# microsoft/Sora

Measured on AMD Instinct MI355X. Metric: IQ Msamples/s through 802.11a 54 Mbps RX PHY, higher is better.
Workload: dtype int16 IQ / u8 path metrics

## Files before the change

### sora_amd/csrc/dev_sym11a.h

```cpp
#pragma once
#include "kernels.h"
#include "dev_viterbi.h"
#include "dev_pilot11a.h"

namespace sora {

__device__ __forceinline__ VitJob frame_vitjob(const FrameRow& r)
{
    VitJob J;
    J.valid = 1; J.soft_off = r.slot0 * (uint32_t)kSoftBytesPerSlot; J.nsoft = (uint32_t)r.nsym * 48u * r.nbpsc; J.length = r.length;
    J.dec_off = 0; J.out_off = r.slot0 * (uint32_t)kOutPerSlot; J.code_rate = r.code_rate; J.soft_bits = 3;
    return J;
}

__device__ __forceinline__ unsigned pilot_sgn(unsigned count)
{
    const unsigned w = count < 32 ? kPilotW0 : count < 64 ? kPilotW1 : count < 96 ? kPilotW2 : kPilotW3;
    return (w >> (count & 31u)) & 1u;
}
static __device__ __constant__ PilotPolarity kPilotSgn = kPilotPolarity;
__device__ __forceinline__ int pilot_angle(int th, unsigned count) { return kPilotSgn.neg[count] ? w16(th + 0x8000) : th; }

template <typename COEF> __device__ __forceinline__ pcx sym_freq_comp(uint32_t raw, COEF fq) { return pk_cmul<15>(pk_sra(raw, 1), pk_tw_mul(fq)); }
template <typename COEF> __device__ __forceinline__ pcx sym_equalise(pcx y, COEF ch, int bin)
{
    return (bin >= 28 && bin < 36) ? 0u : pk_cmul<8>(y, pk_tw_mul(ch));
}
template <typename COEF>
__device__ __forceinline__ void sym_front_quad(const uint32_t raw[4], const COEF fq[4], const COEF ch[4], uint32_t* sl, int e, const Fft64TwPk& W, uint32_t o[4])
{
    pcx x[4];
#pragma unroll
    for (int m = 0; m < 4; m++) x[m] = sym_freq_comp(raw[m], fq[m]);
    fft64_core_pk(x, sl, e, W, wave_lds_sync);
    const unsigned rv = __brev((unsigned)e) >> 28;
#pragma unroll
    for (int q = 0; q < 4; q++) o[q] = sym_equalise(sl[rv + 16u * ((q & 1) * 2 + (q >> 1))], ch[q], 4 * e + q);
    wave_lds_sync();
}

constexpr int kSlotIters = 4;
constexpr uint32_t kNoOwner = 0xFFFFFFFFu;
struct WaveSlots {
    uint32_t first;
    uint32_t my_own;
    unsigned long long owned;
    uint32_t row0;
    bool one_frame;
    __device__ __forceinline__ uint32_t slot(int it, int g) const { return first + 4u * (uint32_t)it + (uint32_t)g; }
    __device__ __forceinline__ uint32_t owner(int it, int g) const { return (uint32_t)__shfl((int)my_own, 4 * it + g); }
    __device__ __forceinline__ unsigned quad(int it) const { return (unsigned)(owned >> (4 * it)) & 0xFu; }
};
__device__ __forceinline__ WaveSlots wave_slots(const RxArgs& A, uint32_t bid)
{
    const int w = threadIdx.x >> 6, lane = threadIdx.x & 63;
    WaveSlots S;
    S.first = (bid * 4u + (uint32_t)w) * (4u * kSlotIters);
    const uint32_t my_slot = S.first + (uint32_t)(lane & 15);
    S.my_own = (lane < 16 && my_slot < A.total_slots) ? A.slot_row[my_slot] : kNoOwner;
    S.owned = __ballot(S.my_own != kNoOwner);
    S.row0 = S.owned ? (uint32_t)__builtin_amdgcn_readlane((int)S.my_own, __builtin_ctzll(S.owned)) : kNoOwner;
    S.one_frame = __ballot(lane < 16 && S.my_own != kNoOwner && S.my_own != S.row0) == 0;
    return S;
}

__device__ __forceinline__ int4 track_advance(int th1, int th2, int th3, int th4, bool act, int& cfo_comp, int& sfo_comp, int& cfo_tr, int& sfo_tr)
{
    const int c0 = cfo_comp, s0 = sfo_comp;
    const int avg = w16((th1 + th2 + th3 + th4) / 4);
    const int del = w16(((th3 - th1) / 28 + (th4 - th2) / 28) >> 1);
    if (act) {
        cfo_tr = w16(cfo_tr + (avg >> 2)); sfo_tr = w16(sfo_tr + (del >> 2));
        cfo_comp = w16(cfo_comp + avg + cfo_tr); sfo_comp = w16(sfo_comp + del + sfo_tr);
    }
    return int4{ c0, s0, act ? avg : 0, act ? del : 0 };
}

__device__ __forceinline__ int4 track_rec4(TrackRec t) { return int4{ t.cfo_comp, t.sfo_comp, t.avg, t.del }; }
__device__ __forceinline__ void sym_back_demap(const Tables& T, const uint8_t* s_demap, const uint32_t v3[3], int4 rec, int nb, int e, uint8_t* dst)
{
    cpx c1[3], c2[3];
#pragma unroll
    for (int m = 0; m < 3; m++) {
        const int bin = carrier_bin48(e + 16 * m);
        const int c = bin < 32 ? bin : bin - 64;
        c1[m] = rot_coeff(T, w16(rec.x + c * rec.y));
        c2[m] = rot_coeff(T, w16(rec.z + c * rec.w));
    }
#pragma unroll
    for (int m = 0; m < 3; m++) {
        const int k = e + 16 * m;
        cpx v = mul_q15(unpack(v3[m]), c1[m]);
        v = mul_q15(v, c2[m]);
        int re = v.re >> 4, im = v.im >> 4;
        re = min(max(re, -128), 127); im = min(max(im, -128), 127);
        const unsigned ur = (unsigned)re & 0xFF, ui = (unsigned)im & 0xFF;
        uint8_t* o = dst + k * nb;
        const int h = nb >> 1;
        o[0] = s_demap[ur];
        if (nb >= 2) {
            o[h] = s_demap[ui];
            if (nb >= 4) {
                const int t1 = nb == 4 ? 256 : 512;
                o[1] = s_demap[t1 + ur]; o[h + 1] = s_demap[t1 + ui];
                if (nb == 6) { o[2] = s_demap[768 + ur]; o[5] = s_demap[768 + ui]; }
            }
        }
    }
}

__device__ __forceinline__ bool deint_packs(int nb, int lane) { return 8 * lane < 48 * nb; }
__device__ __forceinline__ void deint_map_words(const Tables& T, int nb, int lane, uint32_t mp[4])
{
    const uint16_t* map = T.deint + (nb == 1 ? 0 : nb == 2 ? 1 : nb == 4 ? 2 : 3) * 288;
    const bool packs = deint_packs(nb, lane);
#pragma unroll
    for (int t = 0; t < 4; t++) mp[t] = packs ? (uint32_t)map[8 * lane + 2 * t] | ((uint32_t)map[8 * lane + 2 * t + 1] << 16) : 0u;
}
__device__ __forceinline__ uint32_t deint_gather24(const uint8_t* src, const uint32_t mp[4])
{
    uint32_t v[8];
#pragma unroll
    for (int t = 0; t < 4; t++) { v[2 * t] = src[mp[t] & 0xFFFFu]; v[2 * t + 1] = src[mp[t] >> 16]; }
    return soft3_pack8(v);
}

}
```

### sora_amd/csrc/dev_vit16.h

```cpp
#pragma once
#include <hip/hip_runtime.h>
#include "kernels.h"
#include "dev_viterbi.h"

namespace sora {
namespace {

template <int WIN, int LOOK> struct Geom16 {
    static constexpr int kMaxWalk = (WIN + LOOK + 7) / 8 + 2;
    static constexpr int P = kMaxWalk;
    static constexpr int kPathBytes = 40;
};

template <int WIN, int LOOK> struct Lds16 {
    uint16_t ring[Geom16<WIN, LOOK>::P][4][64];
    union {
        uint32_t udump[4][64];
        uint16_t ops[4][24][2];
        uint16_t ops2[2][4][24][2];
    };
    uint32_t path[8][Geom16<WIN, LOOK>::kPathBytes / 4];
};

constexpr unsigned kW[4] = { 0u, 21u, 42u, 63u };
// ... 8 lines not shown
{
    const unsigned c0 = v & 1u, c1 = (v >> 1) & 1u, c2 = (v >> 2) & 1u, c3 = (v >> 3) & 1u;
    return c0 ^ (c2 << 1) ^ (c1 << 3) ^ (c3 ? 7u : 0u);
}
__device__ __forceinline__ unsigned rev6u(unsigned x) { return __brev(x) >> 26; }

template <int CTRL> __device__ __forceinline__ unsigned dppx(unsigned v) { return (unsigned)__builtin_amdgcn_update_dpp(0, (int)v, CTRL, 0xF, 0xF, true); }

__device__ __forceinline__ unsigned partner(unsigned v, int ph)
{
    switch (ph) {
    case 0: return dppx<0x140>(v);
    case 1: return dppx<0x1B>(v);
    case 2: return dppx<0x141>(v);
    case 3: return dppx<0x4E>(v);
    case 4: return dppx<0x128>(v);
    default: return dppx<0xB1>(v);
    }
}

struct Vit16 {
    unsigned U[4];
    unsigned MX[24];
    unsigned MY[6];
    unsigned sadr[3][4];
};

template <int WHICH, int P>
__device__ __forceinline__ void acs16(Vit16& V, int t24, unsigned a, unsigned b, unsigned pos512[3])
{
    const int ph = t24 % 6, k = t24 % 8;
    const unsigned Kp = (WHICH == 0 ? 14u : 7u) * kFld + (kOne << k);
    unsigned bm;
    if (WHICH == 0)      bm = (a ^ V.MX[t24]) + (b ^ V.MY[ph]);
    else if (WHICH == 1) bm = a ^ V.MX[t24];
    else                 bm = b ^ V.MX[t24];
    const unsigned bo = Kp - bm;
    const int rx = ph == 0 ? 2 : ph == 1 ? 1 : 0;
    unsigned N[4];
#pragma unroll
    for (int i = 0; i < 4; i++) {
        const unsigned X = V.U[i], Y = partner(V.U[i ^ rx], ph);
        const bool wb = (kW[i] >> (5 - ph)) & 1u;
        N[i] = wb ? pk_min16(X + bo, Y + bm) : pk_min16(X + bm, Y + bo);
    }
#pragma unroll
    for (int i = 0; i < 4; i++) V.U[i] = N[i];
    if (k == 7) {
        const int jb = t24 / 8;
#pragma unroll
        for (int i = 0; i < 4; i++) {
            const unsigned w = bank_word(V.U[i]);
            const unsigned addr = V.sadr[jb][i] + pos512[jb];
            asm volatile("ds_write_b16 %0, %1" : : "v"(addr), "v"(w) : "memory");
            V.U[i] &= 0xFE00FE00u;
        }
    }
}

__device__ __forceinline__ unsigned row_min_u32(unsigned v)
{
    v = min(v, dppx<0xB1>(v)); v = min(v, dppx<0x4E>(v)); v = min(v, dppx<0x141>(v)); v = min(v, dppx<0x128>(v));
    return v;
}
__device__ __forceinline__ unsigned row_pkmin(unsigned v)
{
    v = pk_min16(v, dppx<0xB1>(v)); v = pk_min16(v, dppx<0x4E>(v)); v = pk_min16(v, dppx<0x141>(v)); v = pk_min16(v, dppx<0x128>(v));
    return v;
}
__device__ __forceinline__ unsigned wave_min_u32(unsigned v) { return (unsigned)__builtin_amdgcn_readfirstlane((int)dpp_min_u32_wave(v)); }
__device__ __forceinline__ unsigned wave_max_u32(unsigned v) { return ~wave_min_u32(~v); }

template <int CR, int WIN, int LOOK, int BITS>
struct Forward16 {
    static constexpr int P = Geom16<WIN, LOOK>::P, GB = Puncture<CR>::GB, GS = Puncture<CR>::GS, CW = Puncture<CR>::CW;
    static constexpr int NV = Puncture<CR>::NV;
    struct Chunk { uint32_t v[CW]; };
    struct Raw { SoftRaw r[NV]; };

    Vit16 V;
    unsigned row, half;
    uint32_t my_j;
    SoftCursor<BITS, CW> cur[NV];
    const uint8_t* soft;
    uint16_t* my_ops;
    const uint4* row_ops;
    uint32_t pos;
    unsigned pos512[3];
    uint32_t tr, nsteps;
    uint32_t next_thr;
    bool all_done;

    __device__ __forceinline__ void init(Lds16<WIN, LOOK>& S, const uint8_t* __restrict__ soft_, uint32_t my_soft_off, uint32_t my_first, uint32_t my_last, unsigned start,
                                         uint32_t nsteps_)
    {
        const unsigned lane = threadIdx.x & 63, l16 = lane & 15;
        row = lane >> 4; half = lane & 1u;
        const unsigned v0 = v_of_lane(l16);
        nsteps = nsteps_;
#pragma unroll
        for (int i = 0; i < 4; i++) V.U[i] = (v0 ^ kW[i]) == 0 ? 0u : start;
        const unsigned ring_base = (unsigned)(uintptr_t)&S.ring[0][0][0];
#pragma unroll
        for (int jb = 0; jb < 3; jb++)
#pragma unroll
            for (int i = 0; i < 4; i++) V.sadr[jb][i] = ring_base + ((row * 64u + rev6u(rol6(v0 ^ kW[i], jb == 0 ? 2 : jb == 1 ? 4 : 0))) << 1);
#pragma unroll
        for (int t = 0; t < 24; t++) {
            const int ph = t % 6, k = t % 8;
            const unsigned n = rol6(v0, ph + 1);
            const bool vb = (v0 >> (5 - ph)) & 1u;
            const unsigned ma = (__popc(n & 0155) & 1) ? 7u * kFld : 0u, mb = (__popc(n & 0117) & 1) ? 7u * kFld : 0u;
            const unsigned mx = Puncture<CR>::which_of(ph) == 2 ? mb : ma;
            V.MX[t] = vb ? ((mx ^ (7u * kFld)) | (kOne << k)) : mx;
            if (t < 6) V.MY[t] = vb ? (mb ^ (7u * kFld)) : mb;
        }
        tr = 0; pos = 0;
        my_j = l16 >> 1;
#pragma unroll
        for (int v = 0; v < NV; v++) cur[v].init(my_soft_off, my_first + my_j + 8u * v, my_last);
        soft = soft_;
        my_ops = &S.ops[row][my_j][half];
        row_ops = reinterpret_cast<const uint4*>(&S.ops[row][0][0]);
        set_row_pos();
    }
    __device__ __forceinline__ bool going() const { return tr < nsteps && !all_done; }

    __device__ __forceinline__ void normalize()
    {
        const unsigned m = row_pkmin(pk_min16(pk_min16(V.U[0], V.U[1]), pk_min16(V.U[2], V.U[3])));
#pragma unroll
        for (int i = 0; i < 4; i++) V.U[i] -= m;
    }
    static __device__ __forceinline__ uint32_t pos_of(uint32_t p, int jb) { const uint32_t q = p + 512u * (uint32_t)jb; return min(q, q - 512u * (uint32_t)P); }
    __device__ __forceinline__ void set_row_pos()
    {
        pos512[0] = pos; pos512[1] = pos_of(pos, 1); pos512[2] = pos_of(pos512[1], 1);
    }
    __device__ __forceinline__ void end_row() { pos = pos_of(pos512[2], 1); set_row_pos(); }
    __device__ __forceinline__ Raw fetch(uint32_t c) const
    {
        Raw R;
#pragma unroll
        for (int v = 0; v < NV; v++) R.r[v] = cur[v].fetch(soft, c);
        return R;
    }
    __device__ __forceinline__ void put(const Raw& R, uint16_t* mine) const
    {
#pragma unroll
        for (int v = 0; v < NV; v++) mine[16 * v] = (uint16_t)cur[v].field(R.r[v]);
    }
    static __device__ __forceinline__ Chunk get(const uint4* table)
    {
        Chunk K;
#pragma unroll
        for (int i = 0; i < (CW + 3) / 4; i++) {
            const uint4 x = table[i];
            K.v[4 * i] = x.x; K.v[4 * i + 1] = x.y;
            if (4 * i + 2 < CW) { K.v[4 * i + 2] = x.z; K.v[4 * i + 3] = x.w; }
        }
        return K;
    }
    __device__ __forceinline__ Chunk unpack(const Raw& R) const
    {
        put(R, my_ops);
        lds_fence();
        const Chunk K = get(row_ops);
        lds_fence();
        return K;
    }
    __device__ __forceinline__ void group(const Chunk& K, int h, int i0)
    {
        const int k0 = i0 / GS * GB, t24 = 12 * h + i0;
        acs16<0, P>(V, t24, K.v[k0], K.v[k0 + 1], pos512);
        if (CR != 0) acs16<1, P>(V, t24 + 1, K.v[k0 + 2], 0, pos512);
        if (CR == 2) acs16<2, P>(V, t24 + 2, 0, K.v[k0 + 3], pos512);
        if ((t24 + GS) % 8 == 0) normalize();
    }
    __device__ __forceinline__ void fast_chunk(const Chunk& K, int h)
    {
#pragma unroll
        for (int g = 0; g < 12 / GS; g++) group(K, h, g * GS);
        tr += 12;
    }
    template <typename CHECK> __device__ __forceinline__ void slow_chunk(const Chunk& K, int h, CHECK& check)
    {
#pragma unroll
        for (int g = 0; g < 12 / GS; g++) {
            if (going()) {
                group(K, h, g * GS);
                tr += GS;
                check(12 * h + g * GS + GS - 1);
            }
        }
    }
    template <typename CHECK> __device__ __forceinline__ void chunk(const Chunk& K, int h, CHECK& check)
    {
        if (tr + 12 <= nsteps && next_thr > tr + 12) fast_chunk(K, h); else slow_chunk(K, h, check);
    }
};

template <int WIN, int LOOK, bool LANE_OB = false>
__device__ __noinline__ void trace16(unsigned lds_off, unsigned U0, unsigned U1, unsigned U2, unsigned U3, uint32_t tr_, uint32_t ob_, uint32_t pj_, uint32_t k_,
                                     uint32_t my_cnt, uint8_t* my_out)
{
    using G = Geom16<WIN, LOOK>;
    constexpr int P = G::P, K = G::kMaxWalk;
    constexpr int NR = K - 1, NF = NR / 4, NW = K / 4 + 1;
    static_assert(NR % 4 == 0 || NR % 4 == 2, "the walk's words are packed in pairs");
    static_assert(NW * 4 <= G::kPathBytes && NW >= WIN / 32 + 1, "the stream's registers hold a window and fit Lds16::path");
    typedef __attribute__((address_space(3))) Lds16<WIN, LOOK> lds_t;
    typedef __attribute__((address_space(3))) const uint16_t lds_u16;
    lds_t& S = *(lds_t*)(uintptr_t)lds_off;
    auto uni = [](uint32_t v) { return (uint32_t)__builtin_amdgcn_readfirstlane((int)v); };
    const uint32_t tr = uni(tr_), ob = LANE_OB ? ob_ : uni(ob_), pj = uni(pj_), k = uni(k_);
    const unsigned lane = threadIdx.x & 63, row = lane >> 4, l16 = lane & 15, half = lane & 1u;
    const unsigned v0 = v_of_lane(l16);
    const unsigned U[4] = { U0, U1, U2, U3 };
    const uint32_t j = (tr - 1) >> 3, nn = tr - 8u * j, m_lo = ob >> 3;
    const unsigned rowbase = (unsigned)(uintptr_t)&S.ring[0][row][0], sh = 8u * half;
    auto ring_j = [&](unsigned idx) -> unsigned { return *(lds_u16*)(uintptr_t)(rowbase + pj + (idx << 1)); };
#pragma unroll
    for (int i = 0; i < 4; i++) S.udump[i][lane] = U[i];
    lds_fence();
    unsigned key[2] = { 0xFFFFFFFFu, 0xFFFFFFFFu };
#pragma unroll
    for (int i = 0; i < 4; i++) {
        const unsigned st = rol6(v0 ^ kW[i], tr);
        unsigned lastA, lastB;
        if (k == 7) { const unsigned w = ring_j(rev6u(st)); lastA = (w >> 7) & 1u; lastB = (w >> 15) & 1u; }
        else { lastA = (U[i] >> k) & 1u; lastB = (U[i] >> (17 + k)) & 1u; }
        const unsigned mA = ((U[i] & 0xFFFFu) >> 9 << 1) | lastA, mB = (U[i] >> 25 << 1) | lastB;
        key[0] = min(key[0], (mA << 8) | (st << 2)); key[1] = min(key[1], (mB << 8) | (st << 2));
// ... 63 lines not shown
```

### sora_amd/csrc/dev_viterbi.h

```cpp
#pragma once
#include <hip/hip_runtime.h>
#include "rx_types.h"

namespace sora {

__device__ __forceinline__ uint32_t uni(uint32_t v) { return (uint32_t)__builtin_amdgcn_readfirstlane((int)v); }
__device__ __forceinline__ void lds_fence() { __builtin_amdgcn_fence(__ATOMIC_RELEASE, "wavefront"); __builtin_amdgcn_wave_barrier();
    __builtin_amdgcn_fence(__ATOMIC_ACQUIRE, "wavefront"); }
constexpr uint32_t kNever = 0xFFFFFFFFu;

template <int CR> struct Puncture {
    static constexpr int GB = CR == 0 ? 2 : CR == 2 ? 4 : 3;
    static constexpr int GS = CR == 0 ? 1 : CR == 2 ? 3 : 2;
    static constexpr int CW = 12 / GS * GB;
    static constexpr int NV = (CW + 7) / 8;
    static constexpr int which_of(int ph) { return CR == 0 ? 0 : CR == 1 ? (ph & 1) : ph % 3; }
};

__device__ __forceinline__ unsigned rol6(unsigned v, unsigned r) { r %= 6; return ((v << r) | (v >> (6 - r))) & 63u; }
__device__ __forceinline__ unsigned lane_map(unsigned x) { return x ^ ((x & 4u) ? 3u : 0u); }

__device__ __forceinline__ unsigned dpp_min_u32_wave(unsigned v)
{
    v = min(v, (unsigned)__builtin_amdgcn_update_dpp(0, (int)v, 0xB1, 0xF, 0xF, true));
    v = min(v, (unsigned)__builtin_amdgcn_update_dpp(0, (int)v, 0x4E, 0xF, 0xF, true));
    v = min(v, (unsigned)__builtin_amdgcn_update_dpp(0, (int)v, 0x124, 0xF, 0xF, true));
    v = min(v, (unsigned)__builtin_amdgcn_update_dpp(0, (int)v, 0x128, 0xF, 0xF, true));
    auto r16 = __builtin_amdgcn_permlane16_swap(v, v, false, false);
    v = min(r16[0], r16[1]);
    auto r32 = __builtin_amdgcn_permlane32_swap(v, v, false, false);
    return min(r32[0], r32[1]);
}

typedef unsigned short u16x2_t __attribute__((ext_vector_type(2)));
__device__ __forceinline__ unsigned pk_add16(unsigned a, unsigned b) { return __builtin_bit_cast(unsigned, (u16x2_t)(__builtin_bit_cast(u16x2_t,
        a) + __builtin_bit_cast(u16x2_t, b))); }
__device__ __forceinline__ unsigned pk_sub16(unsigned a, unsigned b) { return __builtin_bit_cast(unsigned, (u16x2_t)(__builtin_bit_cast(u16x2_t,
        a) - __builtin_bit_cast(u16x2_t, b))); }
__device__ __forceinline__ unsigned pk_min16(unsigned a, unsigned b) { return __builtin_bit_cast(unsigned,
        __builtin_elementwise_min(__builtin_bit_cast(u16x2_t, a), __builtin_bit_cast(u16x2_t, b))); }

__device__ __forceinline__ unsigned dpp_pkmin_wave(unsigned v)
{
    v = pk_min16(v, (unsigned)__builtin_amdgcn_update_dpp(0, (int)v, 0xB1, 0xF, 0xF, true));
    v = pk_min16(v, (unsigned)__builtin_amdgcn_update_dpp(0, (int)v, 0x4E, 0xF, 0xF, true));
    v = pk_min16(v, (unsigned)__builtin_amdgcn_update_dpp(0, (int)v, 0x124, 0xF, 0xF, true));
    v = pk_min16(v, (unsigned)__builtin_amdgcn_update_dpp(0, (int)v, 0x128, 0xF, 0xF, true));
    auto r16 = __builtin_amdgcn_permlane16_swap(v, v, false, false);
    v = pk_min16(r16[0], r16[1]);
    auto r32 = __builtin_amdgcn_permlane32_swap(v, v, false, false);
    return pk_min16(r32[0], r32[1]);
}

__device__ __forceinline__ uint32_t soft3_pack8(const uint32_t v[8])
{
    return v[0] | (v[1] << 3) | (v[2] << 6) | (v[3] << 9) | (v[4] << 12) | (v[5] << 15) | (v[6] << 18) | (v[7] << 21);
}
__device__ __forceinline__ void soft3_store8(uint8_t* stream, uint32_t group, uint32_t bits24)
{
    uint8_t* p = stream + 3u * group;
    p[0] = (uint8_t)bits24; p[1] = (uint8_t)(bits24 >> 8); p[2] = (uint8_t)(bits24 >> 16);
}
struct SoftRaw { uint32_t w, sh; };
template <int BITS, int CW> struct SoftCursor {
    static constexpr int ADV = BITS * CW;
    static constexpr bool kConst = ADV % 8 == 0;
    uint32_t off;
    uint32_t pos;
    uint32_t lim;
    uint32_t lsh;
    __device__ __forceinline__ void init(uint32_t stream_off, uint32_t k, uint32_t last)
    {
        const uint32_t t0 = (uint32_t)BITS * min(k, last), tl = (uint32_t)BITS * last;
        if (kConst) { off = stream_off + (t0 >> 3); pos = 0; lim = stream_off + (tl >> 3); lsh = 9u - (t0 & 7u); }
        else { off = stream_off; pos = t0; lim = tl; lsh = 0; }
    }
    __device__ __forceinline__ SoftRaw fetch(const uint8_t* __restrict__ base, uint32_t c) const
    {
        SoftRaw r;
        if (kConst) { r.sh = 0; r.w = *reinterpret_cast<const uint16_t*>(base + min(off + c * (uint32_t)(ADV / 8), lim)); }
        else { const uint32_t t = min(pos + c * (uint32_t)ADV, lim); r.sh = t & 7u; r.w = *reinterpret_cast<const uint16_t*>(base + (off + (t >> 3))); }
        return r;
    }
    __device__ __forceinline__ uint32_t field(const SoftRaw& r) const
    {
        return kConst ? (r.w << lsh) & 0x0E00u : ((r.w >> r.sh) & 7u) << 9;
    }
};

constexpr unsigned kFld = (1u << 9) | (1u << 25);
constexpr unsigned kOne = 0x00020001u;
constexpr unsigned kGuard = 1u << 16;

template <int WIN, int LOOK> struct RingGeom {
    static constexpr int kMaxWalk = (WIN + LOOK + 7) / 8 + 2;
    static constexpr int P = (kMaxWalk + 2) / 3 * 3;
    static constexpr int kEntries = 2 * P * 64;
};

__device__ __forceinline__ unsigned bank_word(unsigned U) { return __builtin_amdgcn_perm(U >> 1, U, 0x0C0C0600u); }

struct VitLane {
    unsigned U;
    unsigned MX[24];
    unsigned MY[6];
    uint16_t* ring;
    unsigned rowpos;
    unsigned sidx[3];
};

template <int WHICH, int P>
__device__ __forceinline__ void acs_step(VitLane& V, int t24, unsigned a, unsigned b)
{
    const int ph = t24 % 6, k = t24 % 8;
    const unsigned Kp = (WHICH == 0 ? 14u : 7u) * kFld + (kOne << k);
    unsigned bm;
    if (WHICH == 0)      bm = (a ^ V.MX[t24]) + (b ^ V.MY[ph]);
    else if (WHICH == 1) bm = a ^ V.MX[t24];
    else                 bm = b ^ V.MX[t24];
    const unsigned bo = Kp - bm;
    unsigned X, Y;
    const int u = (int)V.U;
    switch (ph) {
    case 0: { auto r = __builtin_amdgcn_permlane32_swap(V.U, V.U, false, false); X = r[0]; Y = r[1]; break; }
    case 1: { auto r = __builtin_amdgcn_permlane16_swap(V.U, V.U, false, false); X = r[0]; Y = r[1]; break; }
    case 2: X = V.U; Y = (unsigned)__builtin_amdgcn_update_dpp(0, u, 0x128, 0xF, 0xF, true); break;
    case 3: X = V.U; Y = (unsigned)__builtin_amdgcn_update_dpp(0, u, 0x141, 0xF, 0xF, true); break;
    case 4: X = V.U; Y = (unsigned)__builtin_amdgcn_update_dpp(0, u, 0x4E, 0xF, 0xF, true); break;
    default: X = V.U; Y = (unsigned)__builtin_amdgcn_update_dpp(0, u, 0xB1, 0xF, 0xF, true); break;
    }
    V.U = pk_min16(X + bm, Y + bo);
    if (k == 7) {
        uint16_t* e = V.ring + V.rowpos + (t24 / 8) * 64 + V.sidx[t24 / 8];
        const uint16_t w = (uint16_t)bank_word(V.U);
        e[0] = w; e[P * 64] = w;
        V.U &= 0xFE00FE00u;
    }
}

template <int kMaxWalk>
__device__ __noinline__ void viterbi_trace(unsigned U, const uint16_t* ring, uint32_t tr_, uint32_t ob_, unsigned mA, unsigned mB,
                                           uint32_t cntA_, uint32_t cntB_, uint8_t* outA, uint8_t* outB, uint32_t top_)
{
    const unsigned lane = threadIdx.x & 63;
    auto uni = [](uint32_t v) { return (uint32_t)__builtin_amdgcn_readfirstlane((int)v); };
    const uint32_t tr = uni(tr_), ob = uni(ob_), cntA = uni(cntA_), cntB = uni(cntB_), top = uni(top_);
    auto rev6 = [](unsigned x) { return __brev(x) >> 26; };
    auto writelane = [](unsigned& vec, unsigned val, unsigned ln) {
        asm volatile("s_mov_b32 m0, %2\n\ts_nop 0\n\tv_writelane_b32 %0, %1, m0" : "+v"(vec) : "s"(val), "s"(ln) : "m0");
    };
    const unsigned lbl = rol6(lane_map(lane), tr) << 2;
    const unsigned kA = (unsigned)__builtin_amdgcn_readfirstlane((int)dpp_min_u32_wave((mA << 8) | lbl));
    const unsigned kB = (unsigned)__builtin_amdgcn_readfirstlane((int)dpp_min_u32_wave((mB << 8) | lbl));
    const unsigned stA = (kA >> 2) & 0x3F, stB = (kB >> 2) & 0x3F;
    const unsigned back = 6u - tr % 6u;
    const unsigned pA = (unsigned)__builtin_amdgcn_readlane((int)U, (int)lane_map(rol6(stA, back))) & 0xFFu;
    const unsigned pB = ((unsigned)__builtin_amdgcn_readlane((int)U, (int)lane_map(rol6(stB, back))) >> 17) & 0xFFu;
    const int m_lo = (int)(ob >> 3);
    const int j = (int)((tr - 1) >> 3);
    const unsigned n = tr - 8u * (unsigned)j;
    const int nblk = j - m_lo;
    __builtin_amdgcn_fence(__ATOMIC_RELEASE, "wavefront"); __builtin_amdgcn_wave_barrier(); __builtin_amdgcn_fence(__ATOMIC_ACQUIRE, "wavefront");
    const unsigned low = (unsigned)(uintptr_t)ring + ((((top - (unsigned)(kMaxWalk - 1)) << 6) | lane) << 1);
    uint32_t W[kMaxWalk];
#pragma unroll
    for (int i = 0; i < kMaxWalk; i++)
        asm volatile("ds_read_u16 %0, %1 offset:%2" : "=v"(W[i]) : "v"(low), "n"((kMaxWalk - 1 - i) * 128) : "memory");
    asm volatile("s_waitcnt lgkmcnt(0)" : "+v"(W[0]) : : "memory");
    unsigned HA, HB;
    if (n == 8) {
        HA = (unsigned)__builtin_amdgcn_readlane((int)W[0], (int)rev6(stA)) & 0xFFu;
        HB = ((unsigned)__builtin_amdgcn_readlane((int)W[0], (int)rev6(stB)) >> 8) & 0xFFu;
    } else { HA = pA & ((1u << n) - 1u); HB = pB & ((1u << n) - 1u); }
    unsigned qA = rev6(((stA >> n) | rev6(HA & 0x3Fu)) & 0x3Fu), qB = rev6(((stB >> n) | rev6(HB & 0x3Fu)) & 0x3Fu);
    unsigned tA = 0, tB = 0;
    asm volatile("s_nop 1\n\tv_writelane_b32 %0, %2, 0\n\tv_writelane_b32 %1, %3, 0" : "+v"(tA), "+v"(tB) : "s"(HA), "s"(HB << 8));
#pragma unroll
    for (int i = 1; i < kMaxWalk; i++) {
        unsigned t;
        asm volatile("v_readlane_b32 %[a], %[w], %[a]\n\t"
                     "v_readlane_b32 %[t], %[w], %[b]\n\t"
                     "s_lshr_b32 %[b], %[t], 8\n\t"
                     "v_writelane_b32 %[ta], %[a], %[i]\n\t"
                     "v_writelane_b32 %[tb], %[t], %[i]"
                     : [a] "+s"(qA), [b] "+s"(qB), [t] "=&s"(t), [ta] "+v"(tA), [tb] "+v"(tB) : [w] "v"(W[i]), [i] "n"(i));
    }
    const int at = (nblk - (int)lane) << 2;
    const unsigned loA = (unsigned)__builtin_amdgcn_ds_bpermute(at, (int)tA) & 0xFFu, upA = (unsigned)__builtin_amdgcn_ds_bpermute(at - 4, (int)tA) & 0xFFu;
    const unsigned loB = ((unsigned)__builtin_amdgcn_ds_bpermute(at, (int)tB) >> 8) & 0xFFu, upB = ((unsigned)__builtin_amdgcn_ds_bpermute(at - 4, (int)tB) >> 8) & 0xFFu;
    if (lane < (cntA >> 3)) outA[m_lo + (int)lane] = (uint8_t)((loA >> 6) | ((upA & 0x3Fu) << 2));
    if (lane < (cntB >> 3)) outB[m_lo + (int)lane] = (uint8_t)((loB >> 6) | ((upB & 0x3Fu) << 2));
}

struct VitSide {
    uint8_t* out; uint32_t nsteps, tr_end; bool done;
    uint32_t soft_off, last, i0;
};

struct WholeFrames {
    __device__ __forceinline__ uint32_t next_event(uint32_t t) const { return t; }
    template <typename E> __device__ __forceinline__ void at_event(E&) {}
    template <typename E> __device__ __forceinline__ void window_done(E&) {}
};

template <int CR, int WIN, int LOOK, int BITS>
struct VitForward {
    using RG = RingGeom<WIN, LOOK>;
    static constexpr int P = RG::P, GB = Puncture<CR>::GB, GS = Puncture<CR>::GS, CW = Puncture<CR>::CW;
    struct Chunk { uint32_t v[(CW + 3) / 4 * 4]; };

    VitLane V;
    VitSide A, B;
    uint32_t nsteps;
    uint32_t tr, ob;
    uint32_t next_thr;
    SoftCursor<BITS, CW> cur;
    const uint8_t* soft_base;
    uint16_t *ops, *my_op;

    __device__ __forceinline__ void init(const VitSide& A_, const VitSide& B_, unsigned start, uint32_t ob0, const uint8_t* __restrict__ soft_base_, uint16_t* ring, uint16_t* ops_)
    {
        const unsigned lane = threadIdx.x & 63;
        A = A_; B = B_;
        nsteps = max(A.nsteps, B.nsteps);
        const VitSide& M = lane >= 32u && !B.done ? B : A;
        const uint32_t my_k = lane & 31u;

        const unsigned vl = lane_map(lane);
        V.U = vl == 0 ? 0u : start;
        V.ring = ring; V.rowpos = 0;
        V.sidx[0] = __brev(rol6(vl, 2)) >> 26; V.sidx[1] = __brev(rol6(vl, 4)) >> 26; V.sidx[2] = __brev(vl) >> 26;
#pragma unroll
        for (int t = 0; t < 24; t++) {
            const int ph = t % 6, k = t % 8;
            const unsigned n = rol6(vl, ph + 1);
            const bool own1 = ph >= 2 && ((vl >> (5 - ph)) & 1);
            const unsigned ma = (__popc(n & 0155) & 1) ? 7u * kFld : 0u, mb = (__popc(n & 0117) & 1) ? 7u * kFld : 0u;
            const unsigned mx = Puncture<CR>::which_of(ph) == 2 ? mb : ma;
            V.MX[t] = own1 ? ((mx ^ (7u * kFld)) | (kOne << k)) : mx;
            if (t < 6) V.MY[t] = own1 ? (mb ^ (7u * kFld)) : mb;
        }
        tr = 0; ob = ob0;
        cur.init(M.soft_off, my_k + M.i0, M.last);
        soft_base = soft_base_; ops = ops_;
        my_op = ops + 2u * my_k + (lane >> 5);
    }
    __device__ __forceinline__ bool going() const { return tr < nsteps && !(A.done && B.done); }

    __device__ __forceinline__ void normalize() { V.U = V.U - dpp_pkmin_wave(V.U); }
    __device__ __forceinline__ SoftRaw fetch(uint32_t c) const { return cur.fetch(soft_base, c); }
    __device__ __forceinline__ Chunk unpack(const SoftRaw& R)
    {
        *my_op = (uint16_t)cur.field(R);
        lds_fence();
        Chunk K;
#pragma unroll
        for (int i = 0; i < (CW + 3) / 4; i++) {
            const uint4 x = reinterpret_cast<const uint4*>(ops)[i];
            K.v[4 * i] = x.x; K.v[4 * i + 1] = x.y; K.v[4 * i + 2] = x.z; K.v[4 * i + 3] = x.w;
        }
        lds_fence();
        return K;
    }
    __device__ __forceinline__ void group(const Chunk& K, int h, int i0)
    {
        const int k0 = i0 / GS * GB, t24 = 12 * h + i0;
        acs_step<0, P>(V, t24, K.v[k0], K.v[k0 + 1]);
        if (CR != 0) acs_step<1, P>(V, t24 + 1, K.v[k0 + 2], 0);
        if (CR == 2) acs_step<2, P>(V, t24 + 2, 0, K.v[k0 + 3]);
        if ((t24 + GS) % 8 == 0) normalize();
    }
    __device__ __forceinline__ void end_row() { V.rowpos = V.rowpos + 3 * 64 == (unsigned)P * 64 ? 0u : V.rowpos + 3 * 64; }
    __device__ __forceinline__ void fast_chunk(const Chunk& K, int h)
    {
#pragma unroll
        for (int g = 0; g < 12 / GS; g++) group(K, h, g * GS);
        tr += 12;
    }

    template <typename SCHED> __device__ __forceinline__ uint32_t next_event(const SCHED& sched) const
    {
        uint32_t t = ob + (uint32_t)(WIN + LOOK + 6);
        if (!A.done) t = min(t, A.tr_end);
        if (!B.done) t = min(t, B.tr_end);
        return sched.next_event(t);
    }
    template <typename SCHED> __device__ __forceinline__ void check(SCHED& sched, int t24_last)
    {
        if (tr >= next_thr) {
            sched.at_event(*this);
            const int k = t24_last % 8;
            const uint32_t pos = V.rowpos + (uint32_t)(t24_last / 8) * 64u;
            unsigned lastA, lastB;
            if (k == 7) { const unsigned w = V.ring[pos + V.sidx[t24_last / 8]]; lastA = (w >> 7) & 1u; lastB = (w >> 15) & 1u; }
            else { lastA = (V.U >> k) & 1u; lastB = (V.U >> (17 + k)) & 1u; }
            const unsigned mA = ((V.U & 0xFFFFu) >> 9 << 1) | lastA, mB = (V.U >> 25 << 1) | lastB;
            const bool partial = tr >= ob + (uint32_t)(WIN + LOOK + 6);
            uint32_t cntA = 0, cntB = 0;
            if (!A.done) {
                if (tr >= A.tr_end) { cntA = A.tr_end - ob - 6; A.done = true; }
                else if (partial) cntA = WIN;
            }
            if (!B.done) {
                if (tr >= B.tr_end) { cntB = B.tr_end - ob - 6; B.done = true; }
                else if (partial) cntB = WIN;
            }
            if (cntA | cntB) viterbi_trace<RG::kMaxWalk>(V.U, V.ring, tr, ob, mA, mB, cntA, cntB, A.out, B.out, (pos >> 6) + (uint32_t)P);
            if (partial) { ob += WIN; sched.window_done(*this); }
            next_thr = next_event(sched);
        }
    }
    template <typename SCHED> __device__ __forceinline__ void slow_chunk(SCHED& sched, const Chunk& K, int h)
    {
#pragma unroll
        for (int g = 0; g < 12 / GS; g++) {
            if (going()) {
                group(K, h, g * GS);
                tr += GS;
                check(sched, 12 * h + g * GS + GS - 1);
            }
        }
    }
    template <typename SCHED> __device__ __forceinline__ void chunk(SCHED& sched, const Chunk& K, int h)
    {
        if (tr + 12 <= nsteps && next_thr > tr + 12) fast_chunk(K, h); else slow_chunk(sched, K, h);
    }

    template <typename SCHED> __device__ __forceinline__ void run(SCHED& sched)
    {
        next_thr = next_event(sched);
        uint32_t c = 0;
        SoftRaw r0 = fetch(0), r1 = fetch(1);
        while (going()) {
            const uint32_t lim = min(nsteps, next_thr - 1);
            for (uint32_t rows = lim > tr ? (lim - tr) / 24 : 0; rows > 0; rows--) {
                const Chunk K0 = unpack(r0); r0 = fetch(c + 2);
// ... 20 lines not shown
```

### sora_amd/csrc/dev_vitwin.h

```cpp
#pragma once
#include <hip/hip_runtime.h>
#include <type_traits>
#include "dev_vit16.h"
#include "dev_winplan.h"

namespace sora {

namespace {

struct UnitGeom {
    uint32_t soft_off, last;
    uint32_t i0;
    uint32_t nsteps;
    uint32_t ob;
    uint32_t tr_end;
    uint32_t vstep, estep;
    uint32_t wleft;
    uint32_t vec;
    uint8_t* out;
    uint32_t need;
    uint32_t idx;
    bool valid, first;
};

// ... 12 lines not shown
    g.soft_off = J.soft_off; g.last = max(J.nsoft, 1u) - 1u;
    g.i0 = s0 / GS * GB;
    g.nsteps = has ? J.nsoft / GB * GS - s0 : 0u;
    g.ob = (uint32_t)WIN * k0 - s0;
    g.tr_end = J.length * 8u + 16u + 6u - s0;
    g.vstep = (has && u != 0) ? (uint32_t)kWinWarm : kNever;
    g.estep = (has && !last) ? (uint32_t)WIN * k1 / 24u * 24u - s0 : kNever;
    g.wleft = last ? 0x10000u : m;
    g.vec = vbase + idx * q + u;
    g.out = out + J.out_off + (s0 >> 3);
    g.need = last ? J.nsoft : min(J.nsoft, (((uint32_t)WIN * k1 + (uint32_t)LOOK + 6u + GS) / GS + 1u) * GB);
    g.idx = idx;
    return g;
}

struct UnitRef { uint32_t idx, uu, m, nun; };
template <int CR, int WIN, int LOOK>
__device__ __forceinline__ UnitRef unit_ref(const VitJob& J, uint32_t n, uint32_t p, uint32_t q, bool inside, uint32_t upos, uint32_t idx)
{
    const uint32_t nev = win_events(J.length, CR, WIN, LOOK), m = win_per_unit(nev, q), nun = (nev + m - 1u) / m;
    const uint32_t uu = !inside ? kWinNone : m != 1u ? (upos < nun ? upos : kWinNone) : n == 1u ? win_unit_lone(upos, nun) : (upos < nun ? win_unit_at(upos, nun) : kWinNone);
    return UnitRef{ idx, uu, m, nun };
}
template <int CR, int WIN, int LOOK, typename JOBS>
__device__ __forceinline__ UnitGeom unit_geom(JOBS job_at, uint32_t n, uint32_t p, uint32_t q, uint32_t vbase, uint8_t* __restrict__ out)
{
    const bool inside = p < win_slots(n, q);
    const uint32_t upos = inside ? p / n : 0u, idx = inside ? p - upos * n : 0u;
    const VitJob J = job_at(idx);
    const UnitRef R = unit_ref<CR, WIN, LOOK>(J, n, p, q, inside, upos, idx);
    return unit_of<CR, WIN, LOOK>(J, idx, R.uu, R.m, R.nun, q, vbase, out);
}
template <int CR, int WIN, int LOOK, typename JOBS>
__device__ __forceinline__ UnitGeom unit_geom_direct(JOBS job_at, uint32_t idx, uint32_t u, bool exists, uint32_t q, uint32_t vbase, uint8_t* __restrict__ out)
{
    const VitJob J = job_at(idx);
    const uint32_t nev = win_events(J.length, CR, WIN, LOOK), m = win_per_unit(nev, q), nun = (nev + m - 1u) / m;
    return unit_of<CR, WIN, LOOK>(J, idx, exists && u < nun ? u : kWinNone, m, nun, q, vbase, out);
}

template <int CR, int WIN, int LOOK, int BITS, typename READY>
__device__ __forceinline__ void forward16w(Lds16<WIN, LOOK>& S, const uint8_t* __restrict__ soft, const UnitGeom& GA, const UnitGeom& GB_, uint16_t* __restrict__ vecs, READY ready)
{
    using F16 = Forward16<CR, WIN, LOOK, BITS>;
    using Raw = typename F16::Raw;
    constexpr uint32_t THR = WIN + LOOK + 6;
    const unsigned l16 = threadIdx.x & 15;
    const UnitGeom& Mine = (threadIdx.x & 1u) ? GB_ : GA;
    F16 F;
    F.init(S, soft, Mine.soft_off, Mine.i0, Mine.last, (GA.first ? 0x18u << 9 : 0u) | (GB_.first ? 0x18u << 25 : 0u), wave_max_u32(max(GA.nsteps, GB_.nsteps)));

    uint32_t my_ob = Mine.ob, my_wleft = Mine.wleft;
    const uint32_t my_tr_end = Mine.tr_end;
    bool my_done = !Mine.valid;
    uint32_t vstepA = GA.vstep, vstepB = GB_.vstep, estepA = GA.estep, estepB = GB_.estep;

    auto trace = [&](uint32_t my_cnt, int t24_last) {
        trace16<WIN, LOOK, true>((unsigned)(uintptr_t)&S, F.V.U[0], F.V.U[1], F.V.U[2], F.V.U[3], F.tr, my_ob, F16::pos_of(F.pos, t24_last / 8), (uint32_t)(t24_last % 8), my_cnt,
                                 Mine.out);
    };
    auto next_event = [&]() -> uint32_t {
        uint32_t mine = my_done ? kNever : min(my_ob + THR, my_tr_end);
        mine = min(min(mine, min(vstepA, vstepB)), min(estepA, estepB));
        return wave_min_u32(mine);
    };
    F.next_thr = next_event();
    F.all_done = wave_min_u32(my_done ? 1u : 0u) != 0u;
    auto save = [&](uint32_t vec, int which, bool hi) {
        uint16_t* d = vecs + ((size_t)vec * 2u + (uint32_t)which) * 64u + l16;
#pragma unroll
        for (int i = 0; i < 4; i++) d[16 * i] = (uint16_t)(hi ? F.V.U[i] >> 16 : F.V.U[i]);
    };
    auto check = [&](int t24_last) {
        if (F.tr >= F.next_thr) {
            if (F.tr == vstepA) { save(GA.vec, 0, false); vstepA = kNever; }
            if (F.tr == vstepB) { save(GB_.vec, 0, true); vstepB = kNever; }
            if (F.tr == estepA) { save(GA.vec, 1, false); estepA = kNever; }
            if (F.tr == estepB) { save(GB_.vec, 1, true); estepB = kNever; }
            uint32_t cnt = 0; bool partial = false;
            if (!my_done) {
                if (F.tr >= my_tr_end) { cnt = my_tr_end - my_ob - 6; my_done = true; }
                else if (F.tr >= my_ob + THR) { cnt = WIN; partial = true; }
            }
            if (wave_max_u32(cnt) != 0u) trace(cnt, t24_last);
            if (partial) { my_ob += WIN; if (--my_wleft == 0) my_done = true; }
            F.next_thr = next_event();
            F.all_done = wave_min_u32(my_done ? 1u : 0u) != 0u;
        }
    };

    uint32_t c = 0;
    if (!ready()) return;
    Raw b0 = F.fetch(0), b1 = F.fetch(1), b2, b3;
    while (F.going()) {
        const uint32_t lim = min(F.nsteps, F.next_thr - 1);
        uint32_t rows = lim > F.tr ? (lim - F.tr) / 24 : 0;
        for (; rows > 0; rows--) {
            b2 = F.fetch(c + 2);
            F.fast_chunk(F.unpack(b0), 0);
            b3 = F.fetch(c + 3);
            F.fast_chunk(F.unpack(b1), 1);
            F.end_row();
            b0 = b2; b1 = b3;
            c += 2;
        }
        if (!(F.tr < F.nsteps)) break;
        b2 = F.fetch(c + 2);
        F.chunk(F.unpack(b0), 0, check);
        if (!F.going()) break;
        b3 = F.fetch(c + 3);
        F.chunk(F.unpack(b1), 1, check);
        F.end_row();
        b0 = b2; b1 = b3;
        c += 2;
    }
}

template <int WIN, int LOOK, int BITS, typename JOBSOF, typename READY>
__device__ __forceinline__ void viterbi16w_wave(Lds16<WIN, LOOK>& S, uint32_t wave_index, JOBSOF jobs_of, READY ready, const uint32_t* __restrict__ hdr,
        uint32_t target, uint32_t vstride,
                                                const uint8_t* __restrict__ soft, uint8_t* __restrict__ out, uint16_t* __restrict__ vecs)
{
    const uint32_t n[3] = { hdr[0], hdr[1], hdr[2] };
    const uint32_t q = uni(win_units_per_frame(n[0] + n[1] + n[2], target));
    uint32_t w = uni(wave_index), list = 0;
    while (list < 3 && w >= (win_slots(n[list], q) + 7) / 8) { w -= (win_slots(n[list], q) + 7) / 8; list++; }
    if (list >= 3) return;
    const uint32_t nl = uni(n[list]);
    const auto job_at = jobs_of(list);
    const unsigned lane = threadIdx.x & 63, row = lane >> 4;
    const uint32_t pa = 8u * w + 2u * row, pb = pa + 1u, vbase = list * vstride;
    const uint32_t code_rate = uni(job_at(0).code_rate);
    auto run = [&](auto cr) {
        constexpr int CR = decltype(cr)::value;
        UnitGeom A = unit_geom<CR, WIN, LOOK>(job_at, nl, pa, q, vbase, out), B = unit_geom<CR, WIN, LOOK>(job_at, nl, pb, q, vbase, out);
        if (__ballot(A.valid || B.valid) == 0) return;
        if (!B.valid) { const bool v = false; B = A; B.valid = v; B.vstep = B.estep = kNever; B.nsteps = 0; }
        if (!A.valid) { const bool v = false; const UnitGeom T = B; A = T; A.valid = v; A.vstep = A.estep = kNever; A.nsteps = 0; }
        forward16w<CR, WIN, LOOK, BITS>(S, soft, A, B, vecs, [&]() { return ready(A, B, list); });
    };
    if (code_rate == 0) run(std::integral_constant<int, 0>{});
    else if (code_rate == 1) run(std::integral_constant<int, 1>{});
    else run(std::integral_constant<int, 2>{});
}

template <int WIN, int LOOK, int BITS>
__device__ __forceinline__ void viterbi16w_body(const VitJob* __restrict__ jobs, const uint32_t* __restrict__ hdr, uint32_t jstride, uint32_t target, uint32_t vstride,
                                                const uint8_t* __restrict__ soft, uint8_t* __restrict__ out, uint16_t* __restrict__ vecs)
{
    __shared__ Lds16<WIN, LOOK> S;
    auto jobs_of = [&](uint32_t list) { const VitJob* __restrict__ jl = jobs + (size_t)list * jstride; return [jl](uint32_t idx) { return jl[idx]; }; };
    auto ready = [](const UnitGeom&, const UnitGeom&, uint32_t) { return true; };
    viterbi16w_wave<WIN, LOOK, BITS>(S, blockIdx.x, jobs_of, ready, hdr, target, vstride, soft, out, vecs);
}

}

}
```

### sora_amd/csrc/host_trellis.h

```cpp
#pragma once
#include <algorithm>
#include <optional>
#include "host_calls.h"
#include "kernels.h"
#include "dev_winplan.h"

namespace sora {

enum class Trellis { Lanes64, Lanes16, Windowed };
using TrellisChoice = std::optional<Trellis>;
inline int trellis_abi(Trellis t) { return t == Trellis::Lanes16 ? 16 : t == Trellis::Windowed ? SORA_TRELLIS_WINDOWED : 64; }
inline int trellis_abi(const TrellisChoice& c) { return c ? trellis_abi(*c) : 0; }
inline bool trellis_parse(int lanes_per_pair, TrellisChoice* out)
{
    if (lanes_per_pair == 0) *out = std::nullopt;
    else if (lanes_per_pair == 16) *out = Trellis::Lanes16;
    else if (lanes_per_pair == 64) *out = Trellis::Lanes64;
    else if (lanes_per_pair == SORA_TRELLIS_WINDOWED) *out = Trellis::Windowed;
    else return false;
    return true;
}

constexpr uint32_t kWinUnitsTarget = 16384;
constexpr uint32_t kWinLoneWaves = 3 * kWinLonePad / 8;
inline uint64_t win_units(uint64_t rows) { return std::min<uint64_t>(std::max<uint64_t>(kWinUnitsTarget, rows), (uint64_t)kWinMaxUnits * rows); }
inline uint64_t win_waves(uint64_t rows) { return (win_units(rows) + 7) / 8 + 3 + kWinLoneWaves; }
inline uint32_t win_vstride(uint64_t rows) { return (uint32_t)(win_units(rows) + rows); }

struct TrellisJobs { const VitJob* jobs; const uint32_t* hdr; uint32_t n, stride; bool single; };
inline TrellisJobs trellis_lists(const VitJob* jobs, const uint32_t* hdr, uint32_t n, uint32_t stride) { return TrellisJobs{ jobs, hdr, n, stride, false }; }
inline TrellisJobs trellis_single(const VitJob* jobs, const uint32_t* hdr, uint32_t n) { return TrellisJobs{ jobs, hdr, n, n, true }; }
inline uint32_t trellis_pair_groups(const TrellisJobs& J) { return J.single ? (J.n + 7) / 8 : (J.n / 2 + 3 + 3) / 4; }
inline uint32_t trellis_waves16(const TrellisJobs& J) { return (J.n + 7) / 8 + (J.single ? 0u : 2u); }
inline uint32_t trellis_win_waves(const TrellisJobs& J)
{
    return J.single ? (win_slots(J.n, win_units_per_frame(J.n, kWinUnitsTarget)) + 7) / 8 : (uint32_t)win_waves(J.n);
}

constexpr size_t kWinStatsBytes = 4 * kWinStatBanks * sizeof(unsigned long long);
struct WinScratch {
    uint16_t* d_vecs = nullptr; unsigned long long* d_stats = nullptr; uint32_t stride = 0;

    unsigned long long* redone() const { return d_stats + kWinStatsBytes / sizeof(unsigned long long); }
    int ensure(uint64_t cap_rows, hipStream_t zero_on, bool extra)
    {
        if (d_vecs) return SORA_OK;
        stride = win_vstride(cap_rows);
        HIPCHK(hipMalloc((void**)&d_vecs, 3 * (size_t)kWinVecBytes * stride));
        HIPCHK(hipMalloc((void**)&d_stats, kWinStatsBytes + sizeof(unsigned long long)));
        const size_t bytes = kWinStatsBytes + (extra ? sizeof(unsigned long long) : 0);
        if (zero_on) HIPCHK(hipMemsetAsync(d_stats, 0, bytes, zero_on));
        else HIPCHK(hipMemset(d_stats, 0, bytes));
        return SORA_OK;
    }
    void free() { (void)hipFree(d_vecs); (void)hipFree(d_stats); d_vecs = nullptr; d_stats = nullptr; stride = 0; }
};
inline int win_stats_add(const unsigned long long* d_stats, hipStream_t st, unsigned long long out[4])
{
    unsigned long long v[4 * kWinStatBanks];
    HIPCHK(hipMemcpyAsync(v, d_stats, sizeof v, hipMemcpyDeviceToHost, st));
    HIPCHK(hipStreamSynchronize(st));
    for (unsigned i = 0; i < 4 * kWinStatBanks; i++) out[i & 3u] += v[i];
    return SORA_OK;
}
template <typename P> inline int win_stats_sum(P* const* s, int n, int device, unsigned long long out[4])
{
    HIPCHK(hipSetDevice(device));
    for (int i = 0; i < 4; i++) out[i] = 0;
    for (int i = 0; i < n; i++) if (s[i] && s[i]->win.d_stats) { const int rc = win_stats_add(s[i]->win.d_stats, s[i]->stream, out); if (rc) return rc; }
    return SORA_OK;
}

template <int WIN> inline void trellis_proof(const TrellisJobs& J, const uint8_t* soft, uint8_t* out, const WinScratch& W, hipStream_t st)
{
    static_assert(WIN == 256 || WIN == 192, "the 802.11a (256) or the 802.11n (192) window schedule");
    if constexpr (WIN == 256)
        hipLaunchKernelGGL(k_win_redo, dim3(trellis_pair_groups(J)), dim3(256), 0, st, J.jobs, J.hdr, J.stride, kWinUnitsTarget, W.stride, (const uint16_t*)W.d_vecs, soft, out, W.d_stats);
    else
        hipLaunchKernelGGL(k_win_redo_11n, dim3(trellis_pair_groups(J)), dim3(256), 0, st, J.jobs, J.hdr, J.stride, kWinUnitsTarget, W.stride, (const uint16_t*)W.d_vecs, soft, out, W.d_stats);
}
template <int WIN> inline void trellis_launch(Trellis kind, const TrellisJobs& J, const uint8_t* soft, uint8_t* out, hipStream_t st, const WinScratch& W = WinScratch(),
        bool proof = true)
{
    static_assert(WIN == 256 || WIN == 192, "the 802.11a (256) or the 802.11n (192) window schedule");
    const uint32_t* hdr = J.single ? nullptr : J.hdr;
    const uint32_t n1 = J.single ? J.n : 0u, stride = J.single ? 0u : J.stride;
    if (kind == Trellis::Windowed) {
        if constexpr (WIN == 256) hipLaunchKernelGGL(k_viterbi16w, dim3(trellis_win_waves(J)), dim3(64), 0, st, J.jobs, J.hdr, J.stride, kWinUnitsTarget, W.stride, soft, out, W.d_vecs);
        else hipLaunchKernelGGL(k_viterbi16w_11n, dim3(trellis_win_waves(J)), dim3(64), 0, st, J.jobs, J.hdr, J.stride, kWinUnitsTarget, W.stride, soft, out, W.d_vecs);
        if (proof) trellis_proof<WIN>(J, soft, out, W, st);
    } else if (kind == Trellis::Lanes16) {
        if constexpr (WIN == 256) hipLaunchKernelGGL(k_viterbi16, dim3(trellis_waves16(J)), dim3(64), 0, st, J.jobs, hdr, n1, stride, soft, out);
        else hipLaunchKernelGGL(k_viterbi16_11n, dim3(trellis_waves16(J)), dim3(64), 0, st, J.jobs, hdr, n1, stride, soft, out);
    } else {
        if constexpr (WIN == 256) hipLaunchKernelGGL(k_viterbi, dim3(trellis_pair_groups(J)), dim3(256), 0, st, J.jobs, hdr, n1, stride, soft, out);
        else hipLaunchKernelGGL(k_viterbi11n, dim3(trellis_pair_groups(J)), dim3(256), 0, st, J.jobs, hdr, n1, stride, soft, out);
    }
}

}
```

### sora_amd/csrc/k_rx.hip

```cpp
#include <hip/hip_runtime.h>
#include <utility>
#include "kernels.h"
#include "dev_sym11a.h"
#include "dev_viterbi.h"
#include "dev_winplan.h"
#include "dev_vitwin.h"

namespace sora {

struct FrameLds {
    uint32_t eq[4][4][64];
    uint8_t  soft[4][4][288];
    uint8_t  demap[1024];
    int4     trk[4][4];
    int      nsym_of[4];
    short    st0[4][4];
};
template <bool SHARED>
__device__ __forceinline__ void frame_symbols(const RxArgs& A, uint32_t j, FrameLds& lds, bool valid = true)
{
    uint32_t (&s_eq)[4][4][64] = lds.eq; uint8_t (&s_soft)[4][4][288] = lds.soft; const uint8_t* s_demap = lds.demap;
    const int w = threadIdx.x >> 6, lane = threadIdx.x & 63, g = lane >> 4, e = lane & 15;
    const Tables& T = A.T;
    const uint32_t f = valid ? A.joblist[j] : 0u;
// ... 15 lines not shown
    const int pbin = pk == 0 ? 43 : pk == 1 ? 57 : pk == 2 ? 7 : 21, pc = pk == 0 ? -21 : pk == 1 ? -7 : pk == 2 ? 7 : 21;
    int cfo_comp = r.cfo_comp, sfo_comp = r.sfo_comp, cfo_tr = r.cfo_tracker, sfo_tr = r.sfo_tracker;
    unsigned symbol_count = 0;

    const uint32_t str_shift = A.str >> 1;
    auto load_samples = [&](int s0, uint32_t raw[4]) {
        const uint32_t p0 = r.data_start + __umul24(80u, (uint32_t)min(s0 + g, nsym)) + 8u + (uint32_t)e;
#pragma unroll
        for (int m = 0; m < 4; m++) raw[m] = iq[(p0 + 16u * (uint32_t)m) << str_shift];
    };
    int nsym_loop = nsym, nsym_f = nsym;
    if (SHARED) {
        if (lane == 0) { lds.nsym_of[w] = nsym; lds.st0[w][0] = (short)cfo_comp; lds.st0[w][1] = (short)sfo_comp; lds.st0[w][2] = (short)cfo_tr; lds.st0[w][3] = (short)sfo_tr; }
        __syncthreads();
        nsym_loop = max(max(lds.nsym_of[0], lds.nsym_of[1]), max(lds.nsym_of[2], lds.nsym_of[3]));
        const int fr = (lane >> 2) & 3;
        nsym_f = lds.nsym_of[fr];
        cfo_comp = lds.st0[fr][0]; sfo_comp = lds.st0[fr][1]; cfo_tr = lds.st0[fr][2]; sfo_tr = lds.st0[fr][3];
    }
    uint32_t raw[4] = { 0u, 0u, 0u, 0u };
    if (1 <= nsym) load_samples(1, raw);
    for (int s0 = 1; s0 <= nsym_loop; s0 += 4) {
        const int sym = s0 + g;
        const bool active = sym <= nsym;
        const bool mine = s0 <= nsym;
        int4 rec = { 0, 0, 0, 0 };
        if (mine) {
            pcx x[4], Y[4];
#pragma unroll
            for (int m = 0; m < 4; m++) x[m] = sym_freq_comp(raw[m], fq[m]);
            if (s0 + 4 <= nsym) load_samples(s0 + 4, raw);
            fft64_core_pk(x, s_eq[w][g], e, W, wave_lds_sync);
#pragma unroll
            for (int q = 0; q < 4; q++) Y[q] = s_eq[w][g][__brev((unsigned)(e + 16 * q)) >> 26];
            wave_lds_sync();
#pragma unroll
            for (int q = 0; q < 4; q++) s_eq[w][g][e + 16 * q] = sym_equalise(Y[q], ch[q], e + 16 * q);
            wave_lds_sync();
        }
        if (SHARED) {
            __syncthreads();
            if (w == 0) {
                const int fr = (lane >> 2) & 3;
#pragma unroll
                for (int gg = 0; gg < 4; gg++) {
                    const cpx p = mul_q15(unpack(s_eq[fr][gg][pbin]), rot_coeff(T, w16(cfo_comp + pc * sfo_comp)));
                    const int th = pilot_angle(pk == 3 ? uatan2(T, -p.im, -p.re) : uatan2(T, p.im, p.re), (symbol_count + (unsigned)gg) % 127u);
                    int th1 = __builtin_amdgcn_update_dpp(0, th, 0x00, 0xF, 0xF, true), th2 = __builtin_amdgcn_update_dpp(0, th, 0x55, 0xF, 0xF, true);
                    int th3 = __builtin_amdgcn_update_dpp(0, th, 0xAA, 0xF, 0xF, true), th4 = __builtin_amdgcn_update_dpp(0, th, 0xFF, 0xF, 0xF, true);
                    asm volatile("" : "+v"(th1), "+v"(th2), "+v"(th3), "+v"(th4));
                    const int4 t = track_advance(th1, th2, th3, th4, s0 + gg <= nsym_f, cfo_comp, sfo_comp, cfo_tr, sfo_tr);
                    if (lane < 16 && pk == 0) lds.trk[fr][gg] = t;
                }
            }
            symbol_count = (symbol_count + 4u) % 127u;
            __syncthreads();
            rec = lds.trk[w][g];
        } else {
            int4 t[4];
#pragma unroll
            for (int gg = 0; gg < 4; gg++) {
                t[gg] = int4{ cfo_comp, sfo_comp, 0, 0 };
                if (s0 + gg <= nsym) {
                    const cpx p = mul_q15(unpack(s_eq[w][gg][pbin]), rot_coeff(T, w16(cfo_comp + pc * sfo_comp)));
                    const int th = pilot_angle(pk == 3 ? uatan2(T, -p.im, -p.re) : uatan2(T, p.im, p.re), symbol_count);
                    symbol_count++; if (symbol_count >= 127) symbol_count = 0;
                    t[gg] = track_advance(__builtin_amdgcn_readlane(th, 0), __builtin_amdgcn_readlane(th, 1), __builtin_amdgcn_readlane(th, 2), __builtin_amdgcn_readlane(th, 3),
                                          true, cfo_comp, sfo_comp, cfo_tr, sfo_tr);
                }
            }
            rec = t[0];
            if (g == 1) rec = t[1]; else if (g == 2) rec = t[2]; else if (g == 3) rec = t[3];
        }
        if (!mine) continue;
        if (active) {
            uint32_t v3[3];
#pragma unroll
            for (int m = 0; m < 3; m++) v3[m] = s_eq[w][g][carrier_bin48(e + 16 * m)];
            sym_back_demap(T, s_demap, v3, rec, nb, e, s_soft[w][g]);
        }
        wave_lds_sync();
        {
            const int nact = min(4, nsym - s0 + 1);
            const uint32_t sym_bytes = 3u * (uint32_t)ncbps / 8u;
            uint8_t* d = dst + (size_t)(s0 - 1) * sym_bytes;
            for (int gs = 0; gs < nact; gs++, d += sym_bytes)
                if (packs) soft3_store8(d, (uint32_t)lane, deint_gather24(s_soft[w][gs], mp));
        }
        wave_lds_sync();
    }
}
__global__ void __launch_bounds__(256) k_frame(RxArgs A)
{
    __shared__ FrameLds lds;
    reinterpret_cast<uint32_t*>(lds.demap)[threadIdx.x] = reinterpret_cast<const uint32_t*>(A.T.demap)[threadIdx.x];
    __syncthreads();
    if (!locate_job(blockIdx.x * 4, A.njobs).ok) return;
    const JobRef jr = locate_job(blockIdx.x * 4 + (threadIdx.x >> 6), A.njobs);
    frame_symbols<true>(A, jr.ok ? jr.list * A.nrows + jr.idx : 0u, lds, jr.ok);
}

typedef uint32_t u32x4_t __attribute__((ext_vector_type(4)));
__device__ __forceinline__ void store16_through(uint4* p, uint4 v)
{
    const u32x4_t x = { v.x, v.y, v.z, v.w };
    asm volatile("global_store_dwordx4 %0, %1, off sc1\n\ts_nop 1" : : "v"(p), "v"(x) : "memory");
}
__device__ __forceinline__ void store4_through(uint32_t* p, uint32_t v) { __hip_atomic_store(p, v, __ATOMIC_RELAXED, __HIP_MEMORY_SCOPE_AGENT); }

template <bool THROUGH>
__device__ __forceinline__ void sym_front_block(const RxArgs& A, uint32_t bid, uint32_t (*s_eq)[4][64])
{
    const int w = threadIdx.x >> 6, lane = threadIdx.x & 63, g = lane >> 4, e = lane & 15;
    const Tables& T = A.T;
    const WaveSlots S = wave_slots(A, bid);
    if (S.owned == 0) return;
    uint32_t own[kSlotIters];
#pragma unroll
    for (int it = 0; it < kSlotIters; it++) own[it] = S.owner(it, g);
    const Fft64TwPk W = fft64_twiddles_pk(T, e);
    uint32_t* sl = s_eq[w][g];
    uint4* eq4 = reinterpret_cast<uint4*>(A.eq);
    auto store = [&](uint32_t slot, const uint32_t o[4]) {
        if (THROUGH) store16_through(eq4 + ((size_t)slot * 16u + (uint32_t)e), uint4{ o[0], o[1], o[2], o[3] });
        else eq4[(size_t)slot * 16u + (uint32_t)e] = uint4{ o[0], o[1], o[2], o[3] };
        auto pilot = [&](uint32_t k, uint32_t v) { if (THROUGH) store4_through(A.pil + ((size_t)slot * 4u + k), v); else A.pil[(size_t)slot * 4u + k] = v; };
        if (e == 10) pilot(0u, o[3]);
        if (e == 14) pilot(1u, o[1]);
        if (e == 1)  pilot(2u, o[3]);
        if (e == 5)  pilot(3u, o[1]);
    };
    if (S.one_frame) {
        const FrameRow& r = A.frames[S.row0];
        const uint32_t* iq = A.iq + A.caps[r.capture].offset;
        const uint32_t ds = r.data_start, s0 = r.slot0, str = A.str;
        const FrameCtx* fx = A.fctx + S.row0;
        uint32_t raw[kSlotIters][4];
#pragma unroll
        for (int it = 0; it < kSlotIters; it++) {
            const uint32_t p0 = ds + 80u * (S.slot(it, g) - s0) + 8u;
#pragma unroll
            for (int m = 0; m < 4; m++) raw[it][m] = own[it] != kNoOwner ? iq[(size_t)(p0 + (uint32_t)(e + 16 * m)) * str] : 0u;
        }
        PkTw fq[4], ch[4];
#pragma unroll
        for (int m = 0; m < 4; m++) { fq[m] = pk_tw_mul(fx->freq[e + 16 * m]); ch[m] = pk_tw_mul(fx->chan[4 * e + m]); }
#pragma unroll
        for (int it = 0; it < kSlotIters; it++) {
            if (S.quad(it) == 0) continue;
            uint32_t o[4];
            sym_front_quad(raw[it], fq, ch, sl, e, W, o);
            if (own[it] != kNoOwner) store(S.slot(it, g), o);
        }
        return;
    }
#pragma unroll 1
    for (int it = 0; it < kSlotIters; it++) {
        if (S.quad(it) == 0) continue;
        const uint32_t ow = S.owner(it, g);
        const bool mine = ow != kNoOwner;
        const uint32_t slot = S.slot(it, g);
        uint32_t raw[4] = { 0u, 0u, 0u, 0u };
        PkTw fq[4], ch[4];
        const FrameCtx* fx = A.fctx + (mine ? ow : 0u);
        if (mine) {
            const FrameRow& r = A.frames[ow];
            const uint32_t* iq = A.iq + A.caps[r.capture].offset;
            const uint32_t p0 = r.data_start + 80u * (slot - r.slot0) + 8u;
#pragma unroll
            for (int m = 0; m < 4; m++) raw[m] = iq[(size_t)(p0 + (uint32_t)(e + 16 * m)) * A.str];
        }
#pragma unroll
        for (int m = 0; m < 4; m++) { fq[m] = pk_tw_mul(mine ? fx->freq[e + 16 * m] : 0u); ch[m] = pk_tw_mul(mine ? fx->chan[4 * e + m] : 0u); }
        uint32_t o[4];
        sym_front_quad(raw, fq, ch, sl, e, W, o);
        if (mine) store(slot, o);
    }
}
// ... 25 lines not shown
                 "v_mov_b32_dpp %1, %4 quad_perm:[1,1,1,1] row_mask:0xf bank_mask:0xf bound_ctrl:1\n\t"
                 "v_mov_b32_dpp %2, %4 quad_perm:[2,2,2,2] row_mask:0xf bank_mask:0xf bound_ctrl:1\n\t"
                 "v_mov_b32_dpp %3, %4 quad_perm:[3,3,3,3] row_mask:0xf bank_mask:0xf bound_ctrl:1"
                 : "=&v"(th1), "=&v"(th2), "=&v"(th3), "=&v"(th4) : "v"(th));
    const int sum = th1 + th2 + th3 + th4;
    const int avg = (sum + ((sum >> 31) & 3)) >> 2;
    const int del = ((int)((float)(th3 - th1) * kInv28) + (int)((float)(th4 - th2) * kInv28)) >> 1;
    const uint2 rec = uint2{ __builtin_amdgcn_perm((uint32_t)sfo, (uint32_t)cfo, 0x05040100u), __builtin_amdgcn_perm((uint32_t)del, (uint32_t)avg, 0x05040100u) };
    ctr += avg >> 2; str += del >> 2;
    cfo = (int)((unsigned)cfo + (unsigned)avg + (unsigned)ctr); sfo = __builtin_amdgcn_sbfe(sfo + del + str, 0, 16);
    return rec;
}

__device__ __forceinline__ void track_tables_to_lds(const uint32_t* __restrict__ trk, TrkTables& s_t, uint32_t* s_pol)
{
    if (threadIdx.x < 127) {
        unsigned b = 0;
#pragma unroll
        for (unsigned u = 0; u < 8; u++) b |= pilot_sgn((threadIdx.x + u) % 127u) << u;
        s_pol[threadIdx.x] = b;
    }
    const uint4* src = reinterpret_cast<const uint4*>(trk);
    uint4* dst = reinterpret_cast<uint4*>(&s_t);
    constexpr uint32_t kWords = sizeof(TrkTables) / 16, kBatch = 11;
    for (uint32_t i0 = threadIdx.x; i0 < kWords; i0 += 256u * kBatch) {
        uint4 v[kBatch];
#pragma unroll
        for (uint32_t b = 0; b < kBatch; b++) v[b] = src[min(i0 + 256u * b, kWords - 1u)];
#pragma unroll
        for (uint32_t b = 0; b < kBatch; b++) if (i0 + 256u * b < kWords) dst[i0 + 256u * b] = v[b];
    }
}

__global__ void __launch_bounds__(256) k_track_lds(RxArgs A)
{
    __shared__ TrkTables s_t;
    __shared__ uint32_t s_pol[128];
    track_tables_to_lds(A.T.trk, s_t, s_pol);
    __syncthreads();
    const int lane = threadIdx.x & 63, pk = lane & 3;
    const JobRef jr = locate_job(blockIdx.x * 64u + (threadIdx.x >> 2), A.njobs);
    const uint32_t j = jr.ok ? jr.list * A.nrows + jr.idx : 0u;
    const uint32_t f = jr.ok ? A.joblist[j] : 0u;
    const FrameRow r = A.frames[f];
    const int nsym = jr.ok ? (int)r.nsym : 0;
    if (jr.ok && pk == 0) A.jobs[j] = frame_vitjob(r);
    const int pc = pk == 0 ? -21 : pk == 1 ? -7 : pk == 2 ? 7 : 21;
    const int m3 = pk == 3 ? -1 : 0;
    int cfo = r.cfo_comp, sfo = r.sfo_comp, ctr = r.cfo_tracker, str = r.sfo_tracker;
    int nmax = nsym;
#pragma unroll
    for (int o = 32; o >= 4; o >>= 1) nmax = max(nmax, __shfl_xor(nmax, o));
    nmax = __builtin_amdgcn_readfirstlane(nmax);
    const uint32_t w0 = (jr.ok ? (r.slot0 + 1u) * 4u + (uint32_t)pk : (uint32_t)pk) * 4u;
    const uint32_t t0 = (jr.ok ? r.slot0 + 1u : A.total_slots + 1u) * 8u;
    const char* __restrict__ pil = reinterpret_cast<const char*>(A.pil);
    char* __restrict__ trk2 = reinterpret_cast<char*>(A.track);
    const unsigned last = (unsigned)max(nsym, 1) - 1u, nrec = (unsigned)nsym;
    constexpr int kAhead = 8;
    uint32_t q[kAhead];
#pragma unroll
    for (int i = 0; i < kAhead; i++) q[i] = *reinterpret_cast<const uint32_t*>(pil + (w0 + 16u * min((unsigned)i, last)));
    unsigned cnt = 0;
    for (int s0 = 1; s0 <= nmax; s0 += kAhead) {
        const unsigned pol = (unsigned)__builtin_amdgcn_readfirstlane((int)s_pol[cnt]);
        cnt = cnt + (unsigned)kAhead >= 127u ? cnt + (unsigned)kAhead - 127u : cnt + (unsigned)kAhead;
#pragma unroll
        for (int u = 0; u < kAhead; u++) {
            const int s = s0 + u;
            const uint32_t cur = q[u];
            q[u] = *reinterpret_cast<const uint32_t*>(pil + (w0 + 16u * min((unsigned)(s + kAhead - 1), last)));
            const int flip = (int)((pol << (15 - u)) & 0x8000u);
            *reinterpret_cast<uint2*>(trk2 + (t0 + 8u * min((unsigned)(s - 1), nrec))) = track_step(s_t, cur, flip, pc, m3, cfo, sfo, ctr, str);
        }
    }
}

__global__ void __launch_bounds__(256) k_sym_back(RxArgs A)
{
    __shared__ uint8_t s_soft[4][4][288];
    __shared__ uint8_t s_demap[1024];
    const int w = threadIdx.x >> 6, lane = threadIdx.x & 63, g = lane >> 4, e = lane & 15;
    const Tables& T = A.T;
    reinterpret_cast<uint32_t*>(s_demap)[threadIdx.x] = reinterpret_cast<const uint32_t*>(T.demap)[threadIdx.x];
    __syncthreads();
    const WaveSlots S = wave_slots(A, blockIdx.x);
    if (S.owned == 0) return;
    int bins[3];
#pragma unroll
    for (int m = 0; m < 3; m++) bins[m] = carrier_bin48(e + 16 * m);
    if (S.one_frame) {
        const FrameRow& r = A.frames[S.row0];
        const int nb = __builtin_amdgcn_readfirstlane((int)r.nbpsc), ncbps = 48 * nb;
        const uint32_t slot0 = (uint32_t)__builtin_amdgcn_readfirstlane((int)r.slot0), sym_bytes = 3u * (uint32_t)ncbps / 8u;
        uint8_t* stream = A.soft + (size_t)slot0 * kSoftBytesPerSlot;
        const bool packs = deint_packs(nb, lane);
        uint32_t mp[4];
        deint_map_words(T, nb, lane, mp);
        TrackRec tr[kSlotIters]; uint32_t v3[kSlotIters][3];
#pragma unroll
        for (int it = 0; it < kSlotIters; it++) {
            const uint32_t slot = S.slot(it, g);
            const bool mine = (S.quad(it) >> g) & 1u;
            tr[it] = mine ? A.track[slot] : TrackRec{ 0, 0, 0, 0 };
#pragma unroll
            for (int m = 0; m < 3; m++) v3[it][m] = mine ? A.eq[(size_t)slot * 64u + (uint32_t)bins[m]] : 0u;
        }
#pragma unroll
        for (int it = 0; it < kSlotIters; it++) {
            const unsigned quad = S.quad(it);
            if (quad == 0) continue;
            if ((quad >> g) & 1u) sym_back_demap(T, s_demap, v3[it], track_rec4(tr[it]), nb, e, s_soft[w][g]);
            wave_lds_sync();
#pragma unroll
            for (int gs = 0; gs < 4; gs++) {
                if (!((quad >> gs) & 1u) || !packs) continue;
                const uint32_t sg = S.slot(it, gs);
                soft3_store8(stream + (size_t)(sg - slot0 - 1u) * sym_bytes, (uint32_t)lane, deint_gather24(s_soft[w][gs], mp));
            }
            wave_lds_sync();
        }
        return;
    }
    int cur_nb = 0; uint32_t mp[4] = { 0, 0, 0, 0 };
#pragma unroll 1
    for (int it = 0; it < kSlotIters; it++) {
        const unsigned quad = S.quad(it);
        if (quad == 0) continue;
        const uint32_t ow = S.owner(it, g);
        const bool mine = ow != kNoOwner;
        const uint32_t slot = S.slot(it, g);
        int nb = 0; uint32_t slot0 = 0;
        if (mine) {
            const FrameRow& r = A.frames[ow];
            nb = r.nbpsc; slot0 = r.slot0;
            uint32_t v3[3];
#pragma unroll
            for (int m = 0; m < 3; m++) v3[m] = A.eq[(size_t)slot * 64u + (uint32_t)bins[m]];
            sym_back_demap(T, s_demap, v3, track_rec4(A.track[slot]), nb, e, s_soft[w][g]);
        }
        wave_lds_sync();
#pragma unroll 1
        for (int gs = 0; gs < 4; gs++) {
            if (!((quad >> gs) & 1u)) continue;
            const int nbg = __shfl(nb, 16 * gs);
            const uint32_t slot0g = (uint32_t)__shfl((int)slot0, 16 * gs);
            if (nbg != cur_nb) { cur_nb = nbg; deint_map_words(T, nbg, lane, mp); }
            if (deint_packs(nbg, lane)) {
                const uint32_t sg = S.slot(it, gs);
                uint8_t* d = A.soft + (size_t)slot0g * kSoftBytesPerSlot + (size_t)(sg - slot0g - 1u) * (3u * 48u * (uint32_t)nbg / 8u);
                soft3_store8(d, (uint32_t)lane, deint_gather24(s_soft[w][gs], mp));
            }
        }
        wave_lds_sync();
    }
}

constexpr uint32_t kPipeMaxSym = 1376;
constexpr uint32_t kPipeRing = 512;
struct PipeTrackLds {
    TrkTables t;
    uint32_t pol[128];
    uint32_t pil[kPipeMaxSym][4];
    uint2 rec[kPipeRing];
    uint8_t demap[1024];
    uint8_t soft[3][4][288];
    uint32_t done;
    uint32_t next_quad[3];
    uint32_t give_up;
    uint32_t pad[11];
};
constexpr uint32_t kPipeLdsBytes = sizeof(PipeTrackLds);
static_assert(kPipeLdsBytes <= 160 * 1024 && sizeof(TrkTables) % 16 == 0, "k_pipe: a tracker workgroup's LDS");
static_assert(4 * sizeof(Lds16<256, 24>) <= kPipeLdsBytes, "k_pipe: four trellis waves' LDS");

#ifdef SORA_DBG_PIPE_TIMELINE
#define PIPE_STAMP(P, i) do { if ((threadIdx.x & 63) == 0) (P).flags[(P).stamp_base + (i)] = (uint32_t)wall_clock64(); } while (0)
#else
#define PIPE_STAMP(P, i) do {} while (0)
#endif
__device__ __forceinline__ uint32_t flag_load(const uint32_t* p) { return __hip_atomic_load(p, __ATOMIC_RELAXED, __HIP_MEMORY_SCOPE_AGENT); }
__device__ __forceinline__ bool pipe_expired(long long t0, uint32_t wait_ticks) { return wall_clock64() - t0 > (long long)wait_ticks; }

__device__ __forceinline__ void pipe_track_block(const RxArgs& A, const PipeArgs& P, uint32_t t, PipeTrackLds& L)
{
    const int w = threadIdx.x >> 6, lane = threadIdx.x & 63;
    const JobRef jr = locate_job(t, A.njobs);
    if (!jr.ok) return;
    track_tables_to_lds(A.T.trk, L.t, L.pol);
    reinterpret_cast<uint32_t*>(L.demap)[threadIdx.x] = reinterpret_cast<const uint32_t*>(A.T.demap)[threadIdx.x];
    const uint32_t j = jr.list * A.nrows + jr.idx, f = A.joblist[j];
    const FrameRow r = A.frames[f];
    const uint32_t nsym = min((uint32_t)r.nsym, kPipeMaxSym - 8u), slot0 = r.slot0;
    if (threadIdx.x == 0) {
        A.jobs[j] = frame_vitjob(r);
        L.done = 0; L.give_up = 0; L.next_quad[0] = 0; L.next_quad[1] = 1; L.next_quad[2] = 2;
    }
    if (w == 0) {
        const uint32_t b0 = (slot0 + 1u) >> 6, b1 = (slot0 + max(nsym, 1u)) >> 6;
        const uint32_t* fl = P.flags + 4u + 4u * A.nrows + b0 + (uint32_t)lane;
        const bool mine = b0 + (uint32_t)lane <= b1;
        const long long t0 = wall_clock64();
        bool gave_up = false;
        while (!__all(!mine || flag_load(fl) != 0u)) {
            if (pipe_expired(t0, P.wait_ticks)) { gave_up = true; break; }
            __builtin_amdgcn_s_sleep(8);
        }
        if (gave_up && lane == 0) { L.give_up = 1; atomicOr(P.flags, 1u); }
        PIPE_STAMP(P, 1);
    }
    __syncthreads();
    if (L.give_up) return;
    {
        const unsigned long long* src = reinterpret_cast<const unsigned long long*>(A.pil) + 2u * (size_t)(slot0 + 1u);
        unsigned long long* dst = reinterpret_cast<unsigned long long*>(&L.pil[0][0]);
        for (uint32_t i = threadIdx.x; i < 2u * (nsym + 8u); i += 256u) dst[i] = i < 2u * nsym ? __hip_atomic_load(src + i, __ATOMIC_RELAXED, __HIP_MEMORY_SCOPE_AGENT) : 0ull;
    }
    __syncthreads();
    if (w == 0) {
        __builtin_amdgcn_s_setprio(3);
        PIPE_STAMP(P, 2);
        if (lane < 4) {
            const int pk = lane & 3;
            const int pc = pk == 0 ? -21 : pk == 1 ? -7 : pk == 2 ? 7 : 21, m3 = pk == 3 ? -1 : 0;
            int cfo = r.cfo_comp, sfo = r.sfo_comp, ctr = r.cfo_tracker, str = r.sfo_tracker;
            unsigned cnt = 0;
            volatile uint32_t* done = &L.done; volatile uint32_t* nq = L.next_quad;
            for (uint32_t s0 = 1; s0 <= nsym; s0 += 8u) {
                if (s0 + 7u > kPipeRing) {
                    while (4u * min(min(nq[0], nq[1]), nq[2]) + kPipeRing < s0 + 7u) __builtin_amdgcn_s_sleep(1);
                }
                const unsigned pol = (unsigned)__builtin_amdgcn_readfirstlane((int)L.pol[cnt]);
                cnt = cnt + 8u >= 127u ? cnt + 8u - 127u : cnt + 8u;
                uint32_t q[8];
#pragma unroll
                for (int u = 0; u < 8; u++) q[u] = L.pil[s0 - 1u + (uint32_t)u][pk];
                const uint32_t ring = (s0 - 1u) & (kPipeRing - 1u);
#pragma unroll
                for (int u = 0; u < 8; u++) L.rec[ring + (uint32_t)u] = track_step(L.t, q[u], (int)((pol << (15 - u)) & 0x8000u), pc, m3, cfo, sfo, ctr, str);
                asm volatile("" ::: "memory");
                if (lane == 0) *done = min(s0 + 7u, nsym);
            }
        }
        PIPE_STAMP(P, 3);
        return;
    }
    __builtin_amdgcn_fence(__ATOMIC_ACQUIRE, "agent");
    const int h = w - 1, g = lane >> 4, e = lane & 15;
    const int nb = __builtin_amdgcn_readfirstlane((int)r.nbpsc), ncbps = 48 * nb;
    const uint32_t sym_bytes = 3u * (uint32_t)ncbps / 8u;
    uint8_t* stream = A.soft + (size_t)slot0 * kSoftBytesPerSlot;
    const bool packs = deint_packs(nb, lane);
    uint32_t mp[4];
    deint_map_words(A.T, nb, lane, mp);
    int bins[3];
#pragma unroll
    for (int m = 0; m < 3; m++) bins[m] = carrier_bin48(e + 16 * m);
    volatile uint32_t* done = &L.done; volatile uint32_t* nq = L.next_quad;
    uint32_t* my_count = P.flags + 4u + 4u * f + (uint32_t)h;
    uint32_t quads = 0;
    uint8_t* bytes = &L.soft[h][0][0];
    for (uint32_t k = (uint32_t)h; 4u * k < nsym; k += 3u) {
        const uint32_t nact = min(4u, nsym - 4u * k), s = 4u * k + 1u + (uint32_t)g;
        const bool mine = (uint32_t)g < nact;
        uint32_t v3[3];
#pragma unroll
        for (int m = 0; m < 3; m++) v3[m] = mine ? A.eq[(size_t)(slot0 + s) * 64u + (uint32_t)bins[m]] : 0u;
        while (*done < 4u * k + nact) __builtin_amdgcn_s_sleep(1);
        asm volatile("" ::: "memory");
        const uint2 rw = L.rec[(s - 1u) & (kPipeRing - 1u)];
        if (mine) sym_back_demap(A.T, L.demap, v3, int4{ (int16_t)rw.x, (int16_t)(rw.x >> 16), (int16_t)rw.y, (int16_t)(rw.y >> 16) }, nb, e, L.soft[h][g]);
        wave_lds_sync();
        uint32_t b24[4];
#pragma unroll
        for (int gs = 0; gs < 4; gs++) b24[gs] = deint_gather24(L.soft[h][gs], mp);
        wave_lds_sync();
        if (packs) {
#pragma unroll
            for (int gs = 0; gs < 4; gs++) soft3_store8(bytes + (uint32_t)gs * sym_bytes, (uint32_t)lane, b24[gs]);
        }
        wave_lds_sync();
        const uint32_t ndw = (nact * sym_bytes + 3u) / 4u;
        uint32_t* out32 = reinterpret_cast<uint32_t*>(stream + (size_t)(4u * k) * sym_bytes);
        for (uint32_t i = (uint32_t)lane; i < ndw; i += 64u) store4_through(out32 + i, reinterpret_cast<const uint32_t*>(bytes)[i]);
        asm volatile("s_waitcnt vmcnt(0)" ::: "memory");
        wave_lds_sync();
        quads++;
        if (lane == 0) { store4_through(my_count, quads); nq[h] = k + 3u; }
    }
    if (lane == 0) nq[h] = 0x3FFFFFFFu;
    PIPE_STAMP(P, 4 + h);
}

__device__ __forceinline__ bool pipe_units_ready(const RxArgs& A, const PipeArgs& P, uint32_t list, const UnitGeom& M, bool polls_, uint32_t wave_index)
{
    const unsigned lane = threadIdx.x & 63;
    const bool polls = polls_ && M.valid;
    const uint32_t f = A.joblist[(size_t)list * A.nrows + M.idx];
    const uint32_t ncbps = 48u * A.frames[f].nbpsc;
    const uint32_t quads = polls ? ((M.need + ncbps - 1u) / ncbps + 3u) / 4u : 0u;
    const uint32_t* c = P.flags + 4u + 4u * f;
    const long long t0 = wall_clock64();
    for (;;) {
        bool ok = true;
#pragma unroll
        for (uint32_t h = 0; h < 3; h++) ok = ok && flag_load(c + h) >= (quads + 2u - h) / 3u;
        if (__all(ok)) break;
        if (pipe_expired(t0, P.wait_ticks)) { if (lane == 0) atomicOr(P.flags, 1u); return false; }
        __builtin_amdgcn_s_sleep(2);
    }
    __builtin_amdgcn_fence(__ATOMIC_ACQUIRE, "agent");
    PIPE_STAMP(P, 16 + 2 * wave_index);
    return true;
}

__device__ __forceinline__ auto pipe_jobs_of(const RxArgs& A, uint32_t list)
{
    const uint32_t* jl = A.joblist + (size_t)list * A.nrows; const FrameRow* fr = A.frames;
    return [jl, fr](uint32_t idx) { return frame_vitjob(fr[jl[idx]]); };
}
__device__ __forceinline__ void pipe_trellis_wave(const RxArgs& A, const PipeArgs& P, uint32_t wave_index, Lds16<256, 24>& S)
{
    auto jobs_of = [&](uint32_t list) { return pipe_jobs_of(A, list); };
    auto ready = [&](const UnitGeom& GA, const UnitGeom& GB_, uint32_t list) -> bool {
        const unsigned lane = threadIdx.x & 63;
        return pipe_units_ready(A, P, list, (lane & 1u) ? GB_ : GA, (lane & 15u) < 2u, wave_index);
    };
    viterbi16w_wave<256, 24, 3>(S, wave_index, jobs_of, ready, A.njobs, P.target, P.vstride, (const uint8_t*)A.soft, A.vout, P.vecs);
    PIPE_STAMP(P, 17 + 2 * wave_index);
}


template <int CR, int WIN, int LOOK, int BITS>
__device__ __forceinline__ void viterbi_forward(const VitJob& JA, const VitJob& JB, bool hasB, const uint8_t* __restrict__ soft_base,
        uint8_t* __restrict__ out_base, uint16_t* ring, uint16_t* ops)
{
    auto side = [&](const VitJob& J, bool has) {
        VitSide s;
        s.out = out_base + J.out_off; s.nsteps = has ? J.nsoft / Puncture<CR>::GB * Puncture<CR>::GS : 0u; s.tr_end = has ? J.length * 8u + 16u + 6u : 0u; s.done = !has;
        s.soft_off = J.soft_off; s.last = max(J.nsoft, 1u) - 1u; s.i0 = 0;
        return s;
    };
    VitForward<CR, WIN, LOOK, BITS> F;
    F.init(side(JA, true), side(JB, hasB), 0x18u * kFld, 0, soft_base, ring, ops);
    WholeFrames sched;
    F.run(sched);
}

struct UnitSchedule64 {
    uint16_t* __restrict__ vecs;
    uint32_t vecA, vecB;
    uint32_t wA, wB, vstepA, vstepB, estepA, estepB;
    __device__ __forceinline__ uint32_t next_event(uint32_t t) const { return min(min(t, min(vstepA, vstepB)), min(estepA, estepB)); }
    __device__ __forceinline__ void save(unsigned U, uint32_t vec, int which, bool hi) const
    {
        vecs[((size_t)vec * 2u + (uint32_t)which) * 64u + (threadIdx.x & 63)] = (uint16_t)(hi ? U >> 16 : U);
    }
    template <typename E> __device__ __forceinline__ void at_event(E& F)
    {
        if (F.tr == vstepA) { save(F.V.U, vecA, 0, false); vstepA = kNever; }
        if (F.tr == vstepB) { save(F.V.U, vecB, 0, true); vstepB = kNever; }
        if (F.tr == estepA) { save(F.V.U, vecA, 1, false); estepA = kNever; }
        if (F.tr == estepB) { save(F.V.U, vecB, 1, true); estepB = kNever; }
    }
    template <typename E> __device__ __forceinline__ void window_done(E& F)
    {
        if (!F.A.done && --wA == 0) F.A.done = true;
        if (!F.B.done && --wB == 0) F.B.done = true;
    }
};
template <int CR, int WIN, int LOOK, int BITS, typename READY>
__device__ __forceinline__ void viterbi_forward_unit(const UnitGeom& GA, const UnitGeom& GB_, const uint8_t* __restrict__ soft_base, uint16_t* ring, uint16_t* ops,
        uint16_t* __restrict__ vecs, READY ready)
{
    const bool hasB = GB_.valid;
    auto side = [](const UnitGeom& G, bool has) {
        VitSide s;
        s.out = G.out; s.nsteps = has ? G.nsteps : 0u; s.tr_end = has ? G.tr_end : 0u; s.done = !has;
        s.soft_off = G.soft_off; s.last = G.last; s.i0 = G.i0;
        return s;
    };
    VitForward<CR, WIN, LOOK, BITS> F;
    F.init(side(GA, true), side(GB_, hasB), (GA.first ? 0x18u << 9 : 0u) | ((hasB && GB_.first) ? 0x18u << 25 : 0u), GA.ob, soft_base, ring, ops);
    UnitSchedule64 sched{ vecs, GA.vec, GB_.vec, GA.wleft, GB_.wleft, GA.vstep, hasB ? GB_.vstep : kNever, GA.estep, hasB ? GB_.estep : kNever };
    if (!ready()) return;
    F.run(sched);
}

struct PipeUnitLds { uint16_t ring[RingGeom<256, 24>::kEntries]; uint16_t ops[64]; };
static_assert(4 * sizeof(PipeUnitLds) <= kPipeLdsBytes, "k_pipe: four 64-lane trellis waves' LDS");
__device__ __forceinline__ void pipe_trellis_wave64(const RxArgs& A, const PipeArgs& P, uint32_t wave_index, PipeUnitLds& L)
{
    const uint32_t n[3] = { A.njobs[0], A.njobs[1], A.njobs[2] };
    const uint32_t q = uni(win_units_per_frame(n[0] + n[1] + n[2], P.target));
    uint32_t w = uni(wave_index), list = 0;
    while (list < 3 && w >= q * ((n[list] + 1u) / 2u)) { w -= q * ((n[list] + 1u) / 2u); list++; }
    if (list >= 3) return;
    const uint32_t nl = uni(n[list]), pairs = (nl + 1u) / 2u, u = w / pairs, ia = 2u * (w - u * pairs), ib = ia + 1u;
    const auto job_at = pipe_jobs_of(A, list);
    const uint32_t code_rate = uni(job_at(0).code_rate), vbase = list * P.vstride;
    auto run = [&](auto cr) {
        constexpr int CR = decltype(cr)::value;
        UnitGeom GA = unit_geom_direct<CR, 256, 24>(job_at, ia, u, true, q, vbase, A.vout);
        UnitGeom GB_ = unit_geom_direct<CR, 256, 24>(job_at, ib < nl ? ib : ia, u, ib < nl, q, vbase, A.vout);
        if (GB_.valid && GA.valid && GB_.ob != GA.ob && (threadIdx.x & 63) == 0) atomicOr(P.flags, 1u);
        if (GB_.valid && (!GA.valid || GB_.ob != GA.ob)) { if (!GA.valid) { GA = GB_; } const bool no = false; GB_.valid = no; }
        if (!GA.valid) return;
        const unsigned lane = threadIdx.x & 63;
        viterbi_forward_unit<CR, 256, 24, 3>(GA, GB_, (const uint8_t*)A.soft, L.ring, L.ops, P.vecs,
                                             [&]() { return pipe_units_ready(A, P, list, lane >= 32u ? GB_ : GA, (lane & 31u) == 0u, wave_index); });
    };
    if (code_rate == 0) run(std::integral_constant<int, 0>{});
    else if (code_rate == 1) run(std::integral_constant<int, 1>{});
    else run(std::integral_constant<int, 2>{});
    PIPE_STAMP(P, 17 + 2 * wave_index);
}

__global__ void __launch_bounds__(256) k_pipe(RxArgs A, PipeArgs P)
{
    __shared__ __attribute__((aligned(16))) char lds[kPipeLdsBytes];
    uint32_t b = blockIdx.x;
    if (b == 0) PIPE_STAMP(P, 0);
    if (b < P.nfront) {
        sym_front_block<true>(A, b, reinterpret_cast<uint32_t (*)[4][64]>(lds));
        asm volatile("s_waitcnt vmcnt(0)" ::: "memory");
        __syncthreads();
#ifndef SORA_DBG_PIPE_LOSE_FLAGS
        if (threadIdx.x == 0) store4_through(P.flags + 4u + 4u * A.nrows + b, 1u);
#endif
        if (b == 0) PIPE_STAMP(P, 8);
        return;
    }
    b -= P.nfront;
    if (b < P.ntrack) { pipe_track_block(A, P, b, *reinterpret_cast<PipeTrackLds*>(lds)); return; }
    b -= P.ntrack;
    if (P.lanes64) pipe_trellis_wave64(A, P, b * 4u + (threadIdx.x >> 6), reinterpret_cast<PipeUnitLds*>(lds)[threadIdx.x >> 6]);
    else pipe_trellis_wave(A, P, b * 4u + (threadIdx.x >> 6), reinterpret_cast<Lds16<256, 24>*>(lds)[threadIdx.x >> 6]);
}


struct DecodeEveryPair { __device__ __forceinline__ bool operator()(uint32_t, uint32_t, uint32_t, bool) const { return true; } };
struct NothingAfter { __device__ __forceinline__ void operator()(uint32_t, uint32_t, uint32_t, bool) const {} };
template <int WIN, int LOOK, int BITS, typename GATE = DecodeEveryPair, typename AFTER = NothingAfter>
__device__ __forceinline__ void viterbi_kernel_body(const VitJob* __restrict__ jobs, const uint32_t* __restrict__ njobs3, uint32_t njobs_single,
        uint32_t stride, const uint8_t* __restrict__ soft, uint8_t* __restrict__ out,
                                                    GATE gate = GATE(), AFTER after = AFTER())
{
    __shared__ uint16_t s_ring[4][RingGeom<WIN, LOOK>::kEntries];
    __shared__ uint16_t s_ops[4][64];
    uint32_t n[3] = { njobs_single, 0, 0 };
    if (njobs3) { n[0] = njobs3[0]; n[1] = njobs3[1]; n[2] = njobs3[2]; }
    uint32_t pw = uni(blockIdx.x * 4 + (threadIdx.x >> 6)), list = 0;
    while (list < 3 && pw >= (n[list] + 1) / 2) { pw -= (n[list] + 1) / 2; list++; }
    if (list >= 3) return;
    const uint32_t njobs = uni(n[list]);
    jobs += (size_t)list * stride;
    const uint32_t fa = pw * 2, fb = fa + 1;
    if (gate(list, fa, fb, fb < njobs)) {
        uint16_t* ring = s_ring[threadIdx.x >> 6];
        auto load_job = [&](uint32_t f) {
            const VitJob& G = jobs[f];
            VitJob J;
            J.soft_off = uni(G.soft_off); J.nsoft = uni(G.nsoft); J.length = uni(G.length); J.dec_off = uni(G.dec_off);
            J.out_off = uni(G.out_off); J.valid = uni(G.valid); J.code_rate = uni(G.code_rate); J.soft_bits = uni(G.soft_bits);
            return J;
        };
        const VitJob JA = load_job(fa);
        const bool hasB = fb < njobs;
        const VitJob JB = hasB ? load_job(fb) : JA;
        if (JA.code_rate == 0)      viterbi_forward<0, WIN, LOOK, BITS>(JA, JB, hasB, soft, out, ring, s_ops[threadIdx.x >> 6]);
        else if (JA.code_rate == 1) viterbi_forward<1, WIN, LOOK, BITS>(JA, JB, hasB, soft, out, ring, s_ops[threadIdx.x >> 6]);
        else                        viterbi_forward<2, WIN, LOOK, BITS>(JA, JB, hasB, soft, out, ring, s_ops[threadIdx.x >> 6]);
        __builtin_amdgcn_fence(__ATOMIC_SEQ_CST, "workgroup");
    }
    after(list, fa, fb, fb < njobs);
}

__global__ void __launch_bounds__(256) k_viterbi(const VitJob* __restrict__ jobs, const uint32_t* __restrict__ njobs3, uint32_t njobs_single, uint32_t stride,
        const uint8_t* __restrict__ soft, uint8_t* __restrict__ out)
{ viterbi_kernel_body<256, 24, 3>(jobs, njobs3, njobs_single, stride, soft, out); }
__global__ void __launch_bounds__(256) k_viterbi11n(const VitJob* __restrict__ jobs, const uint32_t* __restrict__ njobs3, uint32_t njobs_single,
        uint32_t stride, const uint8_t* __restrict__ soft, uint8_t* __restrict__ out)
{ viterbi_kernel_body<192, 36, 8>(jobs, njobs3, njobs_single, stride, soft, out); }

template <uint32_t WIN, uint32_t LOOK>
struct WinProofGateT {
    const VitJob* jobs; const uint32_t* hdr; uint32_t jstride, target, vstride; const uint16_t* vecs; unsigned long long* stats;
    __device__ __forceinline__ bool operator()(uint32_t list, uint32_t fa, uint32_t fb, bool hasB) const
    {
        const unsigned lane = threadIdx.x & 63, side = lane >> 5, l32 = lane & 31u;
        const uint32_t q = win_units_per_frame(hdr[0] + hdr[1] + hdr[2], target);
        const uint32_t idx = side ? fb : fa;
        const bool have = side ? hasB : true;
        const VitJob& J = jobs[(size_t)list * jstride + (have ? idx : fa)];
        const uint32_t nev = win_events(J.length, J.code_rate, WIN, LOOK), m = win_per_unit(nev, q), nun = have ? (nev + m - 1u) / m : 1u;
        const size_t vec0 = (size_t)list * vstride + (size_t)idx * q;
        uint32_t bad = 0;
        for (uint32_t u = 1u + l32; u < nun; u += 32u) {
            const uint4* a = reinterpret_cast<const uint4*>(vecs + ((vec0 + u) * 2u) * 64u);
            const uint4* b = reinterpret_cast<const uint4*>(vecs + ((vec0 + u - 1u) * 2u + 1u) * 64u);
            uint32_t d = 0;
#pragma unroll
            for (int i = 0; i < 8; i++) { const uint4 x = a[i], y = b[i]; d |= (x.x ^ y.x) | (x.y ^ y.y) | (x.z ^ y.z) | (x.w ^ y.w); }
            bad += d != 0u;
        }
        const unsigned long long ba = __ballot(bad != 0u);
        uint32_t nbad = bad;
#pragma unroll
        for (int o = 16; o >= 1; o >>= 1) nbad += __shfl_xor(nbad, o);
        if (stats && l32 == 0 && have) {
            unsigned long long* bk = stats + 4u * ((blockIdx.x * 4u + (threadIdx.x >> 6)) & (kWinStatBanks - 1u));
            atomicAdd(&bk[0], (unsigned long long)(nun - 1u)); atomicAdd(&bk[3], (unsigned long long)nun);
            if (nbad) { atomicAdd(&bk[1], (unsigned long long)nbad); atomicAdd(&bk[2], 1ull); }
        }
        return ba != 0ull;
    }
};
using WinProofGate = WinProofGateT<256u, 24u>;
__global__ void __launch_bounds__(256) k_win_redo(const VitJob* __restrict__ jobs, const uint32_t* __restrict__ hdr, uint32_t jstride, uint32_t target,
        uint32_t vstride, const uint16_t* __restrict__ vecs,
                                                  const uint8_t* __restrict__ soft, uint8_t* __restrict__ out, unsigned long long* __restrict__ stats)
{ viterbi_kernel_body<256, 24, 3>(jobs, hdr, 0u, jstride, soft, out, WinProofGate{ jobs, hdr, jstride, target, vstride, vecs, stats }); }
__global__ void __launch_bounds__(256) k_win_redo_11n(const VitJob* __restrict__ jobs, const uint32_t* __restrict__ hdr, uint32_t jstride, uint32_t target,
        uint32_t vstride, const uint16_t* __restrict__ vecs,
                                                      const uint8_t* __restrict__ soft, uint8_t* __restrict__ out, unsigned long long* __restrict__ stats)
{ viterbi_kernel_body<192, 36, 8>(jobs, hdr, 0u, jstride, soft, out, WinProofGateT<192u, 36u>{ jobs, hdr, jstride, target, vstride, vecs, stats }); }

struct FinishLds {
    uint32_t crc[256]; uint32_t z[6 * 8 * 16]; uint32_t bufs[4][2504 / 4 + 2];
    uint32_t seq4[128];
    uint8_t  phase[128];
};
__device__ __forceinline__ void finish_tables_to_lds(const RxArgs& A, FinishLds& L)
{
    L.crc[threadIdx.x] = A.T.crc[threadIdx.x];
    for (int i = threadIdx.x; i < 6 * 8 * 16; i += 256) L.z[i] = A.T.crcz[i];
    if (threadIdx.x < 127) {
        const uint8_t* q = A.T.scr_seq; const uint32_t p = threadIdx.x;
        L.seq4[p] = (uint32_t)q[p] | ((uint32_t)q[(p + 8u) % 127u] << 8) | ((uint32_t)q[(p + 16u) % 127u] << 16) | ((uint32_t)q[(p + 24u) % 127u] << 24);
    }
    if (threadIdx.x >= 128) L.phase[threadIdx.x - 128] = A.T.scr_phase[threadIdx.x - 128];
}
__device__ __forceinline__ void finish_frame(const RxArgs& A, uint32_t f, FinishLds& lds)
{
    const uint32_t* s_crc = lds.crc; const uint32_t* s_z = lds.z; uint32_t (*s_bufs)[2504 / 4 + 2] = lds.bufs;
    FrameRow& r = A.frames[f];
    if (!r.valid || r.error_code != 0) return;
    const int lane = threadIdx.x & 63;
    uint32_t* s_buf = s_bufs[threadIdx.x >> 6];
    const uint32_t* dec32 = reinterpret_cast<const uint32_t*>(A.vout + (size_t)r.slot0 * kOutPerSlot);
    uint32_t* mp32 = reinterpret_cast<uint32_t*>(A.mpdu + (size_t)r.slot0 * kOutPerSlot);
    uint32_t* hp32 = A.mpdu_host ? reinterpret_cast<uint32_t*>(A.mpdu_host + (size_t)r.slot0 * kOutPerSlot) : nullptr;
    const uint32_t L = min((uint32_t)r.length, 2500u), nwords = (L + 3u) / 4u;
    constexpr int kPasses = (2500 / 4 + 63) / 64;
    uint32_t lo[kPasses], hi[kPasses];
#pragma unroll
    for (int k = 0; k < kPasses; k++) {
        const uint32_t w = (uint32_t)lane + 64u * (uint32_t)k, wc = min(w, nwords);
        lo[k] = dec32[wc]; hi[k] = dec32[wc + 1u];
    }
    const unsigned seed = (unsigned)__builtin_amdgcn_readfirstlane((int)lo[0]) >> 9;
    const unsigned phase = lds.phase[seed & 0x7F];
    uint8_t* bytes = reinterpret_cast<uint8_t*>(s_buf);
#pragma unroll
    for (int k = 0; k < kPasses; k++) {
        const uint32_t w = (uint32_t)lane + 64u * (uint32_t)k;
        if (w < nwords) {
            const uint32_t sb = phase == 255 ? 0u : lds.seq4[(phase + 32u * w) % 127u];
            const uint32_t o = __builtin_amdgcn_alignbyte(hi[k], lo[k], 2u) ^ sb;
            s_buf[w] = o;
            mp32[w] = o;
            if (hp32) hp32[w] = o;
        }
    }
    __builtin_amdgcn_fence(__ATOMIC_RELEASE, "wavefront");
    __builtin_amdgcn_wave_barrier();
    __builtin_amdgcn_fence(__ATOMIC_ACQUIRE, "wavefront");
    const int n = L >= 4 ? (int)L - 4 : 0;
    uint32_t crc;
    if (n >= 4) {
        crc = crc32_wave(bytes, n, s_crc, s_z, lane);
    } else {
        crc = 0xFFFFFFFFu;
        for (int i = 0; i < n; i++) crc = (crc >> 8) ^ s_crc[(bytes[i] ^ crc) & 0xFF];
    }
    if (lane == 0) {
        uint32_t fcs = 0;
        if (L >= 4) fcs = (uint32_t)bytes[L - 4] | ((uint32_t)bytes[L - 3] << 8) | ((uint32_t)bytes[L - 2] << 16) | ((uint32_t)bytes[L - 1] << 24);
        r.crc32 = fcs;
        r.error_code = ((~crc) == fcs) ? E_FRAME_OK : E_CRC32_FAIL;
    }
}

__global__ void __launch_bounds__(256) k_finish(RxArgs A)
{
    __shared__ FinishLds L;
    finish_tables_to_lds(A, L);
    __syncthreads();
    const JobRef jr = locate_job(blockIdx.x * 4 + (threadIdx.x >> 6), A.njobs);
    if (!jr.ok) return;
    finish_frame(A, A.joblist[jr.list * A.nrows + jr.idx], L);
}

struct PipeFallbackGate {
    WinProofGate proof; const RxArgs* A; FrameLds* lds; bool gave_up;
    __device__ __forceinline__ bool operator()(uint32_t list, uint32_t fa, uint32_t fb, bool hasB) const
    {
        if (!gave_up) return proof(list, fa, fb, hasB);
        frame_symbols<false>(*A, list * A->nrows + fa, *lds);
        if (hasB) frame_symbols<false>(*A, list * A->nrows + fb, *lds);
        __builtin_amdgcn_fence(__ATOMIC_RELEASE, "agent"); __builtin_amdgcn_fence(__ATOMIC_ACQUIRE, "agent");
        return true;
    }
};
template <bool PIPE>
__device__ __forceinline__ void win_redo_finish_body(const VitJob* jobs, const uint32_t* hdr, uint32_t jstride, uint32_t target, uint32_t vstride,
                                                     const uint16_t* vecs, const uint8_t* soft, uint8_t* out, unsigned long long* stats, const RxArgs& A, uint32_t* host_note)
{
    __shared__ FinishLds L;
    finish_tables_to_lds(A, L);
    auto after = [&](uint32_t list, uint32_t fa, uint32_t fb, bool hasB) {
        finish_frame(A, A.joblist[list * A.nrows + fa], L);
        if (hasB) finish_frame(A, A.joblist[list * A.nrows + fb], L);
    };
    const WinProofGate proof{ jobs, hdr, jstride, target, vstride, vecs, stats };
    if constexpr (PIPE) {
        __shared__ FrameLds F;
        reinterpret_cast<uint32_t*>(F.demap)[threadIdx.x] = reinterpret_cast<const uint32_t*>(A.T.demap)[threadIdx.x];
        __syncthreads();
        const bool gave_up = __builtin_amdgcn_readfirstlane((int)A.pipe_flags[0]) != 0;
        if (gave_up && blockIdx.x == 0 && threadIdx.x == 0) {
            if (stats) atomicAdd(&stats[4u * kWinStatBanks], 1ull);
            if (host_note) __hip_atomic_store(host_note, 1u, __ATOMIC_RELAXED, __HIP_MEMORY_SCOPE_SYSTEM);
        }
        viterbi_kernel_body<256, 24, 3>(jobs, hdr, 0u, jstride, soft, out, PipeFallbackGate{ proof, &A, &F, gave_up }, after);
    } else {
        __syncthreads();
        viterbi_kernel_body<256, 24, 3>(jobs, hdr, 0u, jstride, soft, out, proof, after);
    }
}
__global__ void __launch_bounds__(256) k_win_redo_finish(const VitJob* jobs, const uint32_t* hdr, uint32_t jstride, uint32_t target, uint32_t vstride,
                                                         const uint16_t* vecs, const uint8_t* soft, uint8_t* out, unsigned long long* stats, RxArgs A)
{ win_redo_finish_body<false>(jobs, hdr, jstride, target, vstride, vecs, soft, out, stats, A, nullptr); }
__global__ void __launch_bounds__(256) k_win_redo_finish_pipe(const VitJob* jobs, const uint32_t* hdr, uint32_t jstride, uint32_t target, uint32_t vstride,
                                                              const uint16_t* vecs, const uint8_t* soft, uint8_t* out, unsigned long long* stats, RxArgs A, uint32_t* host_note)
{ win_redo_finish_body<true>(jobs, hdr, jstride, target, vstride, vecs, soft, out, stats, A, host_note); }

struct PackedRow { uint32_t capture_id, start_sample, end_sample, error_code, rate_kbps; uint16_t length, nsym; uint32_t crc32; int16_t cfo_est;
    uint16_t flags; uint32_t mpdu_offset; };
__global__ void __launch_bounds__(1024) k_pack(const FrameRow* frames, const uint32_t* nframes, const CapDesc* caps, uint32_t ncaps, uint32_t max_frames,
                                               PackedRow* rows, uint32_t* nrows_out)
{
    __shared__ uint32_t s_scan[1024];
    __shared__ uint32_t s_base;
    const uint32_t t = threadIdx.x;
    if (t == 0) s_base = 0;
    __syncthreads();
    for (uint32_t c0 = 0; c0 < ncaps; c0 += 1024) {
        const uint32_t c = c0 + t;
        const uint32_t found = c < ncaps ? nframes[c] : 0u;
        const uint32_t n = min(found, max_frames);
        s_scan[t] = n;
        __syncthreads();
        for (uint32_t o = 1; o < 1024; o <<= 1) {
            const uint32_t v = t >= o ? s_scan[t - o] : 0u;
            __syncthreads();
            s_scan[t] += v;
            __syncthreads();
        }
        const uint32_t first = s_base + s_scan[t] - n;
        for (uint32_t i = 0; i < n; i++) {
            const FrameRow& r = frames[(size_t)c * max_frames + i];
            PackedRow o;
            o.capture_id = caps[c].capture_id; o.start_sample = r.start_sample; o.end_sample = r.end_sample; o.error_code = r.error_code;
            o.rate_kbps = r.rate_kbps; o.length = r.length; o.nsym = r.nsym; o.crc32 = r.crc32; o.cfo_est = r.cfo_est;
            o.flags = (i + 1 == n && found > max_frames) ? 1u : 0u;
            o.mpdu_offset = r.slot0 * (uint32_t)kOutPerSlot;
            rows[first + i] = o;
        }
        __syncthreads();
        if (t == 1023) s_base += s_scan[1023];
        __syncthreads();
    }
    if (t == 0) *nrows_out = s_base;
}


__global__ void __launch_bounds__(256) k_soft_pack3(const uint8_t* soft8, const uint32_t* off8, const uint32_t* nsoft, const uint16_t* flen, const uint32_t* out_off,
                                                    int code_rate, uint8_t* packed, VitJob* jobs)
{
    const uint32_t j = blockIdx.x, mine = nsoft[j], at = (off8[j] + 1u) / 2u;
    const uint8_t* in = soft8 + off8[j];
    for (uint32_t g = threadIdx.x; g < (mine + 7u) / 8u; g += blockDim.x) {
        uint32_t v[8];
#pragma unroll
        for (int k = 0; k < 8; k++) v[k] = 8u * g + k < mine ? in[8u * g + k] & 7u : 0u;
        const uint32_t bits24 = soft3_pack8(v), left = mine - 8u * g;
        if (left >= 8u) soft3_store8(packed + at, g, bits24);
        else for (uint32_t b = 0; b < (3u * left + 7u) / 8u; b++) packed[at + 3u * g + b] = (uint8_t)(bits24 >> (8u * b));
    }
    if (threadIdx.x == 0) {
        VitJob J; J.soft_off = at; J.nsoft = mine; J.length = flen[j]; J.dec_off = 0; J.out_off = out_off[j];
        J.valid = 1; J.code_rate = (uint32_t)code_rate; J.soft_bits = 3;
        jobs[j] = J;
    }
}

__global__ void __launch_bounds__(256) k_soft_jobs8(const uint32_t* off8, const uint32_t* nsoft, const uint16_t* flen, const uint32_t* out_off, int code_rate,
                                                    uint32_t n, VitJob* jobs)
{
    const uint32_t j = blockIdx.x * blockDim.x + threadIdx.x;
    if (j >= n) return;
    VitJob J; J.soft_off = off8[j]; J.nsoft = nsoft[j]; J.length = flen[j]; J.dec_off = 0; J.out_off = out_off[j];
    J.valid = 1; J.code_rate = (uint32_t)code_rate; J.soft_bits = 8;
    jobs[j] = J;
}

}
```

### sora_amd/csrc/k_vit16.hip

```cpp
#include <hip/hip_runtime.h>

#include "dev_vit16.h"

namespace sora {

namespace {

template <int CR, int WIN, int LOOK, int BITS>
__device__ __forceinline__ void forward16(Lds16<WIN, LOOK>& S, const uint8_t* __restrict__ soft, uint32_t my_soft_off, uint32_t my_nsoft,
                                          uint32_t nstepsA, uint32_t nstepsB, uint32_t my_tr_end, bool my_valid, uint8_t* my_out)
{
    using F16 = Forward16<CR, WIN, LOOK, BITS>;
    using Chunk = typename F16::Chunk;
    using Raw = typename F16::Raw;
    constexpr int GS = F16::GS;
    F16 F;
    F.init(S, soft, my_soft_off, 0, max(my_nsoft, 1u) - 1u, 0x18u * kFld, wave_max_u32(max(nstepsA, nstepsB)));

    uint32_t ob = 0;
    bool my_done = !my_valid;

    auto trace = [&](uint32_t my_cnt, int t24_last) {
        trace16<WIN, LOOK>((unsigned)(uintptr_t)&S, F.V.U[0], F.V.U[1], F.V.U[2], F.V.U[3], F.tr, ob, F16::pos_of(F.pos, t24_last / 8), (uint32_t)(t24_last % 8), my_cnt, my_out);
    };
    auto next_event = [&]() -> uint32_t {
        const uint32_t mine = my_done ? kNever : my_tr_end;
        return min(ob + (uint32_t)(WIN + LOOK + 6), wave_min_u32(mine));
    };
    F.next_thr = next_event();
    F.all_done = wave_min_u32(my_done ? 1u : 0u) != 0u;
    auto check = [&](int t24_last) {
        if (F.tr >= F.next_thr) {
            const bool partial = F.tr >= ob + (uint32_t)(WIN + LOOK + 6);
            uint32_t cnt = 0;
            if (!my_done) {
                if (F.tr >= my_tr_end) { cnt = my_tr_end - ob - 6; my_done = true; }
                else if (partial) cnt = WIN;
            }
            if (wave_max_u32(cnt) != 0u) trace(cnt, t24_last);
            if (partial) ob += WIN;
            F.next_thr = next_event();
            F.all_done = wave_min_u32(my_done ? 1u : 0u) != 0u;
        }
    };

    uint16_t* my_ops2[2] = { &S.ops2[0][F.row][F.my_j][F.half], &S.ops2[1][F.row][F.my_j][F.half] };
    const uint4* row_ops2[2] = { reinterpret_cast<const uint4*>(&S.ops2[0][F.row][0][0]), reinterpret_cast<const uint4*>(&S.ops2[1][F.row][0][0]) };
    auto stage = [&](const Raw& R, int t) { F.put(R, my_ops2[t]); };
    auto collect = [&](int t) -> Chunk { lds_fence(); return F16::get(row_ops2[t]); };
    auto fast_chunk_mid = [&](const Chunk& K, int h, Chunk& Knext, int tnext) {
#pragma unroll
        for (int g = 0; g < 12 / GS; g++) {
            if (g == (12 / GS) / 2) Knext = collect(tnext);
            F.group(K, h, g * GS);
        }
        F.tr += 12;
    };

    uint32_t c = 0;
    Raw b0 = F.fetch(0), b1 = F.fetch(1), b2, b3;
    while (F.going()) {
        const uint32_t lim = min(F.nsteps, F.next_thr - 1);
        uint32_t rows = lim > F.tr ? (lim - F.tr) / 24 : 0;
        if (rows >= 2) {
            Chunk Ka, Kb;
            b2 = F.fetch(c + 2);
            stage(b0, 0); Ka = collect(0); lds_fence();
            for (; rows >= 2; rows -= 2) {
                b3 = F.fetch(c + 3); stage(b1, 1); fast_chunk_mid(Ka, 0, Kb, 1);
                b0 = F.fetch(c + 4); stage(b2, 0); fast_chunk_mid(Kb, 1, Ka, 0);
                F.end_row();
                b1 = F.fetch(c + 5); stage(b3, 1); fast_chunk_mid(Ka, 0, Kb, 1);
                b2 = F.fetch(c + 6); stage(b0, 0); fast_chunk_mid(Kb, 1, Ka, 0);
                F.end_row();
                c += 4;
            }
            lds_fence();
        }
        if (!(F.tr < F.nsteps)) break;
        b2 = F.fetch(c + 2);
        if (rows) F.fast_chunk(F.unpack(b0), 0); else F.chunk(F.unpack(b0), 0, check);
        if (!F.going()) break;
        b3 = F.fetch(c + 3);
        if (rows) F.fast_chunk(F.unpack(b1), 1); else F.chunk(F.unpack(b1), 1, check);
        F.end_row();
        b0 = b2; b1 = b3;
        c += 2;
    }
}

template <int WIN, int LOOK, int BITS>
__device__ __forceinline__ void viterbi16_body(const VitJob* __restrict__ jobs, const uint32_t* __restrict__ njobs3, uint32_t njobs_single, uint32_t stride,
                                               const uint8_t* __restrict__ soft, uint8_t* __restrict__ out)
{
    __shared__ Lds16<WIN, LOOK> S;
    uint32_t n[3] = { njobs_single, 0, 0 };
    if (njobs3) { n[0] = njobs3[0]; n[1] = njobs3[1]; n[2] = njobs3[2]; }
    uint32_t w = uni(blockIdx.x), list = 0;
    while (list < 3 && w >= (n[list] + 7) / 8) { w -= (n[list] + 7) / 8; list++; }
    if (list >= 3) return;
    const uint32_t njobs = uni(n[list]);
    jobs += (size_t)list * stride;
    const unsigned lane = threadIdx.x & 63, row = lane >> 4, half = lane & 1u;
    const uint32_t fa = 8u * w + 2u * row, fb = fa + 1u;
    const bool hasA = fa < njobs, hasB = fb < njobs;
    const VitJob& GA = jobs[hasA ? fa : 8u * w];
    const VitJob& GBj = jobs[hasB ? fb : (hasA ? fa : 8u * w)];
    const uint32_t code_rate = uni(jobs[8u * w].code_rate);
    const uint32_t gsd = code_rate == 0 ? 2u : code_rate == 2 ? 4u : 3u, gss = code_rate == 0 ? 1u : code_rate == 2 ? 3u : 2u;
    const uint32_t nstepsA = hasA ? GA.nsoft / gsd * gss : 0u, nstepsB = hasB ? GBj.nsoft / gsd * gss : 0u;
    const VitJob& Mine = half ? GBj : GA;
    const bool my_valid = half ? hasB : hasA;
    const uint32_t my_tr_end = Mine.length * 8u + 16u + 6u;
    uint8_t* my_out = out + Mine.out_off;
    if (code_rate == 0)      forward16<0, WIN, LOOK, BITS>(S, soft, Mine.soft_off, Mine.nsoft, nstepsA, nstepsB, my_tr_end, my_valid, my_out);
    else if (code_rate == 1) forward16<1, WIN, LOOK, BITS>(S, soft, Mine.soft_off, Mine.nsoft, nstepsA, nstepsB, my_tr_end, my_valid, my_out);
    else                     forward16<2, WIN, LOOK, BITS>(S, soft, Mine.soft_off, Mine.nsoft, nstepsA, nstepsB, my_tr_end, my_valid, my_out);
}

}

__global__ void __launch_bounds__(64) k_viterbi16(const VitJob* __restrict__ jobs, const uint32_t* __restrict__ njobs3, uint32_t njobs_single, uint32_t stride,
        const uint8_t* __restrict__ soft, uint8_t* __restrict__ out)
{ viterbi16_body<256, 24, 3>(jobs, njobs3, njobs_single, stride, soft, out); }
__global__ void __launch_bounds__(64) k_viterbi16_11n(const VitJob* __restrict__ jobs, const uint32_t* __restrict__ njobs3, uint32_t njobs_single,
        uint32_t stride, const uint8_t* __restrict__ soft, uint8_t* __restrict__ out)
{ viterbi16_body<192, 36, 8>(jobs, njobs3, njobs_single, stride, soft, out); }

}
```

### sora_amd/csrc/k_vitwin.hip

```cpp
#include <hip/hip_runtime.h>
#include "dev_vitwin.h"

namespace sora {

__global__ void __launch_bounds__(64) k_viterbi16w(const VitJob* __restrict__ jobs, const uint32_t* __restrict__ hdr, uint32_t jstride, uint32_t target, uint32_t vstride,
                                                   const uint8_t* __restrict__ soft, uint8_t* __restrict__ out, uint16_t* __restrict__ vecs)
{ viterbi16w_body<256, 24, 3>(jobs, hdr, jstride, target, vstride, soft, out, vecs); }
__global__ void __launch_bounds__(64) k_viterbi16w_11n(const VitJob* __restrict__ jobs, const uint32_t* __restrict__ hdr, uint32_t jstride, uint32_t target, uint32_t vstride,
                                                       const uint8_t* __restrict__ soft, uint8_t* __restrict__ out, uint16_t* __restrict__ vecs)
{ viterbi16w_body<192, 36, 8>(jobs, hdr, jstride, target, vstride, soft, out, vecs); }


}
```

### sora_amd/csrc/kernels.h

```cpp
#pragma once
#include <hip/hip_runtime.h>
#include <vector>
#include "dev_arith.h"
#include "rx_types.h"
#include "../../include/sora_hip.h"

#if !defined(SORA_TOOLS) && (defined(SORA_SCAN_PROBE) || defined(SORA_DBG_PIPE_TIMELINE) || defined(SORA_DBG_PIPE_LOSE_FLAGS))
#error "SORA_SCAN_PROBE / SORA_DBG_* switches need -DSORA_TOOLS (sora_amd.build.build_variant)"
#endif

namespace sora {

struct ScanArgs {
    const uint32_t* iq;
    const CapDesc*  caps;
    uint32_t        ncaps;
    uint32_t        str;
    uint32_t        keep_queue;
    uint32_t        thr;
    uint32_t        max_frames;
    Tables          T;
    FrameRow*       frames;
    FrameCtx*       fctx;
    uint32_t*       nframes;
    uint32_t*       njobs;
    uint32_t*       joblist;
    uint32_t        nrows;
    uint32_t*       slot_row;
    uint32_t*       cont;
    uint32_t*       consumed;
    uint32_t*       zero_a; uint32_t nzero_a;
    uint32_t*       zero_b; uint32_t nzero_b;
    uint32_t        own_slots;
};
constexpr int kContWords = 64;

struct RxArgs {
    const uint32_t* iq;
    const CapDesc*  caps;
    uint32_t        str;
    uint32_t        total_slots;
    uint32_t        nrows;
    Tables          T;
    FrameRow*       frames;
    const FrameCtx* fctx;
    uint8_t*        soft;
    uint8_t*        vout;
    uint8_t*        mpdu;
    VitJob*         jobs;
    const uint32_t* njobs;
    const uint32_t* joblist;
    const uint32_t* slot_row;
    uint32_t*       eq;
    TrackRec*       track;
    uint32_t*       pil;
    const uint32_t* pipe_flags;
    uint8_t*        mpdu_host;
};

struct PipeArgs {
    uint32_t  nfront, ntrack;
    uint32_t* flags;
    uint32_t  target, vstride;
    uint16_t* vecs;
    uint32_t  stamp_base;
    uint32_t  lanes64;
    uint32_t  wait_ticks;
};

__global__ void k_scan(ScanArgs A);
__global__ void k_frame(RxArgs A);
__global__ void k_sym_front(RxArgs A);
__global__ void k_track_lds(RxArgs A);
__global__ void k_sym_back(RxArgs A);
__global__ void k_pipe(RxArgs A, PipeArgs P);
__global__ void k_viterbi(const VitJob* jobs, const uint32_t* njobs3, uint32_t njobs_single, uint32_t stride, const uint8_t* soft, uint8_t* out);
__global__ void k_viterbi11n(const VitJob* jobs, const uint32_t* njobs3, uint32_t njobs_single, uint32_t stride, const uint8_t* soft, uint8_t* out);
__global__ void k_viterbi16(const VitJob* jobs, const uint32_t* njobs3, uint32_t njobs_single, uint32_t stride, const uint8_t* soft, uint8_t* out);
__global__ void k_viterbi16_11n(const VitJob* jobs, const uint32_t* njobs3, uint32_t njobs_single, uint32_t stride, const uint8_t* soft, uint8_t* out);
__global__ void k_viterbi16w(const VitJob* jobs, const uint32_t* hdr, uint32_t jstride, uint32_t target, uint32_t vstride, const uint8_t* soft, uint8_t* out, uint16_t* vecs);
__global__ void k_viterbi16w_11n(const VitJob* jobs, const uint32_t* hdr, uint32_t jstride, uint32_t target, uint32_t vstride, const uint8_t* soft, uint8_t* out, uint16_t* vecs);
__global__ void k_win_redo_11n(const VitJob* jobs, const uint32_t* hdr, uint32_t jstride, uint32_t target, uint32_t vstride, const uint16_t* vecs,
        const uint8_t* soft, uint8_t* out, unsigned long long* stats);
__global__ void k_win_redo(const VitJob* jobs, const uint32_t* hdr, uint32_t jstride, uint32_t target, uint32_t vstride, const uint16_t* vecs,
        const uint8_t* soft, uint8_t* out, unsigned long long* stats);
__global__ void k_win_redo_finish(const VitJob* jobs, const uint32_t* hdr, uint32_t jstride, uint32_t target, uint32_t vstride, const uint16_t* vecs,
        const uint8_t* soft, uint8_t* out, unsigned long long* stats,
                                  RxArgs A);
__global__ void k_win_redo_finish_pipe(const VitJob* jobs, const uint32_t* hdr, uint32_t jstride, uint32_t target, uint32_t vstride, const uint16_t* vecs,
        const uint8_t* soft, uint8_t* out, unsigned long long* stats, RxArgs A, uint32_t* host_note);
__global__ void k_finish(RxArgs A);
struct PackedRow;
__global__ void k_pack(const FrameRow* frames, const uint32_t* nframes, const CapDesc* caps, uint32_t ncaps, uint32_t max_frames, PackedRow* rows, uint32_t* nrows_out);
__global__ void k_fft64_batch(const uint32_t* in, uint32_t* out, uint32_t n, Tables T);
template <int NB> __global__ void k_demap_batch(const uint32_t* in, uint8_t* soft, uint32_t n, Tables T);
template <int NB> __global__ void k_deint_batch(const uint8_t* in, uint8_t* out, uint32_t n, Tables T);
__global__ void k_lts_batch(const uint32_t* in, uint32_t* ctx, uint32_t n, Tables T);
__global__ void k_symfront_batch(const uint32_t* in, const uint32_t* ctx, const uint32_t* ctx_index, uint32_t* eq, uint32_t n, Tables T);
template <bool PHASE> __global__ void k_ptrack_batch(const uint32_t* eq, const uint32_t* first, const uint32_t* nsym, uint32_t* state, uint32_t* out, uint32_t nframes, Tables T);
template <int KIND> __global__ void k_cmul64_batch(const uint32_t* in, const uint32_t* coef, uint32_t cstride, uint32_t coff, const uint32_t* cindex, uint32_t* out, uint32_t n);
__global__ void k_fft128_batch(const uint32_t* in, uint32_t* out, uint32_t n, Tables T);
struct TxArgs {
    const uint8_t*  mpdu;
    const uint32_t* off;
    const uint32_t* len;
    const uint32_t* rate;
    const uint8_t*  seed;
    int8_t*         out8;
    const uint64_t* out_off;
    const int8_t*   preamble;
    Tables          T;
};
__global__ void k_tx_preamble(int8_t* out8, int8_t* out44, Tables T);
template <bool UP44> __global__ void k_tx11a(TxArgs A);

struct Tx11nArgs {
    const uint8_t*  mpdu;
    const uint32_t* off;
    const uint32_t* len;
    const uint32_t* mcs;
    const uint8_t*  seed;
    uint32_t*       out0;
    uint32_t*       out1;
    const uint64_t* out_off;
    const uint32_t* preamble;
    Tables          T;
};
struct Tx11nPlan { int nb, cr, ndbps; uint32_t nstd, nbytes, nvalid, nsym; };
__host__ __device__ inline bool tx11n_plan(uint32_t len, uint32_t mcs, Tx11nPlan& P)
{
    if (len < 1 || len > 4092) return false;
    switch (mcs) {
    case 8:  P.nb = 1; P.cr = 0; P.ndbps = 52;  break;  case 9:  P.nb = 2; P.cr = 0; P.ndbps = 104; break;
    case 10: P.nb = 2; P.cr = 2; P.ndbps = 156; break;  case 11: P.nb = 4; P.cr = 0; P.ndbps = 208; break;
    case 12: P.nb = 4; P.cr = 2; P.ndbps = 312; break;  case 13: P.nb = 6; P.cr = 1; P.ndbps = 416; break;
    case 14: P.nb = 6; P.cr = 2; P.ndbps = 468; break;
    default: return false;
    }
    const uint32_t nd = (uint32_t)P.ndbps, gin = (uint32_t)P.cr + 1, gout = (uint32_t)P.cr + 2;
    P.nstd = ((len + 4) * 8 + 16 + 6 + nd - 1) / nd;
    P.nbytes = (P.nstd * nd + 7) / 8;
    const uint32_t ngroups = (P.nbytes + gin - 1) / gin;
    P.nvalid = 8 * gin * ngroups;
    P.nsym = (gout * ngroups + 13 * (uint32_t)P.nb - 1) / (13 * (uint32_t)P.nb);
    return true;
}
constexpr uint32_t kTx11nPreamble = 1120;
__global__ void k_tx11n(Tx11nArgs A);

struct TxHt40Args {
    const uint8_t*  mpdu;
    const uint32_t* off;
    const uint32_t* len;
    const uint32_t* mcs;
    const uint8_t*  seed;
    uint32_t*       out0;
    uint32_t*       out1;
    const uint64_t* out_off;
    const uint32_t* preamble;
    Tables          T;
};
struct TxHt40Plan { int nb, cr, ndbps; uint32_t nsym; };
__host__ __device__ inline bool tx_ht40_plan(uint32_t len, uint32_t mcs, TxHt40Plan& P)
{
    if (len < 1 || len > 3996) return false;
    switch (mcs) {
    case 8:  P.nb = 1; P.cr = 0; P.ndbps = 54;  break;  case 9:  P.nb = 2; P.cr = 0; P.ndbps = 108; break;
// ... 107 lines not shown
```

### sora_amd/csrc/rx_types.h

```cpp
#pragma once
#include <stdint.h>

namespace sora {

struct CapDesc {
    uint64_t offset;
    uint32_t nsamples;
    uint32_t capture_id;
    uint32_t slot_base;
    uint32_t nslots;
};

struct FrameRow {
    uint32_t capture;
    uint32_t start_sample;
    uint32_t end_sample;
    uint32_t error_code;
    uint32_t rate_kbps;
    uint16_t length, nsym;
    uint16_t code_rate, nbpsc;
    uint32_t slot0;
    uint32_t crc32;
    int16_t  cfo_est;
    int16_t  cfo_comp, sfo_comp, cfo_tracker, sfo_tracker;
    uint16_t valid;
    uint32_t data_start;
    uint32_t pad[3];
};

struct FrameCtx {
    uint32_t freq[64];
    uint32_t chan[64];
};

struct VitJob {
    uint32_t soft_off;
    uint32_t nsoft;
    uint32_t length;
    uint32_t dec_off;
    uint32_t out_off;
    uint32_t valid;
    uint32_t code_rate;
    uint32_t soft_bits;
};

constexpr int kWinWarm = 144;
constexpr int kWinVecBytes = 256;
constexpr unsigned kWinStatBanks = 64;

struct TrackRec {
    int16_t cfo_comp, sfo_comp;
    int16_t avg, del;
};

struct JobRef { uint32_t list, idx; bool ok; };
__host__ __device__ inline JobRef locate_job(uint32_t g, const uint32_t* njobs)
{
    JobRef r; r.ok = true;
    const uint32_t n0 = njobs[0], n1 = njobs[1], n2 = njobs[2];
    if (g < n0) { r.list = 0; r.idx = g; }
    else if (g < n0 + n1) { r.list = 1; r.idx = g - n0; }
    else if (g < n0 + n1 + n2) { r.list = 2; r.idx = g - n0 - n1; }
    else { r.list = 0; r.idx = 0; r.ok = false; }
    return r;
}

constexpr int kSoftPerSlot = 288;
constexpr int kSoftBytesPerSlot = 108;
constexpr int kSoftSlack = 64;
constexpr int kOutPerSlot  = 32;

constexpr uint32_t E_FRAME_OK = 0x00000001u, E_PLCP_HEADER_FAIL = 0x80000005u, E_CRC32_FAIL = 0x80000006u,
                   E_CS_TIMEOUT = 0x80000007u,
                   E_INTERNAL_TIMEOUT = 0x8000F001u;

}
```

### sora_amd/csrc/sora_hip.cpp

```cpp
#include <hip/hip_runtime.h>
#include <cmath>
#include <cstdio>
#include <cstdlib>
#include <cstring>
#include <algorithm>
#include <atomic>
#include <chrono>
#include <mutex>
#include <string>
#include <vector>
#include "../../include/sora_hip.h"
#include "kernels.h"
#include "host_trellis.h"

using namespace sora;

static thread_local std::string g_last_error;
hipError_t sora_internal_stream_create(hipStream_t* out, int index)
{
    int least = 0, greatest = 0;
    (void)hipDeviceGetStreamPriorityRange(&least, &greatest);
    const int level = index % 3, prio = level == 0 ? 0 : level == 1 ? greatest : least;
    if (least != greatest) return hipStreamCreateWithPriority(out, hipStreamNonBlocking, prio);
    return hipStreamCreateWithFlags(out, hipStreamNonBlocking);
// ... 451 lines not shown
namespace { struct NamedTable { const char* name; const void* host; size_t bytes; const void* const* dev; }; }
static std::vector<NamedTable> named_tables(const HostTables& H, const std::vector<uint32_t>& sc, const std::vector<short>& at, const Tables* T,
        const uint32_t* const* dsc, const short* const* dat)
{
#define NT(n, v, d) { n, (v).data(), (v).size() * sizeof((v)[0]), (const void* const*)(d) }
    return { NT("usin", H.usin, T ? &T->usin : nullptr), NT("ucos", H.ucos, T ? &T->ucos : nullptr), NT("rot", H.rot, T ? &T->rot : nullptr), NT("uatan2",
            H.uatan2, T ? &T->uatan2 : nullptr),
             NT("demap", H.demap, T ? &T->demap : nullptr), NT("tw64", H.tw64, T ? &T->tw64 : nullptr), NT("tw16", H.tw16, T ? &T->tw16 : nullptr), NT("sts",
                     H.sts, T ? &T->sts : nullptr),
             NT("deint", H.deint, T ? &T->deint : nullptr), NT("crc", H.crc, T ? &T->crc : nullptr), NT("scr", H.scr, T ? &T->scr : nullptr), NT("scr_seq",
                     H.scr_seq, T ? &T->scr_seq : nullptr),
             NT("scr_phase", H.scr_phase, T ? &T->scr_phase : nullptr), NT("tw128", H.tw128, T ? &T->tw128 : nullptr), NT("tw32", H.tw32,
                     T ? &T->tw32 : nullptr), NT("tw8", H.tw8, T ? &T->tw8 : nullptr),
             NT("crcz", H.crcz, T ? &T->crcz : nullptr), NT("trk", H.trk, T ? &T->trk : nullptr), NT("dsp_sincos", sc, dsc), NT("dsp_atan", at, dat) };
#undef NT
}
int sora_hip_table_count(void) { return (int)(sizeof(kTablePins) / sizeof(kTablePins[0])); }
const char* sora_hip_table_name(int index) { return index >= 0 && index < sora_hip_table_count() ? kTablePins[index].name : nullptr; }
const char* sora_hip_table_pin(const char* name) { for (const TablePin& t : kTablePins) if (name && !strcmp(t.name, name)) return t.sha256; return nullptr; }
int sora_hip_table_digest(const char* name, char hex65[65])
{
    if (!name || !hex65) return fail(SORA_ERR_INVALID_PARAM, "sora_hip_table_digest: null argument");
    HostTables H; build_tables(H);
    std::vector<uint32_t> sc; std::vector<short> at; sora_internal_dsp_host_tables(sc, at);
    if (!strcmp(name, "trk") && !trk_tables_exact(H)) return fail(SORA_ERR_FAILED, "the tracker's folded tables (TrkTables) do not reproduce usin / ucos / uatan2");
    for (const NamedTable& t : named_tables(H, sc, at, nullptr, nullptr, nullptr)) if (!strcmp(t.name, name)) {
        const std::string d = table_digest(t.host, t.bytes);
        memcpy(hex65, d.c_str(), 65);
        return SORA_OK;
    }
    return fail(SORA_ERR_INVALID_PARAM, "sora_hip_table_digest: no such table");
}
int sora_hip_table_read(const char* name, void* h_out, size_t cap, size_t* bytes)
{
    if (!name || !bytes) return fail(SORA_ERR_INVALID_PARAM, "sora_hip_table_read: null argument");
    DevTables* D = stage_tables();
    if (!D) return fail(SORA_ERR_HARDWARE_FAILED, "sora_hip_table_read: no tables on this device");
    const uint32_t* dsc = nullptr; const short* dat = nullptr;
    if (!strncmp(name, "dsp_", 4) && sora_internal_dsp_tables(&dsc, &dat) != SORA_OK) return fail(SORA_ERR_HARDWARE_FAILED, "sora_hip_table_read: dsp_math tables");
    HostTables H; build_tables(H);
    std::vector<uint32_t> sc; std::vector<short> at; sora_internal_dsp_host_tables(sc, at);
    for (const NamedTable& t : named_tables(H, sc, at, &D->T, &dsc, &dat)) if (!strcmp(t.name, name)) {
        *bytes = t.bytes;
        if (!h_out) return SORA_OK;
        if (cap < t.bytes) return fail(SORA_ERR_CAPACITY, "sora_hip_table_read: buffer too small");
        HIPCHK(hipMemcpy(h_out, *t.dev, t.bytes, hipMemcpyDeviceToHost));
        return SORA_OK;
    }
    return fail(SORA_ERR_INVALID_PARAM, "sora_hip_table_read: no such table");
}

void* sora_hip_malloc(size_t bytes) { void* p = nullptr; if (hipMalloc(&p, bytes) != hipSuccess) return nullptr; return p; }
void  sora_hip_free(void* p) { if (p) (void)hipFree(p); }
int   sora_hip_memcpy_h2d(void* d, const void* h, size_t n) { HIPCHK(hipMemcpy(d, h, n, hipMemcpyHostToDevice)); return SORA_OK; }
int   sora_hip_stream_synchronize(void* stream) { HIPCHK(hipStreamSynchronize((hipStream_t)stream)); return SORA_OK; }
int   sora_hip_memcpy_d2h(void* h, const void* d, size_t n) { HIPCHK(hipMemcpy(h, d, n, hipMemcpyDeviceToHost)); return SORA_OK; }
int   sora_hip_memcpy_d2d(void* dd, const void* ds, size_t n, void* stream) { HIPCHK(hipMemcpyAsync(dd, ds, n, hipMemcpyDeviceToDevice, (hipStream_t)stream)); return SORA_OK; }
void* sora_hip_host_alloc(size_t bytes) { void* p = nullptr; if (hipHostMalloc(&p, bytes, hipHostMallocDefault) != hipSuccess) return nullptr; return p; }
void  sora_hip_host_free(void* p) { if (p) (void)hipHostFree(p); }

static int pipe_create(const sora_rx_cfg* cfg, RxPipe** out, int index = 0)
{
    if (!cfg || !out || cfg->struct_size != sizeof(sora_rx_cfg)) return fail(SORA_ERR_INVALID_PARAM, "sora_rx_create: bad cfg");
    if (cfg->sample_rate_mhz != 20 && cfg->sample_rate_mhz != 40 && cfg->sample_rate_mhz != 44) return fail(SORA_ERR_INVALID_PARAM, "sample_rate_mhz must be 20, 40 or 44");
    if (cfg->max_captures == 0 || cfg->max_total_samples == 0 || cfg->max_frames_per_capture == 0) return fail(SORA_ERR_INVALID_PARAM, "zero capacity");
    int ndev = 0;
    if (hipGetDeviceCount(&ndev) != hipSuccess || ndev <= 0) return fail(SORA_ERR_NO_DEVICE, "no HIP device: this library has no CPU path");
    if (cfg->device < 0 || cfg->device >= ndev) return fail(SORA_ERR_INVALID_PARAM, "device ordinal out of range");
    HIPCHK(hipSetDevice(cfg->device));
    RxPipe* rx = new RxPipe();
    rx->cfg = *cfg;
    if (rx->cfg.cca_pwr_threshold == 0) rx->cfg.cca_pwr_threshold = 1000 * 1000;
    rx->str = cfg->sample_rate_mhz == 20 ? 1 : 2;
    rx->tabs.device = cfg->device;
    int rc = make_dev_tables(rx->tabs);
    if (rc) { rx_free(rx); return rc; }
    hipError_t e = sora_internal_stream_create(&rx->stream, index);
    if (e != hipSuccess) { rx_free(rx); return fail(SORA_ERR_HARDWARE_FAILED, "hipStreamCreate", e); }
    e = hipHostMalloc((void**)&rx->h_caps_pinned, sizeof(CapDesc) * cfg->max_captures, hipHostMallocDefault);
    if (e == hipSuccess) e = hipEventCreateWithFlags(&rx->ev_caps, hipEventDisableTiming);
    if (e != hipSuccess) { rx_free(rx); return fail(SORA_ERR_HARDWARE_FAILED, "pinned descriptor buffer", e); }
    const uint64_t n20 = cfg->max_total_samples / rx->str;
    const uint64_t want_slots = n20 / 80 + cfg->max_captures + 16, want_rows = (uint64_t)cfg->max_captures * cfg->max_frames_per_capture;
    if (want_slots * (1ull * kSoftPerSlot) >= (1ull << 32) || want_rows >= (1ull << 31) / 3 || cfg->max_total_samples >= (1ull << 32)) {
        rx_free(rx);
        return fail(SORA_ERR_CAPACITY, "sora_rx_create: max_total_samples / max_captures x max_frames_per_capture exceed the 32-bit slot geometry of one handle "
                                       "(split the batch over several handles)");
    }
    rx->cap_slots = (uint32_t)want_slots;
    rx->cap_rows = (uint32_t)want_rows;
    struct { void** p; size_t bytes; } allocs[] = {
        { (void**)&rx->d_caps, sizeof(CapDesc) * cfg->max_captures },
        { (void**)&rx->d_fctx, sizeof(FrameCtx) * ((size_t)rx->cap_rows + cfg->max_captures) }, { (void**)&rx->d_nframes, 4 * (size_t)cfg->max_captures },
        { (void**)&rx->d_vout, (size_t)kOutPerSlot * rx->cap_slots }, { (void**)&rx->d_mpdu, (size_t)kOutPerSlot * rx->cap_slots },
        { (void**)&rx->d_rows, sizeof(sora_frame_result) * rx->cap_rows },
        { (void**)&rx->d_nrows, 4 }, { (void**)&rx->d_joblist, 3 * 4 * (size_t)rx->cap_rows },
        { (void**)&rx->d_njobs, 64 + sizeof(FrameRow) * rx->cap_rows },
    };
    for (auto& a : allocs) {
        e = hipMalloc(a.p, a.bytes);
        if (e != hipSuccess) { rx_free(rx); return fail(SORA_ERR_HARDWARE_FAILED, "hipMalloc (receive-path arrays)", e); }
    }
    rx->d_frames = reinterpret_cast<FrameRow*>(reinterpret_cast<uint8_t*>(rx->d_njobs) + 64);
    *out = rx;
    return SORA_OK;
}

static void pipe_destroy(RxPipe* rx) { if (rx) { (void)hipSetDevice(rx->cfg.device); (void)hipStreamSynchronize(rx->stream); rx_free(rx); } }

static int pipe_reset(RxPipe* rx)
{
    if (!rx) return SORA_ERR_INVALID_PARAM;
    HIPCHK(hipSetDevice(rx->cfg.device));
    HIPCHK(hipStreamSynchronize(rx->stream));
    rx->ncaps = 0; rx->total_slots = 0; rx->have_results = false; rx->h_caps.clear(); rx->ticket = 0; rx->delivered = rx->released = false;
    return SORA_OK;
}

static int pipe_flush(RxPipe* rx)
{
    if (!rx) return SORA_ERR_INVALID_PARAM;
    HIPCHK(hipSetDevice(rx->cfg.device));
    HIPCHK(hipStreamSynchronize(rx->stream));
    return SORA_OK;
}

static void* pipe_stream(RxPipe* rx) { return rx ? (void*)rx->stream : nullptr; }

static int pipe_process_dev(RxPipe* rx, const sora_complex16* d_iq, const sora_capture_desc* caps, size_t ncaps, uint64_t iq_samples = 0)
{
    if (!rx || (!d_iq && ncaps) || (!caps && ncaps)) return fail(SORA_ERR_INVALID_PARAM, "sora_rx_process_dev: null argument");
    if (ncaps > rx->cfg.max_captures) return fail(SORA_ERR_CAPACITY, "more captures than sora_rx_cfg.max_captures");
    HIPCHK(hipSetDevice(rx->cfg.device));
    std::vector<CapDesc> hc(ncaps);
    uint64_t total = 0, slots64 = 0;
    for (size_t i = 0; i < ncaps; i++) {
        if (caps[i].offset & 3) return fail(SORA_ERR_INVALID_PARAM, "capture offset must be a multiple of 4 samples (16-byte alignment, memsource.hpp:59)");
        CapDesc& c = hc[i];
        c.offset = caps[i].offset; c.nsamples = caps[i].nsamples; c.capture_id = caps[i].capture_id;
        c.slot_base = (uint32_t)slots64; c.nslots = (caps[i].nsamples / rx->str) / 80 + 1;
        slots64 += c.nslots; total += caps[i].nsamples;
        if (iq_samples && (caps[i].offset > iq_samples || caps[i].nsamples > iq_samples - caps[i].offset))
            return fail(SORA_ERR_INVALID_PARAM, "a capture descriptor reaches past the end of the sample buffer");
    }
    if (total > rx->cfg.max_total_samples || slots64 > rx->cap_slots) return fail(SORA_ERR_CAPACITY, "more samples than sora_rx_cfg.max_total_samples");
    if (rx->bound_mpdu && rx->bound_bytes < (size_t)kOutPerSlot * slots64) {
        rx->bound_mpdu = nullptr;
        return fail(SORA_ERR_CAPACITY, "sora_rx_bind_mpdu: the bound array is smaller than the call's sora_rx_mpdu_bytes()");
    }
    const uint32_t slots = (uint32_t)slots64;
    rx->h_caps.swap(hc);
    rx->ncaps = (uint32_t)ncaps; rx->total_slots = slots; rx->have_results = false; rx->delivered = rx->released = false;
    if (ncaps == 0) { rx->have_results = true; return SORA_OK; }
    if (!rx->d_soft) {
        HIPCHK(hipMalloc((void**)&rx->d_soft, (size_t)kSoftBytesPerSlot * rx->cap_slots + kSoftSlack));
        HIPCHK(hipMalloc((void**)&rx->d_jobs, 3 * sizeof(VitJob) * rx->cap_rows));
    }
    const bool windowed = rx->trellis == Trellis::Windowed;
    if (windowed) { const int rc = rx->win.ensure(rx->cap_rows, nullptr, true); if (rc) return rc; }
    const bool split = rx->front >= 3;
    const bool pipe = split && rx->front == 4 && windowed;
    if (pipe && !rx->d_pflags) {
        rx->pflag_words = (4u + 4u * rx->cap_rows + (rx->cap_slots + 63u) / 64u + 4u + 3u) / 4u * 4u;
        HIPCHK(hipMalloc((void**)&rx->d_pflags, 4 * ((size_t)rx->pflag_words + 1024)));
    }
    if (split && !rx->d_slot_row) {
        HIPCHK(hipMalloc((void**)&rx->d_slot_row, 4 * ((size_t)rx->cap_slots + 64)));
        HIPCHK(hipMalloc((void**)&rx->d_eq, 256 * ((size_t)rx->cap_slots + 64)));
        HIPCHK(hipMalloc((void**)&rx->d_track, sizeof(TrackRec) * ((size_t)rx->cap_slots + 64)));
        HIPCHK(hipMalloc((void**)&rx->d_pil, 16 * ((size_t)rx->cap_slots + 64)));
    }
    hipStream_t st = rx->stream;
    const bool prof = rx->profiling;
    if (prof) { const int rc = fold_profile(rx); if (rc) return rc; }
    int evi = 0;
    auto mark = [&]() { if (prof) (void)hipEventRecord(rx->ev[evi++], st); };
    mark();
    bool caps_changed = false;
    if (rx->caps_resident != ncaps || memcmp(rx->h_caps_pinned, rx->h_caps.data(), sizeof(CapDesc) * ncaps) != 0) {
        if (rx->caps_resident) HIPCHK(hipEventSynchronize(rx->ev_caps));
        memcpy(rx->h_caps_pinned, rx->h_caps.data(), sizeof(CapDesc) * ncaps);
        HIPCHK(hipMemcpyAsync(rx->d_caps, rx->h_caps_pinned, sizeof(CapDesc) * ncaps, hipMemcpyHostToDevice, st));
        HIPCHK(hipEventRecord(rx->ev_caps, st));
        rx->caps_resident = ncaps;
        caps_changed = true;
    }
    const uint32_t nrows = rx->ncaps * rx->cfg.max_frames_per_capture;

    auto enqueue = [&](bool recording) -> int {
#ifdef SORA_TOOLS
        const bool self_clean = false;
#else
        const bool self_clean = !recording;
#endif
        const bool fill = !self_clean || !rx->counters_ready;
        const uint32_t par = fill ? 0u : rx->parity;
        uint32_t* const counters = rx->d_njobs + 8u * par;
        const uint32_t pipe_words = pipe ? 4u + 4u * nrows + (slots + 63u) / 64u : 0u;
        if (fill && RX_ONLY(rx, 1u)) {
            const uint32_t n16 = (uint32_t)((64 + sizeof(FrameRow) * (size_t)nrows) / 16), m16 = split ? (slots + 3) / 4 : 0u;
            const uint32_t k16 = (pipe_words + 3u) / 4u;
            hipLaunchKernelGGL(k_clear16, dim3((n16 + m16 + k16 + 255) / 256), dim3(256), 0, st, reinterpret_cast<uint4*>(rx->d_njobs), n16,
                               reinterpret_cast<uint4*>(rx->d_slot_row), m16, reinterpret_cast<uint4*>(rx->d_pflags), k16);
        }
        ScanArgs S{};
        S.iq = reinterpret_cast<const uint32_t*>(d_iq); S.caps = rx->d_caps; S.ncaps = rx->ncaps; S.str = rx->str;
        S.keep_queue = rx->cfg.sample_rate_mhz == 44 ? 1u : 0u; S.thr = rx->cfg.cca_pwr_threshold;
        S.max_frames = rx->cfg.max_frames_per_capture; S.T = rx->tabs.T; S.frames = rx->d_frames; S.fctx = rx->d_fctx; S.nframes = rx->d_nframes;
        S.njobs = counters; S.joblist = rx->d_joblist; S.nrows = nrows; S.slot_row = split ? rx->d_slot_row : nullptr; S.cont = rx->cont; S.consumed = rx->consumed;
        if (self_clean) {
            S.zero_a = rx->d_njobs + 8u * (1u - par); S.nzero_a = 4; S.zero_b = pipe ? rx->d_pflags : nullptr; S.nzero_b = pipe_words; S.own_slots = 1;
        }
        rx->parity = self_clean ? 1u - par : 0u; rx->counters_ready = self_clean;
        mark();
        if (RX_ONLY(rx, 1u)) hipLaunchKernelGGL(k_scan, dim3(rx->ncaps), dim3(64), 0, st, S);
        mark();

        RxArgs R{};
        R.iq = S.iq; R.caps = rx->d_caps; R.str = rx->str; R.total_slots = slots; R.nrows = nrows; R.T = rx->tabs.T;
        R.frames = rx->d_frames; R.fctx = rx->d_fctx;
        R.vout = rx->d_vout; R.mpdu = rx->d_mpdu; R.njobs = counters; R.joblist = rx->d_joblist; R.mpdu_host = rx->bound_mpdu;
        R.soft = rx->d_soft; R.jobs = rx->d_jobs; R.slot_row = rx->d_slot_row; R.eq = rx->d_eq; R.track = rx->d_track; R.pil = rx->d_pil;
        R.pipe_flags = pipe ? rx->d_pflags : nullptr;
        const bool redo_finish = windowed && RX_ONLY(rx, 4u) && RX_ONLY(rx, 8u);
        const TrellisJobs J = trellis_lists(rx->d_jobs, counters, nrows, nrows);
        const uint32_t pair_groups = trellis_pair_groups(J);

        if (pipe) {
            if (RX_ONLY(rx, 2u)) {
                PipeArgs P{};
                P.nfront = (slots + 63) / 64; P.ntrack = nrows; P.flags = rx->d_pflags; P.target = kWinUnitsTarget; P.vstride = rx->win.stride;
                P.vecs = rx->win.d_vecs; P.stamp_base = rx->pflag_words;
                P.lanes64 = rx->pipe64 ? 1u : 0u; P.wait_ticks = rx->pipe_wait_ticks;
                const uint32_t waves = rx->pipe64 ? kWinMaxUnits * ((nrows + 3) / 2) : trellis_win_waves(J);
                hipLaunchKernelGGL(k_pipe, dim3(P.nfront + P.ntrack + (waves + 3) / 4), dim3(256), 0, st, R, P);
            }
            mark();
            if (RX_ONLY(rx, 4u) && !redo_finish) trellis_proof<256>(J, rx->d_soft, rx->d_vout, rx->win, st);
// ... 997 lines not shown
    }
    if (flags & SORA_INGEST_DECIMATE2) n = n / 8 * 4;
    return (size_t)n;
}

int sora_hip_ingest(const void* d_raw, size_t raw_bytes, unsigned flags, sora_complex16* d_out, size_t out_capacity, size_t* n_out, void* stream)
{
    if (sora_hip_device_count() <= 0) return fail(SORA_ERR_NO_DEVICE, "no HIP device: this library has no CPU path");
    if (!d_raw || !d_out || (flags & ~15u)) return fail(SORA_ERR_INVALID_PARAM, "sora_hip_ingest: bad argument");
    if (((uintptr_t)d_raw & 3) || ((uintptr_t)d_out & 3)) return fail(SORA_ERR_INVALID_PARAM, "sora_hip_ingest: buffers must be 4-byte aligned");
    const size_t n = sora_hip_ingest_count(raw_bytes, flags);
    if (n_out) *n_out = n;
    if (n > out_capacity) return fail(SORA_ERR_CAPACITY, "sora_hip_ingest: output buffer too small");
    if (n == 0) return SORA_OK;
    uint64_t done = 0;
    if ((flags & (SORA_INGEST_RXBLOCK | SORA_INGEST_44TO40)) == (SORA_INGEST_RXBLOCK | SORA_INGEST_44TO40) &&
        !((uintptr_t)d_raw & 15) && !((uintptr_t)d_out & 15)) {
        const uint64_t per_tile = (flags & SORA_INGEST_DECIMATE2) ? 700 : 1400;
        const uint64_t tiles = std::min<uint64_t>(raw_bytes / (55 * 128), n / per_tile);
        if (tiles) {
            hipLaunchKernelGGL(k_ingest_tile, dim3((unsigned)std::min<uint64_t>(tiles, 8 * 256)), dim3(256), 0, (hipStream_t)stream, (const uint8_t*)d_raw,
                    reinterpret_cast<uint32_t*>(d_out), flags, (uint32_t)tiles);
            done = tiles * per_tile;
        }
    }
    if (done < n)
        hipLaunchKernelGGL(k_ingest, dim3((unsigned)((n - done + 255) / 256)), dim3(256), 0, (hipStream_t)stream, (const uint8_t*)d_raw,
                reinterpret_cast<uint32_t*>(d_out), done, (uint64_t)n, flags);
    HIPCHK(hipGetLastError());
    return SORA_OK;
}

constexpr size_t kVitWsHdr = 0, kVitWsStats = 256, kVitWsHead = kVitWsStats + kWinStatsBytes;
static size_t vit_ws_round(size_t b) { return (b + 255) & ~(size_t)255; }
static size_t vit_ws_packed_bytes(size_t soft_span_bytes) { return vit_ws_round(soft_span_bytes / 2 + 4 + kSoftSlack); }
static size_t vit_ws_bytes8(size_t soft_span_bytes) { return vit_ws_round(soft_span_bytes + kSoftSlack); }
static size_t vit_ws_tail(size_t n) { return vit_ws_round(sizeof(VitJob) * n) + (size_t)kWinVecBytes * win_vstride(n); }
size_t sora_hip_viterbi11a_workspace_bytes(size_t soft_span_bytes, size_t n)
{
    return kVitWsHead + vit_ws_packed_bytes(soft_span_bytes) + vit_ws_tail(n);
}
size_t sora_hip_viterbi11n_workspace_bytes(size_t soft_span_bytes, size_t n)
{
    return kVitWsHead + vit_ws_bytes8(soft_span_bytes) + vit_ws_tail(n);
}

extern "C++" {
template <int WIN>
static int viterbi_ws(const char* name, const uint8_t* d_soft, size_t soft_span_bytes, const uint32_t* d_soft_off, const uint32_t* d_nsoft,
                      const uint16_t* d_frame_len, int code_rate, uint8_t* d_out, const uint32_t* d_out_off, size_t n, void* d_workspace, size_t workspace_bytes,
                      int lanes_per_pair, void* stream)
{
    const std::string nm(name);
    if (sora_hip_device_count() <= 0) return fail(SORA_ERR_NO_DEVICE, "no HIP device: this library has no CPU path");
    if (!d_soft || !d_soft_off || !d_nsoft || !d_frame_len || !d_out || !d_out_off || code_rate < 0 || code_rate > 2) return fail(SORA_ERR_INVALID_PARAM,
            (nm + ": bad argument").c_str());
    if (n == 0) return SORA_OK;
    TrellisChoice choice;
    if (!trellis_parse(lanes_per_pair, &choice)) return fail(SORA_ERR_INVALID_PARAM, (nm + ": lanes_per_pair is 0 (default: 64), 16, 64 or SORA_TRELLIS_WINDOWED").c_str());
    if (!d_workspace || ((uintptr_t)d_workspace & 15)) return fail(SORA_ERR_INVALID_PARAM, (nm + ": the workspace must be a 16-byte aligned device buffer").c_str());
    const size_t need = WIN == 256 ? sora_hip_viterbi11a_workspace_bytes(soft_span_bytes, n) : sora_hip_viterbi11n_workspace_bytes(soft_span_bytes, n);
    if (workspace_bytes < need) return fail(SORA_ERR_CAPACITY, (nm + ": workspace smaller than its _workspace_bytes()").c_str());
    if (soft_span_bytes >= (1ull << 32) || n >= (1ull << 31)) return fail(SORA_ERR_CAPACITY, (nm + ": batch too large").c_str());
    hipStream_t st = (hipStream_t)stream;
    uint8_t* ws = (uint8_t*)d_workspace;
    uint32_t* hdr = (uint32_t*)(ws + kVitWsHdr);
    unsigned long long* stats = (unsigned long long*)(ws + kVitWsStats);
    uint8_t* soft = ws + kVitWsHead;
    VitJob* jobs = (VitJob*)(soft + (WIN == 256 ? vit_ws_packed_bytes(soft_span_bytes) : vit_ws_bytes8(soft_span_bytes)));
    uint16_t* vecs = (uint16_t*)((uint8_t*)jobs + vit_ws_round(sizeof(VitJob) * n));
    if (WIN == 256)
        hipLaunchKernelGGL(k_soft_pack3, dim3((unsigned)n), dim3(256), 0, st, d_soft, d_soft_off, d_nsoft, d_frame_len, d_out_off, code_rate, soft, jobs);
    else {
        HIPCHK(hipMemcpyAsync(soft, d_soft, soft_span_bytes, hipMemcpyDeviceToDevice, st));
        hipLaunchKernelGGL(k_soft_jobs8, dim3((unsigned)((n + 255) / 256)), dim3(256), 0, st, d_soft_off, d_nsoft, d_frame_len, d_out_off, code_rate, (uint32_t)n, jobs);
    }
    const Trellis kind = choice.value_or(Trellis::Lanes64);
    const WinScratch W{ vecs, stats, win_vstride(n) };
    if (kind == Trellis::Windowed) {
        HIPCHK(hipMemsetD32Async((hipDeviceptr_t)hdr, 0, 4, st));
        HIPCHK(hipMemsetD32Async((hipDeviceptr_t)hdr, (int)n, 1, st));
        HIPCHK(hipMemsetAsync(stats, 0, kWinStatsBytes, st));
    }
    trellis_launch<WIN>(kind, trellis_single(jobs, hdr, (uint32_t)n), soft, d_out, st, W);
    HIPCHK(hipGetLastError());
    return SORA_OK;
}
}

int sora_hip_viterbi11a_ws(const uint8_t* d_soft, size_t soft_span_bytes, const uint32_t* d_soft_off, const uint32_t* d_nsoft, const uint16_t* d_frame_len,
                           int code_rate, uint8_t* d_out, const uint32_t* d_out_off, size_t n, void* d_workspace, size_t workspace_bytes, int lanes_per_pair, void* stream)
{
    return viterbi_ws<256>("sora_hip_viterbi11a_ws", d_soft, soft_span_bytes, d_soft_off, d_nsoft, d_frame_len, code_rate, d_out, d_out_off, n, d_workspace,
                           workspace_bytes, lanes_per_pair, stream);
}
int sora_hip_viterbi11n_ws(const uint8_t* d_soft, size_t soft_span_bytes, const uint32_t* d_soft_off, const uint32_t* d_nsoft, const uint16_t* d_frame_len,
                           int code_rate, uint8_t* d_out, const uint32_t* d_out_off, size_t n, void* d_workspace, size_t workspace_bytes, int lanes_per_pair, void* stream)
{
    return viterbi_ws<192>("sora_hip_viterbi11n_ws", d_soft, soft_span_bytes, d_soft_off, d_nsoft, d_frame_len, code_rate, d_out, d_out_off, n, d_workspace,
                           workspace_bytes, lanes_per_pair, stream);
}

int sora_hip_viterbi_window_stats(const void* d_workspace, unsigned long long out[4], void* stream)
{
    if (!d_workspace || !out) return fail(SORA_ERR_INVALID_PARAM, "sora_hip_viterbi_window_stats: null argument");
    hipStream_t st = (hipStream_t)stream;
    for (int i = 0; i < 4; i++) out[i] = 0;
    return win_stats_add((const unsigned long long*)((const uint8_t*)d_workspace + kVitWsStats), st, out);
}

namespace {
struct VitWs { void* p = nullptr; size_t bytes = 0; };
std::mutex g_vitws_mutex;
VitWs g_vitws[64];
}

int sora_hip_viterbi11a(const uint8_t* d_soft, const uint32_t* d_soft_off, const uint32_t* d_nsoft, const uint16_t* d_frame_len,
                        int code_rate, uint8_t* d_out, const uint32_t* d_out_off, size_t n, void* stream)
{
    if (sora_hip_device_count() <= 0) return fail(SORA_ERR_NO_DEVICE, "no HIP device: this library has no CPU path");
    if (!d_soft || !d_soft_off || !d_nsoft || !d_frame_len || !d_out || !d_out_off || code_rate < 0 || code_rate > 2) return fail(SORA_ERR_INVALID_PARAM,
            "sora_hip_viterbi11a: bad argument");
    if (n == 0) return SORA_OK;
    hipStream_t st = (hipStream_t)stream;
    std::vector<uint32_t> h_off(n), h_nsoft(n);
    HIPCHK(hipMemcpyAsync(h_off.data(), d_soft_off, 4 * n, hipMemcpyDeviceToHost, st));
    HIPCHK(hipMemcpyAsync(h_nsoft.data(), d_nsoft, 4 * n, hipMemcpyDeviceToHost, st));
    HIPCHK(hipStreamSynchronize(st));
    uint64_t span = 0;
    for (size_t i = 0; i < n; i++) {
        if (h_nsoft[i] < 24) return fail(SORA_ERR_INVALID_PARAM, "sora_hip_viterbi11a: a job needs at least one OFDM symbol of soft values");
        span = std::max<uint64_t>(span, (uint64_t)h_off[i] + h_nsoft[i]);
    }
    if (span >> 32) return fail(SORA_ERR_CAPACITY, "sora_hip_viterbi11a: batch too large");
    int dev = 0; HIPCHK(hipGetDevice(&dev));
    if (dev < 0 || dev >= 64) return fail(SORA_ERR_INVALID_PARAM, "sora_hip_viterbi11a: device ordinal out of range");
    const size_t need = sora_hip_viterbi11a_workspace_bytes((size_t)span, n);
    std::lock_guard<std::mutex> lock(g_vitws_mutex);
    VitWs& W = g_vitws[dev];
    if (W.bytes < need) {
        if (W.p) { HIPCHK(hipDeviceSynchronize()); (void)hipFree(W.p); W.p = nullptr; W.bytes = 0; }
        HIPCHK(hipMalloc(&W.p, need + need / 4));
        W.bytes = need + need / 4;
    }
    const int rc = sora_hip_viterbi11a_ws(d_soft, (size_t)span, d_soft_off, d_nsoft, d_frame_len, code_rate, d_out, d_out_off, n, W.p, W.bytes, 0, stream);
    if (rc != SORA_OK) return rc;
    HIPCHK(hipStreamSynchronize(st));
    return SORA_OK;
}

}
```

Baseline: 53490.

## Store RX soft bits as one byte per value instead of 3-bit packed

Changes the main RX soft-bit stream from 3-bit packing (108 bytes per slot) to one byte per soft value (288 bytes per slot). The demap table is pre-shifted into the byte position the trellis ops expect, so the Viterbi kernels can load bytes directly, with a new fast fetch_at path that skips the unpack and clamping. Deinterleave stores become plain 8-byte writes, and the old packed kernels are kept as _p3 variants for the standalone decoder API. In exchange, soft-bit memory traffic and footprint grow by about 2.7x, plus a padded, zeroed allocation and extra LDS clearing.

After: 56080, median of 6. +4.8%, better.

```diff
diff --git a/sora_amd/csrc/dev_sym11a.h b/sora_amd/csrc/dev_sym11a.h
--- a/sora_amd/csrc/dev_sym11a.h
+++ b/sora_amd/csrc/dev_sym11a.h
@@ -9,7 +9,7 @@
 {
     VitJob J;
     J.valid = 1; J.soft_off = r.slot0 * (uint32_t)kSoftBytesPerSlot; J.nsoft = (uint32_t)r.nsym * 48u * r.nbpsc; J.length = r.length;
-    J.dec_off = 0; J.out_off = r.slot0 * (uint32_t)kOutPerSlot; J.code_rate = r.code_rate; J.soft_bits = 3;
+    J.dec_off = 0; J.out_off = r.slot0 * (uint32_t)kOutPerSlot; J.code_rate = r.code_rate; J.soft_bits = (uint32_t)kSoftScaled;
     return J;
 }
 
@@ -109,6 +109,11 @@
     }
 }
 
+__device__ __forceinline__ void demap_table_to_lds(const Tables& T, uint8_t* s_demap)
+{
+    reinterpret_cast<uint32_t*>(s_demap)[threadIdx.x] = (reinterpret_cast<const uint32_t*>(T.demap)[threadIdx.x] << 1) & 0xFEFEFEFEu;
+}
+
 __device__ __forceinline__ bool deint_packs(int nb, int lane) { return 8 * lane < 48 * nb; }
 __device__ __forceinline__ void deint_map_words(const Tables& T, int nb, int lane, uint32_t mp[4])
 {
@@ -117,12 +122,13 @@
 #pragma unroll
     for (int t = 0; t < 4; t++) mp[t] = packs ? (uint32_t)map[8 * lane + 2 * t] | ((uint32_t)map[8 * lane + 2 * t + 1] << 16) : 0u;
 }
-__device__ __forceinline__ uint32_t deint_gather24(const uint8_t* src, const uint32_t mp[4])
+__device__ __forceinline__ uint2 deint_gather8(const uint8_t* src, const uint32_t mp[4])
 {
     uint32_t v[8];
 #pragma unroll
     for (int t = 0; t < 4; t++) { v[2 * t] = src[mp[t] & 0xFFFFu]; v[2 * t + 1] = src[mp[t] >> 16]; }
-    return soft3_pack8(v);
+    return uint2{ v[0] | (v[1] << 8) | (v[2] << 16) | (v[3] << 24), v[4] | (v[5] << 8) | (v[6] << 16) | (v[7] << 24) };
 }
+__device__ __forceinline__ void soft8_store(uint8_t* sym, uint32_t lane, uint2 b) { reinterpret_cast<uint2*>(sym)[lane] = b; }
 
 }
diff --git a/sora_amd/csrc/dev_vit16.h b/sora_amd/csrc/dev_vit16.h
--- a/sora_amd/csrc/dev_vit16.h
+++ b/sora_amd/csrc/dev_vit16.h
@@ -114,6 +114,7 @@
     unsigned row, half;
     uint32_t my_j;
     SoftCursor<BITS, CW> cur[NV];
+    uint32_t my_base;
     const uint8_t* soft;
     uint16_t* my_ops;
     const uint4* row_ops;
@@ -151,10 +152,12 @@
         my_j = l16 >> 1;
 #pragma unroll
         for (int v = 0; v < NV; v++) cur[v].init(my_soft_off, my_first + my_j + 8u * v, my_last);
+        my_base = my_soft_off + my_first + my_j;
         soft = soft_;
         my_ops = &S.ops[row][my_j][half];
         row_ops = reinterpret_cast<const uint4*>(&S.ops[row][0][0]);
         set_row_pos();
+        clear_ops(S);
     }
     __device__ __forceinline__ bool going() const { return tr < nsteps && !all_done; }
 
@@ -180,7 +183,25 @@
     __device__ __forceinline__ void put(const Raw& R, uint16_t* mine) const
     {
 #pragma unroll
-        for (int v = 0; v < NV; v++) mine[16 * v] = (uint16_t)cur[v].field(R.r[v]);
+        for (int v = 0; v < NV; v++) soft_put(mine + 16 * v, cur[v], R.r[v]);
+    }
+    __device__ __forceinline__ void clear_ops(Lds16<WIN, LOOK>& S) const
+    {
+        if constexpr (BITS == kSoftScaled) {
+            static_assert(sizeof(S.ops2) == 3 * 64 * 4, "three dwords per lane");
+            uint32_t* z = reinterpret_cast<uint32_t*>(&S.ops2[0][0][0][0]) + (threadIdx.x & 63);
+            z[0] = 0u; z[64] = 0u; z[128] = 0u;
+            lds_fence();
+        }
+    }
+    __device__ __forceinline__ uint32_t fast_base(uint32_t c0) const { return my_base + c0 * (uint32_t)CW; }
+    template <int DC> __device__ __forceinline__ Raw fetch_at(uint32_t p) const
+    {
+        static_assert(BITS == kSoftScaled, "one byte per value");
+        Raw R;
+#pragma unroll
+        for (int v = 0; v < NV; v++) { R.r[v].sh = 0; R.r[v].w = soft[(size_t)p + (size_t)(DC * CW + 8 * v)]; }
+        return R;
     }
     static __device__ __forceinline__ Chunk get(const uint4* table)
     {
diff --git a/sora_amd/csrc/dev_viterbi.h b/sora_amd/csrc/dev_viterbi.h
--- a/sora_amd/csrc/dev_viterbi.h
+++ b/sora_amd/csrc/dev_viterbi.h
@@ -87,6 +87,22 @@
         return kConst ? (r.w << lsh) & 0x0E00u : ((r.w >> r.sh) & 7u) << 9;
     }
 };
+
+template <int CW> struct SoftCursor<kSoftScaled, CW> {
+    uint32_t off, lim;
+    __device__ __forceinline__ void init(uint32_t stream_off, uint32_t k, uint32_t last) { off = stream_off + min(k, last); lim = stream_off + last; }
+    __device__ __forceinline__ SoftRaw fetch(const uint8_t* __restrict__ base, uint32_t c) const
+    {
+        SoftRaw r; r.sh = 0; r.w = base[min(off + c * (uint32_t)CW, lim)];
+        return r;
+    }
+};
+template <int BITS, int CW>
+__device__ __forceinline__ void soft_put(uint16_t* slot, const SoftCursor<BITS, CW>& cur, const SoftRaw& r)
+{
+    if constexpr (BITS == kSoftScaled) reinterpret_cast<uint8_t*>(slot)[1] = (uint8_t)r.w;
+    else *slot = (uint16_t)cur.field(r);
+}
 
 constexpr unsigned kFld = (1u << 9) | (1u << 25);
 constexpr unsigned kOne = 0x00020001u;
@@ -243,6 +259,7 @@
         tr = 0; ob = ob0;
         cur.init(M.soft_off, my_k + M.i0, M.last);
         soft_base = soft_base_; ops = ops_;
+        if (BITS == kSoftScaled) { ops[lane] = 0; lds_fence(); }
         my_op = ops + 2u * my_k + (lane >> 5);
     }
     __device__ __forceinline__ bool going() const { return tr < nsteps && !(A.done && B.done); }
@@ -251,7 +268,7 @@
     __device__ __forceinline__ SoftRaw fetch(uint32_t c) const { return cur.fetch(soft_base, c); }
     __device__ __forceinline__ Chunk unpack(const SoftRaw& R)
     {
-        *my_op = (uint16_t)cur.field(R);
+        soft_put(my_op, cur, R);
         lds_fence();
         Chunk K;
 #pragma unroll
diff --git a/sora_amd/csrc/dev_vitwin.h b/sora_amd/csrc/dev_vitwin.h
--- a/sora_amd/csrc/dev_vitwin.h
+++ b/sora_amd/csrc/dev_vitwin.h
@@ -118,7 +118,7 @@
                 if (F.tr >= my_tr_end) { cnt = my_tr_end - my_ob - 6; my_done = true; }
                 else if (F.tr >= my_ob + THR) { cnt = WIN; partial = true; }
             }
-            if (wave_max_u32(cnt) != 0u) trace(cnt, t24_last);
+            if (wave_max_u32(cnt) != 0u) { trace(cnt, t24_last); F.clear_ops(S); }
             if (partial) { my_ob += WIN; if (--my_wleft == 0) my_done = true; }
             F.next_thr = next_event();
             F.all_done = wave_min_u32(my_done ? 1u : 0u) != 0u;
diff --git a/sora_amd/csrc/host_trellis.h b/sora_amd/csrc/host_trellis.h
--- a/sora_amd/csrc/host_trellis.h
+++ b/sora_amd/csrc/host_trellis.h
@@ -27,9 +27,9 @@
 inline uint64_t win_waves(uint64_t rows) { return (win_units(rows) + 7) / 8 + 3 + kWinLoneWaves; }
 inline uint32_t win_vstride(uint64_t rows) { return (uint32_t)(win_units(rows) + rows); }
 
-struct TrellisJobs { const VitJob* jobs; const uint32_t* hdr; uint32_t n, stride; bool single; };
-inline TrellisJobs trellis_lists(const VitJob* jobs, const uint32_t* hdr, uint32_t n, uint32_t stride) { return TrellisJobs{ jobs, hdr, n, stride, false }; }
-inline TrellisJobs trellis_single(const VitJob* jobs, const uint32_t* hdr, uint32_t n) { return TrellisJobs{ jobs, hdr, n, n, true }; }
+struct TrellisJobs { const VitJob* jobs; const uint32_t* hdr; uint32_t n, stride; bool single, packed3; };
+inline TrellisJobs trellis_lists(const VitJob* jobs, const uint32_t* hdr, uint32_t n, uint32_t stride) { return TrellisJobs{ jobs, hdr, n, stride, false, false }; }
+inline TrellisJobs trellis_single(const VitJob* jobs, const uint32_t* hdr, uint32_t n, bool packed3) { return TrellisJobs{ jobs, hdr, n, n, true, packed3 }; }
 inline uint32_t trellis_pair_groups(const TrellisJobs& J) { return J.single ? (J.n + 7) / 8 : (J.n / 2 + 3 + 3) / 4; }
 inline uint32_t trellis_waves16(const TrellisJobs& J) { return (J.n + 7) / 8 + (J.single ? 0u : 2u); }
 inline uint32_t trellis_win_waves(const TrellisJobs& J)
@@ -75,7 +75,8 @@
 {
     static_assert(WIN == 256 || WIN == 192, "the 802.11a (256) or the 802.11n (192) window schedule");
     if constexpr (WIN == 256)
-        hipLaunchKernelGGL(k_win_redo, dim3(trellis_pair_groups(J)), dim3(256), 0, st, J.jobs, J.hdr, J.stride, kWinUnitsTarget, W.stride, (const uint16_t*)W.d_vecs, soft, out, W.d_stats);
+        hipLaunchKernelGGL(J.packed3 ? k_win_redo_p3 : k_win_redo, dim3(trellis_pair_groups(J)), dim3(256), 0, st, J.jobs, J.hdr, J.stride, kWinUnitsTarget, W.stride,
+                           (const uint16_t*)W.d_vecs, soft, out, W.d_stats);
     else
         hipLaunchKernelGGL(k_win_redo_11n, dim3(trellis_pair_groups(J)), dim3(256), 0, st, J.jobs, J.hdr, J.stride, kWinUnitsTarget, W.stride, (const uint16_t*)W.d_vecs, soft, out, W.d_stats);
 }
@@ -86,14 +87,16 @@
     const uint32_t* hdr = J.single ? nullptr : J.hdr;
     const uint32_t n1 = J.single ? J.n : 0u, stride = J.single ? 0u : J.stride;
     if (kind == Trellis::Windowed) {
-        if constexpr (WIN == 256) hipLaunchKernelGGL(k_viterbi16w, dim3(trellis_win_waves(J)), dim3(64), 0, st, J.jobs, J.hdr, J.stride, kWinUnitsTarget, W.stride, soft, out, W.d_vecs);
+        if constexpr (WIN == 256)
+            hipLaunchKernelGGL(J.packed3 ? k_viterbi16w_p3 : k_viterbi16w, dim3(trellis_win_waves(J)), dim3(64), 0, st, J.jobs, J.hdr, J.stride, kWinUnitsTarget, W.stride, soft, out,
+                               W.d_vecs);
         else hipLaunchKernelGGL(k_viterbi16w_11n, dim3(trellis_win_waves(J)), dim3(64), 0, st, J.jobs, J.hdr, J.stride, kWinUnitsTarget, W.stride, soft, out, W.d_vecs);
         if (proof) trellis_proof<WIN>(J, soft, out, W, st);
     } else if (kind == Trellis::Lanes16) {
-        if constexpr (WIN == 256) hipLaunchKernelGGL(k_viterbi16, dim3(trellis_waves16(J)), dim3(64), 0, st, J.jobs, hdr, n1, stride, soft, out);
+        if constexpr (WIN == 256) hipLaunchKernelGGL(J.packed3 ? k_viterbi16_p3 : k_viterbi16, dim3(trellis_waves16(J)), dim3(64), 0, st, J.jobs, hdr, n1, stride, soft, out);
         else hipLaunchKernelGGL(k_viterbi16_11n, dim3(trellis_waves16(J)), dim3(64), 0, st, J.jobs, hdr, n1, stride, soft, out);
     } else {
-        if constexpr (WIN == 256) hipLaunchKernelGGL(k_viterbi, dim3(trellis_pair_groups(J)), dim3(256), 0, st, J.jobs, hdr, n1, stride, soft, out);
+        if constexpr (WIN == 256) hipLaunchKernelGGL(J.packed3 ? k_viterbi_p3 : k_viterbi, dim3(trellis_pair_groups(J)), dim3(256), 0, st, J.jobs, hdr, n1, stride, soft, out);
         else hipLaunchKernelGGL(k_viterbi11n, dim3(trellis_pair_groups(J)), dim3(256), 0, st, J.jobs, hdr, n1, stride, soft, out);
     }
 }
diff --git a/sora_amd/csrc/k_rx.hip b/sora_amd/csrc/k_rx.hip
--- a/sora_amd/csrc/k_rx.hip
+++ b/sora_amd/csrc/k_rx.hip
@@ -121,10 +121,10 @@
         wave_lds_sync();
         {
             const int nact = min(4, nsym - s0 + 1);
-            const uint32_t sym_bytes = 3u * (uint32_t)ncbps / 8u;
+            const uint32_t sym_bytes = (uint32_t)ncbps;
             uint8_t* d = dst + (size_t)(s0 - 1) * sym_bytes;
             for (int gs = 0; gs < nact; gs++, d += sym_bytes)
-                if (packs) soft3_store8(d, (uint32_t)lane, deint_gather24(s_soft[w][gs], mp));
+                if (packs) soft8_store(d, (uint32_t)lane, deint_gather8(s_soft[w][gs], mp));
         }
         wave_lds_sync();
     }
@@ -132,7 +132,7 @@
 __global__ void __launch_bounds__(256) k_frame(RxArgs A)
 {
     __shared__ FrameLds lds;
-    reinterpret_cast<uint32_t*>(lds.demap)[threadIdx.x] = reinterpret_cast<const uint32_t*>(A.T.demap)[threadIdx.x];
+    demap_table_to_lds(A.T, lds.demap);
     __syncthreads();
     if (!locate_job(blockIdx.x * 4, A.njobs).ok) return;
     const JobRef jr = locate_job(blockIdx.x * 4 + (threadIdx.x >> 6), A.njobs);
@@ -324,7 +324,7 @@
     __shared__ uint8_t s_demap[1024];
     const int w = threadIdx.x >> 6, lane = threadIdx.x & 63, g = lane >> 4, e = lane & 15;
     const Tables& T = A.T;
-    reinterpret_cast<uint32_t*>(s_demap)[threadIdx.x] = reinterpret_cast<const uint32_t*>(T.demap)[threadIdx.x];
+    demap_table_to_lds(T, s_demap);
     __syncthreads();
     const WaveSlots S = wave_slots(A, blockIdx.x);
     if (S.owned == 0) return;
@@ -334,7 +334,7 @@
     if (S.one_frame) {
         const FrameRow& r = A.frames[S.row0];
         const int nb = __builtin_amdgcn_readfirstlane((int)r.nbpsc), ncbps = 48 * nb;
-        const uint32_t slot0 = (uint32_t)__builtin_amdgcn_readfirstlane((int)r.slot0), sym_bytes = 3u * (uint32_t)ncbps / 8u;
+        const uint32_t slot0 = (uint32_t)__builtin_amdgcn_readfirstlane((int)r.slot0), sym_bytes = (uint32_t)ncbps;
         uint8_t* stream = A.soft + (size_t)slot0 * kSoftBytesPerSlot;
         const bool packs = deint_packs(nb, lane);
         uint32_t mp[4];
@@ -358,7 +358,7 @@
             for (int gs = 0; gs < 4; gs++) {
                 if (!((quad >> gs) & 1u) || !packs) continue;
                 const uint32_t sg = S.slot(it, gs);
-                soft3_store8(stream + (size_t)(sg - slot0 - 1u) * sym_bytes, (uint32_t)lane, deint_gather24(s_soft[w][gs], mp));
+                soft8_store(stream + (size_t)(sg - slot0 - 1u) * sym_bytes, (uint32_t)lane, deint_gather8(s_soft[w][gs], mp));
             }
             wave_lds_sync();
         }
@@ -390,8 +390,8 @@
             if (nbg != cur_nb) { cur_nb = nbg; deint_map_words(T, nbg, lane, mp); }
             if (deint_packs(nbg, lane)) {
                 const uint32_t sg = S.slot(it, gs);
-                uint8_t* d = A.soft + (size_t)slot0g * kSoftBytesPerSlot + (size_t)(sg - slot0g - 1u) * (3u * 48u * (uint32_t)nbg / 8u);
-                soft3_store8(d, (uint32_t)lane, deint_gather24(s_soft[w][gs], mp));
+                uint8_t* d = A.soft + (size_t)slot0g * kSoftBytesPerSlot + (size_t)(sg - slot0g - 1u) * (48u * (uint32_t)nbg);
+                soft8_store(d, (uint32_t)lane, deint_gather8(s_soft[w][gs], mp));
             }
         }
         wave_lds_sync();
@@ -430,7 +430,7 @@
     const JobRef jr = locate_job(t, A.njobs);
     if (!jr.ok) return;
     track_tables_to_lds(A.T.trk, L.t, L.pol);
-    reinterpret_cast<uint32_t*>(L.demap)[threadIdx.x] = reinterpret_cast<const uint32_t*>(A.T.demap)[threadIdx.x];
+    demap_table_to_lds(A.T, L.demap);
     const uint32_t j = jr.list * A.nrows + jr.idx, f = A.joblist[j];
     const FrameRow r = A.frames[f];
     const uint32_t nsym = min((uint32_t)r.nsym, kPipeMaxSym - 8u), slot0 = r.slot0;
@@ -490,7 +490,7 @@
     __builtin_amdgcn_fence(__ATOMIC_ACQUIRE, "agent");
     const int h = w - 1, g = lane >> 4, e = lane & 15;
     const int nb = __builtin_amdgcn_readfirstlane((int)r.nbpsc), ncbps = 48 * nb;
-    const uint32_t sym_bytes = 3u * (uint32_t)ncbps / 8u;
+    const uint32_t sym_bytes = (uint32_t)ncbps;
     uint8_t* stream = A.soft + (size_t)slot0 * kSoftBytesPerSlot;
     const bool packs = deint_packs(nb, lane);
     uint32_t mp[4];
@@ -513,16 +513,16 @@
         const uint2 rw = L.rec[(s - 1u) & (kPipeRing - 1u)];
         if (mine) sym_back_demap(A.T, L.demap, v3, int4{ (int16_t)rw.x, (int16_t)(rw.x >> 16), (int16_t)rw.y, (int16_t)(rw.y >> 16) }, nb, e, L.soft[h][g]);
         wave_lds_sync();
-        uint32_t b24[4];
-#pragma unroll
-        for (int gs = 0; gs < 4; gs++) b24[gs] = deint_gather24(L.soft[h][gs], mp);
+        uint2 b8[4];
+#pragma unroll
+        for (int gs = 0; gs < 4; gs++) b8[gs] = deint_gather8(L.soft[h][gs], mp);
         wave_lds_sync();
         if (packs) {
 #pragma unroll
-            for (int gs = 0; gs < 4; gs++) soft3_store8(bytes + (uint32_t)gs * sym_bytes, (uint32_t)lane, b24[gs]);
+            for (int gs = 0; gs < 4; gs++) soft8_store(bytes + (uint32_t)gs * sym_bytes, (uint32_t)lane, b8[gs]);
         }
         wave_lds_sync();
-        const uint32_t ndw = (nact * sym_bytes + 3u) / 4u;
+        const uint32_t ndw = nact * sym_bytes / 4u;
         uint32_t* out32 = reinterpret_cast<uint32_t*>(stream + (size_t)(4u * k) * sym_bytes);
         for (uint32_t i = (uint32_t)lane; i < ndw; i += 64u) store4_through(out32 + i, reinterpret_cast<const uint32_t*>(bytes)[i]);
         asm volatile("s_waitcnt vmcnt(0)" ::: "memory");
@@ -568,7 +568,7 @@
         const unsigned lane = threadIdx.x & 63;
         return pipe_units_ready(A, P, list, (lane & 1u) ? GB_ : GA, (lane & 15u) < 2u, wave_index);
     };
-    viterbi16w_wave<256, 24, 3>(S, wave_index, jobs_of, ready, A.njobs, P.target, P.vstride, (const uint8_t*)A.soft, A.vout, P.vecs);
+    viterbi16w_wave<256, 24, kSoftScaled>(S, wave_index, jobs_of, ready, A.njobs, P.target, P.vstride, (const uint8_t*)A.soft, A.vout, P.vecs);
     PIPE_STAMP(P, 17 + 2 * wave_index);
 }
 
@@ -649,7 +649,7 @@
         if (GB_.valid && (!GA.valid || GB_.ob != GA.ob)) { if (!GA.valid) { GA = GB_; } const bool no = false; GB_.valid = no; }
         if (!GA.valid) return;
         const unsigned lane = threadIdx.x & 63;
-        viterbi_forward_unit<CR, 256, 24, 3>(GA, GB_, (const uint8_t*)A.soft, L.ring, L.ops, P.vecs,
+        viterbi_forward_unit<CR, 256, 24, kSoftScaled>(GA, GB_, (const uint8_t*)A.soft, L.ring, L.ops, P.vecs,
                                              [&]() { return pipe_units_ready(A, P, list, lane >= 32u ? GB_ : GA, (lane & 31u) == 0u, wave_index); });
     };
     if (code_rate == 0) run(std::integral_constant<int, 0>{});
@@ -720,6 +720,9 @@
 
 __global__ void __launch_bounds__(256) k_viterbi(const VitJob* __restrict__ jobs, const uint32_t* __restrict__ njobs3, uint32_t njobs_single, uint32_t stride,
         const uint8_t* __restrict__ soft, uint8_t* __restrict__ out)
+{ viterbi_kernel_body<256, 24, kSoftScaled>(jobs, njobs3, njobs_single, stride, soft, out); }
+__global__ void __launch_bounds__(256) k_viterbi_p3(const VitJob* __restrict__ jobs, const uint32_t* __restrict__ njobs3, uint32_t njobs_single, uint32_t stride,
+        const uint8_t* __restrict__ soft, uint8_t* __restrict__ out)
 { viterbi_kernel_body<256, 24, 3>(jobs, njobs3, njobs_single, stride, soft, out); }
 __global__ void __launch_bounds__(256) k_viterbi11n(const VitJob* __restrict__ jobs, const uint32_t* __restrict__ njobs3, uint32_t njobs_single,
         uint32_t stride, const uint8_t* __restrict__ soft, uint8_t* __restrict__ out)
@@ -762,6 +765,10 @@
 __global__ void __launch_bounds__(256) k_win_redo(const VitJob* __restrict__ jobs, const uint32_t* __restrict__ hdr, uint32_t jstride, uint32_t target,
         uint32_t vstride, const uint16_t* __restrict__ vecs,
                                                   const uint8_t* __restrict__ soft, uint8_t* __restrict__ out, unsigned long long* __restrict__ stats)
+{ viterbi_kernel_body<256, 24, kSoftScaled>(jobs, hdr, 0u, jstride, soft, out, WinProofGate{ jobs, hdr, jstride, target, vstride, vecs, stats }); }
+__global__ void __launch_bounds__(256) k_win_redo_p3(const VitJob* __restrict__ jobs, const uint32_t* __restrict__ hdr, uint32_t jstride, uint32_t target,
+        uint32_t vstride, const uint16_t* __restrict__ vecs,
+                                                     const uint8_t* __restrict__ soft, uint8_t* __restrict__ out, unsigned long long* __restrict__ stats)
 { viterbi_kernel_body<256, 24, 3>(jobs, hdr, 0u, jstride, soft, out, WinProofGate{ jobs, hdr, jstride, target, vstride, vecs, stats }); }
 __global__ void __launch_bounds__(256) k_win_redo_11n(const VitJob* __restrict__ jobs, const uint32_t* __restrict__ hdr, uint32_t jstride, uint32_t target,
         uint32_t vstride, const uint16_t* __restrict__ vecs,
@@ -868,17 +875,17 @@
     const WinProofGate proof{ jobs, hdr, jstride, target, vstride, vecs, stats };
     if constexpr (PIPE) {
         __shared__ FrameLds F;
-        reinterpret_cast<uint32_t*>(F.demap)[threadIdx.x] = reinterpret_cast<const uint32_t*>(A.T.demap)[threadIdx.x];
+        demap_table_to_lds(A.T, F.demap);
         __syncthreads();
         const bool gave_up = __builtin_amdgcn_readfirstlane((int)A.pipe_flags[0]) != 0;
         if (gave_up && blockIdx.x == 0 && threadIdx.x == 0) {
             if (stats) atomicAdd(&stats[4u * kWinStatBanks], 1ull);
             if (host_note) __hip_atomic_store(host_note, 1u, __ATOMIC_RELAXED, __HIP_MEMORY_SCOPE_SYSTEM);
         }
-        viterbi_kernel_body<256, 24, 3>(jobs, hdr, 0u, jstride, soft, out, PipeFallbackGate{ proof, &A, &F, gave_up }, after);
+        viterbi_kernel_body<256, 24, kSoftScaled>(jobs, hdr, 0u, jstride, soft, out, PipeFallbackGate{ proof, &A, &F, gave_up }, after);
     } else {
         __syncthreads();
-        viterbi_kernel_body<256, 24, 3>(jobs, hdr, 0u, jstride, soft, out, proof, after);
+        viterbi_kernel_body<256, 24, kSoftScaled>(jobs, hdr, 0u, jstride, soft, out, proof, after);
     }
 }
 __global__ void __launch_bounds__(256) k_win_redo_finish(const VitJob* jobs, const uint32_t* hdr, uint32_t jstride, uint32_t target, uint32_t vstride,
diff --git a/sora_amd/csrc/k_vit16.hip b/sora_amd/csrc/k_vit16.hip
--- a/sora_amd/csrc/k_vit16.hip
+++ b/sora_amd/csrc/k_vit16.hip
@@ -37,7 +37,7 @@
                 if (F.tr >= my_tr_end) { cnt = my_tr_end - ob - 6; my_done = true; }
                 else if (partial) cnt = WIN;
             }
-            if (wave_max_u32(cnt) != 0u) trace(cnt, t24_last);
+            if (wave_max_u32(cnt) != 0u) { trace(cnt, t24_last); F.clear_ops(S); }
             if (partial) ob += WIN;
             F.next_thr = next_event();
             F.all_done = wave_min_u32(my_done ? 1u : 0u) != 0u;
@@ -66,14 +66,27 @@
             Chunk Ka, Kb;
             b2 = F.fetch(c + 2);
             stage(b0, 0); Ka = collect(0); lds_fence();
-            for (; rows >= 2; rows -= 2) {
-                b3 = F.fetch(c + 3); stage(b1, 1); fast_chunk_mid(Ka, 0, Kb, 1);
-                b0 = F.fetch(c + 4); stage(b2, 0); fast_chunk_mid(Kb, 1, Ka, 0);
-                F.end_row();
-                b1 = F.fetch(c + 5); stage(b3, 1); fast_chunk_mid(Ka, 0, Kb, 1);
-                b2 = F.fetch(c + 6); stage(b0, 0); fast_chunk_mid(Kb, 1, Ka, 0);
-                F.end_row();
-                c += 4;
+            if constexpr (BITS == kSoftScaled) {
+                uint32_t p = F.fast_base(c);
+                for (; rows >= 2; rows -= 2) {
+                    b3 = F.template fetch_at<3>(p); stage(b1, 1); fast_chunk_mid(Ka, 0, Kb, 1);
+                    b0 = F.template fetch_at<4>(p); stage(b2, 0); fast_chunk_mid(Kb, 1, Ka, 0);
+                    F.end_row();
+                    b1 = F.template fetch_at<5>(p); stage(b3, 1); fast_chunk_mid(Ka, 0, Kb, 1);
+                    b2 = F.template fetch_at<6>(p); stage(b0, 0); fast_chunk_mid(Kb, 1, Ka, 0);
+                    F.end_row();
+                    c += 4; p += 4u * (uint32_t)F16::CW;
+                }
+            } else {
+                for (; rows >= 2; rows -= 2) {
+                    b3 = F.fetch(c + 3); stage(b1, 1); fast_chunk_mid(Ka, 0, Kb, 1);
+                    b0 = F.fetch(c + 4); stage(b2, 0); fast_chunk_mid(Kb, 1, Ka, 0);
+                    F.end_row();
+                    b1 = F.fetch(c + 5); stage(b3, 1); fast_chunk_mid(Ka, 0, Kb, 1);
+                    b2 = F.fetch(c + 6); stage(b0, 0); fast_chunk_mid(Kb, 1, Ka, 0);
+                    F.end_row();
+                    c += 4;
+                }
             }
             lds_fence();
         }
@@ -122,6 +135,9 @@
 
 __global__ void __launch_bounds__(64) k_viterbi16(const VitJob* __restrict__ jobs, const uint32_t* __restrict__ njobs3, uint32_t njobs_single, uint32_t stride,
         const uint8_t* __restrict__ soft, uint8_t* __restrict__ out)
+{ viterbi16_body<256, 24, kSoftScaled>(jobs, njobs3, njobs_single, stride, soft, out); }
+__global__ void __launch_bounds__(64) k_viterbi16_p3(const VitJob* __restrict__ jobs, const uint32_t* __restrict__ njobs3, uint32_t njobs_single, uint32_t stride,
+        const uint8_t* __restrict__ soft, uint8_t* __restrict__ out)
 { viterbi16_body<256, 24, 3>(jobs, njobs3, njobs_single, stride, soft, out); }
 __global__ void __launch_bounds__(64) k_viterbi16_11n(const VitJob* __restrict__ jobs, const uint32_t* __restrict__ njobs3, uint32_t njobs_single,
         uint32_t stride, const uint8_t* __restrict__ soft, uint8_t* __restrict__ out)
diff --git a/sora_amd/csrc/k_vitwin.hip b/sora_amd/csrc/k_vitwin.hip
--- a/sora_amd/csrc/k_vitwin.hip
+++ b/sora_amd/csrc/k_vitwin.hip
@@ -5,6 +5,9 @@
 
 __global__ void __launch_bounds__(64) k_viterbi16w(const VitJob* __restrict__ jobs, const uint32_t* __restrict__ hdr, uint32_t jstride, uint32_t target, uint32_t vstride,
                                                    const uint8_t* __restrict__ soft, uint8_t* __restrict__ out, uint16_t* __restrict__ vecs)
+{ viterbi16w_body<256, 24, kSoftScaled>(jobs, hdr, jstride, target, vstride, soft, out, vecs); }
+__global__ void __launch_bounds__(64) k_viterbi16w_p3(const VitJob* __restrict__ jobs, const uint32_t* __restrict__ hdr, uint32_t jstride, uint32_t target, uint32_t vstride,
+                                                      const uint8_t* __restrict__ soft, uint8_t* __restrict__ out, uint16_t* __restrict__ vecs)
 { viterbi16w_body<256, 24, 3>(jobs, hdr, jstride, target, vstride, soft, out, vecs); }
 __global__ void __launch_bounds__(64) k_viterbi16w_11n(const VitJob* __restrict__ jobs, const uint32_t* __restrict__ hdr, uint32_t jstride, uint32_t target, uint32_t vstride,
                                                        const uint8_t* __restrict__ soft, uint8_t* __restrict__ out, uint16_t* __restrict__ vecs)
diff --git a/sora_amd/csrc/kernels.h b/sora_amd/csrc/kernels.h
--- a/sora_amd/csrc/kernels.h
+++ b/sora_amd/csrc/kernels.h
@@ -75,14 +75,19 @@
 __global__ void k_sym_back(RxArgs A);
 __global__ void k_pipe(RxArgs A, PipeArgs P);
 __global__ void k_viterbi(const VitJob* jobs, const uint32_t* njobs3, uint32_t njobs_single, uint32_t stride, const uint8_t* soft, uint8_t* out);
+__global__ void k_viterbi_p3(const VitJob* jobs, const uint32_t* njobs3, uint32_t njobs_single, uint32_t stride, const uint8_t* soft, uint8_t* out);
 __global__ void k_viterbi11n(const VitJob* jobs, const uint32_t* njobs3, uint32_t njobs_single, uint32_t stride, const uint8_t* soft, uint8_t* out);
 __global__ void k_viterbi16(const VitJob* jobs, const uint32_t* njobs3, uint32_t njobs_single, uint32_t stride, const uint8_t* soft, uint8_t* out);
+__global__ void k_viterbi16_p3(const VitJob* jobs, const uint32_t* njobs3, uint32_t njobs_single, uint32_t stride, const uint8_t* soft, uint8_t* out);
 __global__ void k_viterbi16_11n(const VitJob* jobs, const uint32_t* njobs3, uint32_t njobs_single, uint32_t stride, const uint8_t* soft, uint8_t* out);
 __global__ void k_viterbi16w(const VitJob* jobs, const uint32_t* hdr, uint32_t jstride, uint32_t target, uint32_t vstride, const uint8_t* soft, uint8_t* out, uint16_t* vecs);
+__global__ void k_viterbi16w_p3(const VitJob* jobs, const uint32_t* hdr, uint32_t jstride, uint32_t target, uint32_t vstride, const uint8_t* soft, uint8_t* out, uint16_t* vecs);
 __global__ void k_viterbi16w_11n(const VitJob* jobs, const uint32_t* hdr, uint32_t jstride, uint32_t target, uint32_t vstride, const uint8_t* soft, uint8_t* out, uint16_t* vecs);
 __global__ void k_win_redo_11n(const VitJob* jobs, const uint32_t* hdr, uint32_t jstride, uint32_t target, uint32_t vstride, const uint16_t* vecs,
         const uint8_t* soft, uint8_t* out, unsigned long long* stats);
 __global__ void k_win_redo(const VitJob* jobs, const uint32_t* hdr, uint32_t jstride, uint32_t target, uint32_t vstride, const uint16_t* vecs,
+        const uint8_t* soft, uint8_t* out, unsigned long long* stats);
+__global__ void k_win_redo_p3(const VitJob* jobs, const uint32_t* hdr, uint32_t jstride, uint32_t target, uint32_t vstride, const uint16_t* vecs,
         const uint8_t* soft, uint8_t* out, unsigned long long* stats);
 __global__ void k_win_redo_finish(const VitJob* jobs, const uint32_t* hdr, uint32_t jstride, uint32_t target, uint32_t vstride, const uint16_t* vecs,
         const uint8_t* soft, uint8_t* out, unsigned long long* stats,
diff --git a/sora_amd/csrc/rx_types.h b/sora_amd/csrc/rx_types.h
--- a/sora_amd/csrc/rx_types.h
+++ b/sora_amd/csrc/rx_types.h
@@ -66,8 +66,11 @@
 }
 
 constexpr int kSoftPerSlot = 288;
-constexpr int kSoftBytesPerSlot = 108;
+constexpr int kSoftBytesPerSlot = 288;
 constexpr int kSoftSlack = 64;
+constexpr int kSoftScaled = 9;
+constexpr int kSoftPad = 66 * 1024;
+static_assert(kSoftPad >= 65568 + 7 * 24 + 16 + kSoftSlack, "the pad holds a maximal stream and the look-ahead");
 constexpr int kOutPerSlot  = 32;
 
 constexpr uint32_t E_FRAME_OK = 0x00000001u, E_PLCP_HEADER_FAIL = 0x80000005u, E_CRC32_FAIL = 0x80000006u,
diff --git a/sora_amd/csrc/sora_hip.cpp b/sora_amd/csrc/sora_hip.cpp
--- a/sora_amd/csrc/sora_hip.cpp
+++ b/sora_amd/csrc/sora_hip.cpp
@@ -557,7 +557,7 @@
     if (e != hipSuccess) { rx_free(rx); return fail(SORA_ERR_HARDWARE_FAILED, "pinned descriptor buffer", e); }
     const uint64_t n20 = cfg->max_total_samples / rx->str;
     const uint64_t want_slots = n20 / 80 + cfg->max_captures + 16, want_rows = (uint64_t)cfg->max_captures * cfg->max_frames_per_capture;
-    if (want_slots * (1ull * kSoftPerSlot) >= (1ull << 32) || want_rows >= (1ull << 31) / 3 || cfg->max_total_samples >= (1ull << 32)) {
+    if (want_slots * (1ull * kSoftBytesPerSlot) + kSoftPad >= (1ull << 32) || want_rows >= (1ull << 31) / 3 || cfg->max_total_samples >= (1ull << 32)) {
         rx_free(rx);
         return fail(SORA_ERR_CAPACITY, "sora_rx_create: max_total_samples / max_captures x max_frames_per_capture exceed the 32-bit slot geometry of one handle "
                                        "(split the batch over several handles)");
@@ -628,7 +628,9 @@
     rx->ncaps = (uint32_t)ncaps; rx->total_slots = slots; rx->have_results = false; rx->delivered = rx->released = false;
     if (ncaps == 0) { rx->have_results = true; return SORA_OK; }
     if (!rx->d_soft) {
-        HIPCHK(hipMalloc((void**)&rx->d_soft, (size_t)kSoftBytesPerSlot * rx->cap_slots + kSoftSlack));
+        const size_t soft_bytes = (size_t)kSoftBytesPerSlot * rx->cap_slots + kSoftPad;
+        HIPCHK(hipMalloc((void**)&rx->d_soft, soft_bytes));
+        HIPCHK(hipMemsetAsync(rx->d_soft, 0, soft_bytes, rx->stream));
         HIPCHK(hipMalloc((void**)&rx->d_jobs, 3 * sizeof(VitJob) * rx->cap_rows));
     }
     const bool windowed = rx->trellis == Trellis::Windowed;
@@ -1792,7 +1794,7 @@
         HIPCHK(hipMemsetD32Async((hipDeviceptr_t)hdr, (int)n, 1, st));
         HIPCHK(hipMemsetAsync(stats, 0, kWinStatsBytes, st));
     }
-    trellis_launch<WIN>(kind, trellis_single(jobs, hdr, (uint32_t)n), soft, d_out, st, W);
+    trellis_launch<WIN>(kind, trellis_single(jobs, hdr, (uint32_t)n, WIN == 256), soft, d_out, st, W);
     HIPCHK(hipGetLastError());
     return SORA_OK;
 }
```
